# nvaccess/NVSpeechPlayer

Measured on AMD Instinct MI355X. Metric: audio samples/sec (whole node) at 22.05 kHz Klatt synth, batch-N utterances, higher is better.
Workload: dtype f64

## Files before the change

### include/speechPlayer_batch.h

```cpp
#ifndef NVSP_AMD_SPEECHPLAYER_BATCH_H
#define NVSP_AMD_SPEECHPLAYER_BATCH_H

#include "speechPlayer.h"

#ifdef __cplusplus
extern "C" {
#endif

typedef void* speechPlayer_batch_t;

#define SPEECHPLAYER_MODE_EXACT 0
#define SPEECHPLAYER_MODE_FAST 1

speechPlayer_batch_t speechPlayer_batch_create(int sampleRate, int device);
void speechPlayer_batch_destroy(speechPlayer_batch_t batch);

int speechPlayer_batch_setOption(speechPlayer_batch_t batch, const char* name, int value);

int speechPlayer_batch_setUtterances(speechPlayer_batch_t batch, long long nUtterances, const long long* frameStart,
	const speechPlayer_frame_t* frames, const unsigned int* minFrameDuration, const unsigned int* fadeDuration,
	const int* userIndex, const unsigned char* isNull, const unsigned int* noiseSeed);

#define SPEECHPLAYER_RECORD_SILENCE 0xFFFFFFFFu
typedef struct {
	double voicePitch, endVoicePitch;
	unsigned int shape;
	unsigned int minFrameDuration, fadeDuration;
	int userIndex;
} speechPlayer_frameRecord_t;
int speechPlayer_batch_setUtterancesShared(speechPlayer_batch_t batch, long long nLists, const long long* listStart,
	const speechPlayer_frame_t* frames, const unsigned int* minFrameDuration, const unsigned int* fadeDuration,
	const int* userIndex, const unsigned char* isNull, long long nUtterances, const unsigned int* listOf, const unsigned int* noiseSeed);
int speechPlayer_batch_setRecords(speechPlayer_batch_t batch, long long nShapes, const speechPlayer_frame_t* shapes,
	long long nLists, const long long* listStart, const speechPlayer_frameRecord_t* records,
	long long nUtterances, const unsigned int* listOf, const unsigned int* noiseSeed);
int speechPlayer_batch_setUtterancesDevice(speechPlayer_batch_t batch, long long nUtterances, const long long* frameStart,
	const speechPlayer_frame_t* deviceFrames, const unsigned int* minFrameDuration, const unsigned int* fadeDuration,
	const int* userIndex, const unsigned char* isNull, const unsigned int* noiseSeed, void* readyStream);
long long speechPlayer_batch_exportPcm(speechPlayer_batch_t batch, const long long* utterances, long long nUtterances,
	void* deviceOut, int format, long long rowStride, void* stream);
#define SPEECHPLAYER_TRACK_MARK  47
#define SPEECHPLAYER_TRACK_FRAME 48
long long speechPlayer_planTimeline(long long nUtterances, const long long* frameStart, const unsigned int* minFrameDuration,
	const unsigned int* fadeDuration, long long* firstSample, long long* length);
long long speechPlayer_batch_timeline(speechPlayer_batch_t batch, long long utterance, long long* firstSample, int* userIndex,
	long long capacity);
long long speechPlayer_batch_exportTracks(speechPlayer_batch_t batch, const long long* utterances, long long nUtterances,
	const int* columns, int nColumns, long long hop, long long phase, void* deviceOut, int format, long long rowStride, void* stream);
#define SPEECHPLAYER_SOURCE_F0            0
#define SPEECHPLAYER_SOURCE_PHASE         1
#define SPEECHPLAYER_SOURCE_VIBRATO_PHASE 2
#define SPEECHPLAYER_SOURCE_CYCLE         3
#define SPEECHPLAYER_SOURCE_OPEN          4
#define SPEECHPLAYER_SOURCE_WAVE          5
#define SPEECHPLAYER_SOURCE_COLUMNS       6
#define SPEECHPLAYER_EPOCH_COLUMNS 4
long long speechPlayer_batch_exportSource(speechPlayer_batch_t batch, const long long* utterances, long long nUtterances,
	const int* columns, int nColumns, long long hop, long long phase, void* deviceOut, int format, long long rowStride, void* stream);
long long speechPlayer_batch_epochCounts(speechPlayer_batch_t batch, const long long* utterances, long long nUtterances, long long* counts);
long long speechPlayer_batch_exportEpochs(speechPlayer_batch_t batch, const long long* utterances, long long nUtterances,
	void* deviceOut, long long rowStride, double pad, long long capacity, void* stream);
#define SPEECHPLAYER_RESPONSE_CASCADE_RE   0
#define SPEECHPLAYER_RESPONSE_CASCADE_IM   1
#define SPEECHPLAYER_RESPONSE_CASCADE_MAG  2
#define SPEECHPLAYER_RESPONSE_CASCADE_DB   3
#define SPEECHPLAYER_RESPONSE_PARALLEL_RE  4
#define SPEECHPLAYER_RESPONSE_PARALLEL_IM  5
#define SPEECHPLAYER_RESPONSE_PARALLEL_MAG 6
#define SPEECHPLAYER_RESPONSE_PARALLEL_DB  7
#define SPEECHPLAYER_RESPONSE_KINDS        8
long long speechPlayer_frameResponse(const speechPlayer_frame_t* frames, long long nFrames, int sampleRate, const double* frequencies,
	int nFrequencies, const int* kinds, int nKinds, int gain, double* out);
long long speechPlayer_batch_exportResponse(speechPlayer_batch_t batch, const long long* utterances, long long nUtterances,
	const double* frequencies, int nFrequencies, const int* kinds, int nKinds, int gain, long long hop, long long phase,
	void* deviceOut, int format, long long rowStride, void* stream);
#define SPEECHPLAYER_STEM_VOICE      0
#define SPEECHPLAYER_STEM_ASPIRATION 1
#define SPEECHPLAYER_STEM_SOURCE     2
#define SPEECHPLAYER_STEM_FRICATION  3
#define SPEECHPLAYER_STEM_CASCADE    4
#define SPEECHPLAYER_STEM_PARALLEL   5
#define SPEECHPLAYER_STEM_OUTPUT     6
#define SPEECHPLAYER_STEM_COLUMNS    7
long long speechPlayer_batch_exportStems(speechPlayer_batch_t batch, const long long* utterances, long long nUtterances,
	const int* columns, int nColumns, void* deviceOut, int format, long long rowStride, void* stream);
long long speechPlayer_resonatorCoefficients(const double* frequency, const double* bandwidth, long long n, int anti, int sampleRate,
	double* abc);
long long speechPlayer_pcmSpectrogram(const sample* pcm, long long length, int nFft, long long hop, long long phase, const double* window,
	const double* bank, int nBands, int power, double logScale, double floor, double* out);
long long speechPlayer_batch_exportSpectrogram(speechPlayer_batch_t batch, const long long* utterances, long long nUtterances, int nFft,
	long long hop, long long phase, const double* window, const double* bank, int nBands, int power, double logScale, double floor,
	void* deviceOut, int format, long long rowStride, void* stream);
int speechPlayer_batch_device(speechPlayer_batch_t batch);

long long speechPlayer_batch_frames(speechPlayer_batch_t batch, long long utterance, speechPlayer_frame_t* frames,
	unsigned int* minFrameDuration, unsigned int* fadeDuration, int* userIndex, unsigned char* isNull, long long capacity);

long long speechPlayer_batch_utteranceSamples(speechPlayer_batch_t batch, long long utterance);
long long speechPlayer_batch_lengths(speechPlayer_batch_t batch, long long* lengths, long long capacity);
long long speechPlayer_batch_totalSamples(speechPlayer_batch_t batch);
long long speechPlayer_batch_totalFrames(speechPlayer_batch_t batch);
int speechPlayer_batch_sampleRate(speechPlayer_batch_t batch);

int speechPlayer_batch_synthesize(speechPlayer_batch_t batch);
int speechPlayer_batch_wait(speechPlayer_batch_t batch);

long long speechPlayer_batch_read(speechPlayer_batch_t batch, long long utterance, sample* sampleBuf, long long capacity);
long long speechPlayer_batch_readFloat(speechPlayer_batch_t batch, long long utterance, float* sampleBuf, long long capacity);
long long speechPlayer_batch_readAll(speechPlayer_batch_t batch, sample* sampleBuf, long long capacity, long long* outStart);
void* speechPlayer_hostAlloc(long long bytes);
void speechPlayer_hostFree(void* p);
long long speechPlayer_batch_readAllAsync(speechPlayer_batch_t batch, sample* sampleBuf, long long capacity, long long* outStart);
int speechPlayer_batch_readWait(speechPlayer_batch_t batch);
int speechPlayer_batch_digest(speechPlayer_batch_t batch, unsigned long long* perUtterance, unsigned long long* whole);
int speechPlayer_batch_getLastIndex(speechPlayer_batch_t batch, long long utterance);

const sample* speechPlayer_batch_devicePcm(speechPlayer_batch_t batch);
long long speechPlayer_batch_deviceOffset(speechPlayer_batch_t batch, long long utterance);

int speechPlayer_batch_time(speechPlayer_batch_t batch, int launches, float* msPerLaunch);

int speechPlayer_batch_kernelInfo(speechPlayer_batch_t batch, int* info, int nInfo);

long long speechPlayer_planTracks(long long nUtterances, const long long* frameStart, const speechPlayer_frame_t* frames,
	const unsigned int* fadeDuration, const unsigned char* isNull, const unsigned char* eligible, long long budgetMB,
	unsigned long long* trackOff, unsigned int* trackMask, unsigned char* tracked, unsigned long long* nEntries);

long long speechPlayer_planTracksFacts(long long nUtterances, const long long* frameStart, const speechPlayer_frame_t* frames,
	const unsigned int* fadeDuration, const unsigned char* isNull, const unsigned char* eligible, long long budgetMB, const void* facts24,
	unsigned long long* trackOff, unsigned int* trackMask, unsigned char* tracked, unsigned long long* nEntries, long long* collisionAt);
long long speechPlayer_planDirect(long long nUtterances, const long long* frameStart, const unsigned char* isNull,
                                  unsigned int* from, unsigned int* to, unsigned int* flags);
long long speechPlayer_frameFacts(const speechPlayer_frame_t* frames, long long nFrames, int sampleRate, int onDevice, void* facts24);

typedef void* speechPlayer_node_t;
speechPlayer_node_t speechPlayer_node_create(int sampleRate, int nDevices, const int* devices);
void speechPlayer_node_destroy(speechPlayer_node_t node);
int speechPlayer_node_devices(speechPlayer_node_t node);
int speechPlayer_node_setOption(speechPlayer_node_t node, const char* name, int value);
int speechPlayer_node_setUtterances(speechPlayer_node_t node, long long nUtterances, const long long* frameStart,
	const speechPlayer_frame_t* frames, const unsigned int* minFrameDuration, const unsigned int* fadeDuration,
	const int* userIndex, const unsigned char* isNull, const unsigned int* noiseSeed);
int speechPlayer_node_setRecords(speechPlayer_node_t node, long long nShapes, const speechPlayer_frame_t* shapes, long long nLists,
	const long long* listStart, const speechPlayer_frameRecord_t* records, long long nUtterances, const unsigned int* listOf,
	const unsigned int* noiseSeed);
int speechPlayer_node_setIpa(speechPlayer_node_t node, int sampleRate, long long nTexts, const char* const* ipaUtf8, double speed,
	const double* basePitch, double inflection, const char* clauseTypes, const int* voiceOf, const char* voiceName,
	double trailingSilenceMs, const unsigned int* noiseSeed);
int speechPlayer_node_synthesize(speechPlayer_node_t node);
int speechPlayer_node_wait(speechPlayer_node_t node);
long long speechPlayer_node_totalSamples(speechPlayer_node_t node);
long long speechPlayer_node_read(speechPlayer_node_t node, long long utterance, sample* sampleBuf, long long capacity);
int speechPlayer_node_getLastIndex(speechPlayer_node_t node, long long utterance);
int speechPlayer_node_shardInfo(speechPlayer_node_t node, int shard, long long* firstUtterance, long long* nUtterances, long long* samples, int* device);
long long speechPlayer_node_shardUtterances(speechPlayer_node_t node, int shard, long long* utterances, long long capacity);
speechPlayer_batch_t speechPlayer_node_part(speechPlayer_node_t node, int shard);
int speechPlayer_node_time(speechPlayer_node_t node, int launches, float* msPerLaunch);

int speechPlayer_synthesizeMany(speechPlayer_handle_t* handles, int nHandles, unsigned int sampleCount, sample** sampleBufs, int* produced);
int speechPlayer_synthesizeManyDevice(speechPlayer_handle_t* handles, int nHandles, unsigned int sampleCount, const sample** devicePcm,
	long long* rowStride, int* produced);
int speechPlayer_synthesizeManyExport(speechPlayer_handle_t* handles, int nHandles, unsigned int sampleCount, void* deviceOut,
	int format, long long rowStride, void* stream, int* produced);
int speechPlayer_queueFramesMany(const speechPlayer_handle_t* handles, int nHandles, const long long* frameStart,
	const speechPlayer_frame_t* frames, const unsigned int* minFrameDuration, const unsigned int* fadeDuration,
	const int* userIndex, const unsigned char* isNull, const unsigned char* purge);
int speechPlayer_queueFramesManyDevice(const speechPlayer_handle_t* handles, int nHandles, const long long* frameStart,
	const speechPlayer_frame_t* deviceFrames, const unsigned int* minFrameDuration, const unsigned int* fadeDuration,
	const int* userIndex, const unsigned char* isNull, const unsigned char* purge, void* readyStream);
int speechPlayer_handleDevice(speechPlayer_handle_t handle);
float speechPlayer_lastLiveKernelMs(int device);
int speechPlayer_lastLiveLaunches(int device);
int speechPlayer_setGlobalOption(const char* name, int value);
int speechPlayer_setNoiseSeed(speechPlayer_handle_t playerHandle, unsigned int seed);

long long speechPlayer_ipa_frames(const char* ipaUtf8, double speed, double basePitch, double inflection, int clauseType,
	const char* voiceName, speechPlayer_frame_t* frames, unsigned char* isNull, double* durationMs, double* fadeMs, long long capacity);
long long speechPlayer_ipa_pack(int sampleRate, long long nTexts, const char* const* ipaUtf8, double speed, const double* basePitch,
	double inflection, const char* clauseTypes, const char* voiceName, double trailingSilenceMs,
	long long* frameStart, speechPlayer_frame_t* frames, unsigned int* minFrameDuration, unsigned int* fadeDuration,
	unsigned char* isNull, long long frameCapacity);
int speechPlayer_batch_setIpa(speechPlayer_batch_t batch, long long nTexts, const char* const* ipaUtf8, double speed,
	const double* basePitch, double inflection, const char* clauseTypes, const char* voiceName, double trailingSilenceMs,
	const unsigned int* noiseSeed);
int speechPlayer_batch_setIpaVoices(speechPlayer_batch_t batch, long long nTexts, const char* const* ipaUtf8, double speed,
	const double* basePitch, double inflection, const char* clauseTypes, const int* voiceOf, double trailingSilenceMs,
	const unsigned int* noiseSeed);
typedef void* speechPlayer_records_t;
typedef struct {
	long long nShapes; const speechPlayer_frame_t* shapes;
	long long nLists; const long long* listStart;
	long long nRecords; const speechPlayer_frameRecord_t* records;
	long long nUtterances; const unsigned int* listOf;
} speechPlayer_recordsView_t;
speechPlayer_records_t speechPlayer_ipa_records(int sampleRate, long long nTexts, const char* const* ipaUtf8, double speed, const double* basePitch,
	double inflection, const char* clauseTypes, const int* voiceOf, const char* voiceName, double trailingSilenceMs);
int speechPlayer_records_view(speechPlayer_records_t records, speechPlayer_recordsView_t* view);
void speechPlayer_records_free(speechPlayer_records_t records);
typedef struct {
	int phoneme;
	unsigned int flags;
	int unit;
	int textOffset;
} speechPlayer_frameLabel_t;
enum {
	SPEECHPLAYER_LABEL_STRESS_MASK    = 3,
	SPEECHPLAYER_LABEL_TIED_TO        = 4,
	SPEECHPLAYER_LABEL_TIED_FROM      = 8,
	SPEECHPLAYER_LABEL_LONG           = 16,
	SPEECHPLAYER_LABEL_WORD_START     = 32,
	SPEECHPLAYER_LABEL_SYLLABLE_START = 64,
	SPEECHPLAYER_LABEL_GAP            = 128,
	SPEECHPLAYER_LABEL_PUFF           = 256
};
long long speechPlayer_ipa_labels(const char* ipaUtf8, int* phoneme, unsigned int* flags, int* unit, int* textOffset, long long capacity);
int speechPlayer_records_labels(speechPlayer_records_t records, const speechPlayer_frameLabel_t** labels, long long* nLabels);
int speechPlayer_batch_setRecordsLabelled(speechPlayer_batch_t batch, long long nShapes, const speechPlayer_frame_t* shapes,
	long long nLists, const long long* listStart, const speechPlayer_frameRecord_t* records, const speechPlayer_frameLabel_t* labels,
	long long nUtterances, const unsigned int* listOf, const unsigned int* noiseSeed);
int speechPlayer_batch_hasLabels(speechPlayer_batch_t batch);
#define SPEECHPLAYER_ALIGN_PHONEME     0
#define SPEECHPLAYER_ALIGN_STRESS      1
#define SPEECHPLAYER_ALIGN_FLAGS       2
#define SPEECHPLAYER_ALIGN_UNIT        3
#define SPEECHPLAYER_ALIGN_TEXT_OFFSET 4
#define SPEECHPLAYER_ALIGN_FRAME       5
#define SPEECHPLAYER_ALIGN_POSITION    6
#define SPEECHPLAYER_ALIGN_REMAINING   7
#define SPEECHPLAYER_ALIGN_COLUMNS     8
long long speechPlayer_batch_exportAlignment(speechPlayer_batch_t batch, const long long* utterances, long long nUtterances,
	const int* columns, int nColumns, long long hop, long long phase, void* deviceOut, int format, long long rowStride, long long pad,
	long long capacity, void* stream);
#define SPEECHPLAYER_UNIT_COLUMNS 7
long long speechPlayer_batch_exportUnits(speechPlayer_batch_t batch, const long long* utterances, long long nUtterances, long long hop,
	long long phase, int byFrame, void* deviceOut, long long rowStride, long long pad, long long capacity, void* stream);
long long speechPlayer_batch_unitCounts(speechPlayer_batch_t batch, const long long* utterances, long long nUtterances, int byFrame, long long* counts);
int speechPlayer_text_available(void);
long long speechPlayer_text_clauses(const char* textUtf8, long long* begin, long long* end, char* clauseType, double* endPauseMs, long long capacity);
long long speechPlayer_text_fixups(const char* ipaUtf8, char* out, long long capacity);
long long speechPlayer_text_toIpa(const char* textUtf8, const char* espeakVoice, char* out, long long capacity);
int speechPlayer_batch_setText(speechPlayer_batch_t batch, long long nTexts, const char* const* textUtf8, const char* espeakVoice, double speed,
	const double* basePitch, double inflection, const char* voiceName, const unsigned int* noiseSeed);
int speechPlayer_ipa_phonemeCount(void);
int speechPlayer_ipa_phoneme(int index, char* symbolUtf8, int symbolCapacity, double* values, unsigned long long* fieldMask, unsigned int* classBits);
int speechPlayer_voiceCount(void);
int speechPlayer_voicePresetCount(void);
const char* speechPlayer_voiceName(int index);
int speechPlayer_voiceIndex(const char* voiceName);
int speechPlayer_voiceDefine(const char* voiceName, int nEntries, const int* param, const double* absValue, const double* multiplier);
int speechPlayer_applyVoiceToFrame(speechPlayer_frame_t* frame, const char* voiceName);

const char* speechPlayer_lastError(void);
#define SPEECHPLAYER_OK 0
#define SPEECHPLAYER_ERR_ARGUMENT 1
#define SPEECHPLAYER_ERR_NO_DEVICE 2
#define SPEECHPLAYER_ERR_HIP 3
#define SPEECHPLAYER_ERR_TEXT_FRONTEND 4
int speechPlayer_lastErrorCode(void);

#ifdef __cplusplus
}
#endif

#endif
```

### nvspeechplayer_amd/_native.py

```python
import ctypes
import os
import shutil
import subprocess

PKG_DIR = os.path.dirname(os.path.abspath(__file__))
CSRC = os.path.join(PKG_DIR, "csrc")
LIB_DIR = os.path.join(PKG_DIR, "lib")
LIB_PATH = os.path.join(LIB_DIR, "libspeechPlayer.so")
SOURCES = ["klatt_engine.hip", "frame_producer.cpp"]
INCLUDE_DIR = os.path.join(os.path.dirname(PKG_DIR), "include")
OBJ_DIR = os.path.join(PKG_DIR, "build_tmp")
HIPCC_FLAGS = ["-O3", "--offload-arch=gfx950", "-ffp-contract=off", "-fPIC", "-std=c++17", "-Wall", "-Wno-unused-function",
               "-mllvm", "-amdgpu-sched-strategy=max-memory-clause"]
CXX_FLAGS = ["-O2", "-ffp-contract=off", "-fPIC", "-std=c++17", "-Wall", "-Wextra", "-DSPEECHPLAYER_LABELLED_SET"]
LINK_FLAGS = ["-shared", "-fPIC", "--offload-arch=gfx950", "-Wl,-rpath,/opt/rocm/lib"]

EXPORTS = [
    "speechPlayer_initialize", "speechPlayer_queueFrame", "speechPlayer_synthesize",
    "speechPlayer_getLastIndex", "speechPlayer_terminate",
    "speechPlayer_batch_create", "speechPlayer_batch_destroy", "speechPlayer_batch_setOption",
    "speechPlayer_batch_setUtterances", "speechPlayer_batch_utteranceSamples",
    "speechPlayer_batch_totalSamples", "speechPlayer_batch_totalFrames", "speechPlayer_batch_sampleRate",
    "speechPlayer_batch_synthesize", "speechPlayer_batch_wait", "speechPlayer_batch_read",
    "speechPlayer_batch_readAll", "speechPlayer_batch_readAllAsync", "speechPlayer_batch_readWait", "speechPlayer_hostAlloc", "speechPlayer_hostFree",
    "speechPlayer_batch_readFloat", "speechPlayer_batch_digest", "speechPlayer_batch_getLastIndex", "speechPlayer_batch_devicePcm",
    "speechPlayer_batch_deviceOffset", "speechPlayer_batch_time", "speechPlayer_batch_kernelInfo",
    "speechPlayer_lastError", "speechPlayer_lastErrorCode", "speechPlayer_setNoiseSeed", "speechPlayer_synthesizeMany", "speechPlayer_setGlobalOption",
    "speechPlayer_synthesizeManyDevice", "speechPlayer_lastLiveKernelMs", "speechPlayer_lastLiveLaunches",
    "speechPlayer_ipa_frames", "speechPlayer_ipa_pack", "speechPlayer_batch_setIpa",
    "speechPlayer_text_available", "speechPlayer_text_clauses", "speechPlayer_text_fixups", "speechPlayer_text_toIpa", "speechPlayer_batch_setText",
    "speechPlayer_voiceCount", "speechPlayer_voiceName", "speechPlayer_applyVoiceToFrame",
    "speechPlayer_ipa_phonemeCount", "speechPlayer_ipa_phoneme",
    "speechPlayer_node_create", "speechPlayer_node_destroy", "speechPlayer_node_devices", "speechPlayer_node_setOption",
    "speechPlayer_node_setUtterances", "speechPlayer_node_synthesize", "speechPlayer_node_wait", "speechPlayer_node_totalSamples",
    "speechPlayer_node_read", "speechPlayer_node_getLastIndex", "speechPlayer_node_shardInfo", "speechPlayer_node_shardUtterances", "speechPlayer_node_part", "speechPlayer_node_setRecords", "speechPlayer_node_setIpa",
    "speechPlayer_node_time", "speechPlayer_planTracks", "speechPlayer_planDirect", "speechPlayer_frameFacts", "speechPlayer_planTracksFacts",
    "speechPlayer_batch_setUtterancesShared", "speechPlayer_batch_setRecords", "speechPlayer_batch_frames", "speechPlayer_batch_setIpaVoices",
    "speechPlayer_ipa_records", "speechPlayer_records_view", "speechPlayer_records_free", "speechPlayer_voiceIndex", "speechPlayer_voiceDefine", "speechPlayer_voicePresetCount",
    "speechPlayer_batch_setUtterancesDevice", "speechPlayer_batch_exportPcm", "speechPlayer_batch_device", "speechPlayer_batch_lengths",
    "speechPlayer_queueFramesMany", "speechPlayer_queueFramesManyDevice", "speechPlayer_synthesizeManyExport", "speechPlayer_handleDevice",
    "speechPlayer_planTimeline", "speechPlayer_batch_timeline", "speechPlayer_batch_exportTracks",
    "speechPlayer_ipa_labels", "speechPlayer_records_labels", "speechPlayer_batch_setRecordsLabelled", "speechPlayer_batch_hasLabels",
    "speechPlayer_batch_exportAlignment", "speechPlayer_batch_exportUnits", "speechPlayer_batch_unitCounts",
    "speechPlayer_batch_exportSource", "speechPlayer_batch_epochCounts", "speechPlayer_batch_exportEpochs",
    "speechPlayer_frameResponse", "speechPlayer_batch_exportResponse",
    "speechPlayer_batch_exportStems", "speechPlayer_resonatorCoefficients",
    "speechPlayer_pcmSpectrogram", "speechPlayer_batch_exportSpectrogram",
]


def _deps(source):
    own = [os.path.join(CSRC, f) for f in os.listdir(CSRC) if f.endswith((".h", ".inc"))]
    pub = [os.path.join(INCLUDE_DIR, f) for f in os.listdir(INCLUDE_DIR) if f.endswith(".h")]
    return [os.path.join(CSRC, source)] + own + pub


def _obj(source):
    return os.path.join(OBJ_DIR, os.path.splitext(source)[0] + ".o")


def _obj_stale(source):
    o = _obj(source)
    if not os.path.exists(o):
        return True
    t = os.path.getmtime(o)
    return any(os.path.getmtime(p) > t for p in _deps(source))


def _stale():
    if not os.path.exists(LIB_PATH):
        return True
    t = os.path.getmtime(LIB_PATH)
    return any(os.path.getmtime(p) > t for src in SOURCES for p in _deps(src))


def build(force=False, verbose=False, extra_hipcc_flags=(), lib_path=None):
    out = lib_path or LIB_PATH
    variant = bool(extra_hipcc_flags) or lib_path is not None
    if not force and not variant and not _stale():
        return out
    hipcc = shutil.which("hipcc") or "/opt/rocm/bin/hipcc"
    if not os.path.exists(hipcc):
        raise RuntimeError("hipcc not found; cannot build %s" % out)
    os.makedirs(os.path.dirname(out), exist_ok=True)
    os.makedirs(OBJ_DIR, exist_ok=True)
    import fcntl
    with open(os.path.join(OBJ_DIR, ".build.lock"), "w") as lock:
        fcntl.flock(lock, fcntl.LOCK_EX)
        if not force and not variant and not _stale():
            return out
        return _build_locked(hipcc, out, variant, force, verbose, extra_hipcc_flags)


def _build_locked(hipcc, out, variant, force, verbose, extra_hipcc_flags):
    objs = []
    for src in SOURCES:
        is_hip = src.endswith(".hip")
        own = variant and is_hip
        o = os.path.join(OBJ_DIR, os.path.basename(out) + "." + os.path.splitext(src)[0] + ".o") if own else _obj(src)
        if force or own or _obj_stale(src):
            flags = list(HIPCC_FLAGS)
            extra = list(extra_hipcc_flags)
            for f in [f for f in extra if f.startswith("--sched=")]:
                extra.remove(f)
                i = flags.index("-mllvm")
                del flags[i:i + 2]
                if f != "--sched=none":
                    flags += ["-mllvm", "-amdgpu-sched-strategy=" + f[len("--sched="):]]
            cmd = ([hipcc] + flags + extra if is_hip else ["g++"] + CXX_FLAGS) + ["-c", os.path.join(CSRC, src), "-o", o]
            if verbose:
                print(" ".join(cmd))
            subprocess.check_call(cmd)
        objs.append(o)
    tmp = out + ".tmp.%d" % os.getpid()
    cmd = [hipcc] + LINK_FLAGS + ["-o", tmp] + objs
    if verbose:
        print(" ".join(cmd))
    subprocess.check_call(cmd)
    os.replace(tmp, out)
    if variant:
        for o in objs:
            if os.path.basename(o).startswith(os.path.basename(out) + "."):
                try:
                    os.remove(o)
                except OSError:
                    pass
    return out


_lib = None


def load():
    global _lib
    if _lib is not None:
        return _lib
    path = os.environ.get("SPEECHPLAYER_LIB", LIB_PATH)
    if not os.path.exists(path):
        raise RuntimeError("%s is missing: run `python -c 'import __graft_entry__ as g; g.build()'` "
                           "(the engine has no CPU fallback)" % path)
    L = ctypes.CDLL(path)
    vp, u32, i32, i64 = ctypes.c_void_p, ctypes.c_uint, ctypes.c_int, ctypes.c_longlong
    L.speechPlayer_initialize.restype = vp
    L.speechPlayer_initialize.argtypes = [i32]
    L.speechPlayer_queueFrame.restype = None
    L.speechPlayer_queueFrame.argtypes = [vp, vp, u32, u32, i32, ctypes.c_bool]
    L.speechPlayer_synthesize.restype = i32
    L.speechPlayer_synthesize.argtypes = [vp, u32, vp]
    L.speechPlayer_getLastIndex.restype = i32
    L.speechPlayer_getLastIndex.argtypes = [vp]
    L.speechPlayer_terminate.restype = None
    L.speechPlayer_terminate.argtypes = [vp]
    L.speechPlayer_setNoiseSeed.restype = i32
    L.speechPlayer_setNoiseSeed.argtypes = [vp, u32]
    L.speechPlayer_synthesizeMany.restype = i32
    L.speechPlayer_synthesizeMany.argtypes = [vp, i32, u32, vp, vp]
    L.speechPlayer_synthesizeManyDevice.restype = i32
    L.speechPlayer_synthesizeManyDevice.argtypes = [vp, i32, u32, vp, vp, vp]
    L.speechPlayer_synthesizeManyExport.restype = i32
    L.speechPlayer_synthesizeManyExport.argtypes = [vp, i32, u32, vp, i32, i64, vp, vp]
    L.speechPlayer_queueFramesMany.restype = i32
    L.speechPlayer_queueFramesMany.argtypes = [vp, i32, vp, vp, vp, vp, vp, vp, vp]
    L.speechPlayer_queueFramesManyDevice.restype = i32
    L.speechPlayer_queueFramesManyDevice.argtypes = [vp, i32, vp, vp, vp, vp, vp, vp, vp, vp]
    L.speechPlayer_handleDevice.restype = i32
    L.speechPlayer_handleDevice.argtypes = [vp]
    L.speechPlayer_lastLiveKernelMs.restype = ctypes.c_float
    L.speechPlayer_lastLiveKernelMs.argtypes = [i32]
    L.speechPlayer_lastLiveLaunches.restype = i32
    L.speechPlayer_lastLiveLaunches.argtypes = [i32]
    L.speechPlayer_setGlobalOption.restype = i32
    L.speechPlayer_setGlobalOption.argtypes = [ctypes.c_char_p, i32]
    L.speechPlayer_lastError.restype = ctypes.c_char_p
    L.speechPlayer_lastError.argtypes = []
    L.speechPlayer_lastErrorCode.restype = i32
    L.speechPlayer_lastErrorCode.argtypes = []
    L.speechPlayer_batch_create.restype = vp
    L.speechPlayer_batch_create.argtypes = [i32, i32]
    L.speechPlayer_batch_destroy.restype = None
    L.speechPlayer_batch_destroy.argtypes = [vp]
    L.speechPlayer_batch_setOption.restype = i32
    L.speechPlayer_batch_setOption.argtypes = [vp, ctypes.c_char_p, i32]
    L.speechPlayer_batch_setUtterances.restype = i32
    L.speechPlayer_batch_setUtterances.argtypes = [vp, i64, vp, vp, vp, vp, vp, vp, vp]
    L.speechPlayer_batch_utteranceSamples.restype = i64
    L.speechPlayer_batch_utteranceSamples.argtypes = [vp, i64]
    L.speechPlayer_batch_totalSamples.restype = i64
    L.speechPlayer_batch_totalSamples.argtypes = [vp]
    L.speechPlayer_batch_totalFrames.restype = i64
    L.speechPlayer_batch_totalFrames.argtypes = [vp]
    L.speechPlayer_batch_synthesize.restype = i32
    L.speechPlayer_batch_synthesize.argtypes = [vp]
    L.speechPlayer_batch_wait.restype = i32
    L.speechPlayer_batch_wait.argtypes = [vp]
    L.speechPlayer_batch_read.restype = i64
    L.speechPlayer_batch_read.argtypes = [vp, i64, vp, i64]
    L.speechPlayer_batch_readFloat.restype = i64
    L.speechPlayer_batch_readFloat.argtypes = [vp, i64, vp, i64]
    L.speechPlayer_batch_readAll.restype = i64
    L.speechPlayer_batch_readAll.argtypes = [vp, vp, i64, vp]
    L.speechPlayer_batch_readAllAsync.restype = i64
    L.speechPlayer_batch_readAllAsync.argtypes = [vp, vp, i64, vp]
    L.speechPlayer_batch_readWait.restype = i32
    L.speechPlayer_batch_readWait.argtypes = [vp]
    L.speechPlayer_hostAlloc.restype = vp
    L.speechPlayer_hostAlloc.argtypes = [i64]
    L.speechPlayer_hostFree.restype = None
    L.speechPlayer_hostFree.argtypes = [vp]
    L.speechPlayer_batch_digest.restype = i32
    L.speechPlayer_batch_digest.argtypes = [vp, vp, vp]
    L.speechPlayer_batch_getLastIndex.restype = i32
    L.speechPlayer_batch_getLastIndex.argtypes = [vp, i64]
    L.speechPlayer_batch_devicePcm.restype = vp
    L.speechPlayer_batch_devicePcm.argtypes = [vp]
    L.speechPlayer_batch_deviceOffset.restype = i64
    L.speechPlayer_batch_deviceOffset.argtypes = [vp, i64]
    L.speechPlayer_batch_time.restype = i32
    L.speechPlayer_batch_time.argtypes = [vp, i32, vp]
    L.speechPlayer_batch_kernelInfo.restype = i32
    L.speechPlayer_batch_kernelInfo.argtypes = [vp, vp, i32]
    L.speechPlayer_batch_sampleRate.restype = i32
    L.speechPlayer_batch_sampleRate.argtypes = [vp]
    f64 = ctypes.c_double
    L.speechPlayer_ipa_frames.restype = i64
    L.speechPlayer_ipa_frames.argtypes = [ctypes.c_char_p, f64, f64, f64, i32, ctypes.c_char_p, vp, vp, vp, vp, i64]
    L.speechPlayer_ipa_pack.restype = i64
    L.speechPlayer_ipa_pack.argtypes = [i32, i64, vp, f64, vp, f64, ctypes.c_char_p, ctypes.c_char_p, f64, vp, vp, vp, vp, vp, i64]
    L.speechPlayer_text_available.restype = i32
    L.speechPlayer_text_available.argtypes = []
    L.speechPlayer_text_clauses.restype = i64
    L.speechPlayer_text_clauses.argtypes = [ctypes.c_char_p, vp, vp, vp, vp, i64]
    L.speechPlayer_text_fixups.restype = i64
    L.speechPlayer_text_fixups.argtypes = [ctypes.c_char_p, vp, i64]
    L.speechPlayer_text_toIpa.restype = i64
    L.speechPlayer_text_toIpa.argtypes = [ctypes.c_char_p, ctypes.c_char_p, vp, i64]
    L.speechPlayer_batch_setText.restype = i32
    L.speechPlayer_batch_setText.argtypes = [vp, i64, vp, ctypes.c_char_p, f64, vp, f64, ctypes.c_char_p, vp]
    L.speechPlayer_batch_setIpa.restype = i32
    L.speechPlayer_batch_setIpa.argtypes = [vp, i64, vp, f64, vp, f64, ctypes.c_char_p, ctypes.c_char_p, f64, vp]
    L.speechPlayer_node_create.restype = vp
    L.speechPlayer_node_create.argtypes = [i32, i32, vp]
    L.speechPlayer_node_destroy.restype = None
    L.speechPlayer_node_destroy.argtypes = [vp]
    L.speechPlayer_node_devices.restype = i32
    L.speechPlayer_node_devices.argtypes = [vp]
    L.speechPlayer_node_setOption.restype = i32
    L.speechPlayer_node_setOption.argtypes = [vp, ctypes.c_char_p, i32]
    L.speechPlayer_node_setUtterances.restype = i32
    L.speechPlayer_node_setUtterances.argtypes = [vp, i64, vp, vp, vp, vp, vp, vp, vp]
    L.speechPlayer_node_synthesize.restype = i32
    L.speechPlayer_node_synthesize.argtypes = [vp]
    L.speechPlayer_node_wait.restype = i32
    L.speechPlayer_node_wait.argtypes = [vp]
    L.speechPlayer_node_totalSamples.restype = i64
    L.speechPlayer_node_totalSamples.argtypes = [vp]
    L.speechPlayer_node_read.restype = i64
    L.speechPlayer_node_read.argtypes = [vp, i64, vp, i64]
    L.speechPlayer_node_getLastIndex.restype = i32
    L.speechPlayer_node_getLastIndex.argtypes = [vp, i64]
    L.speechPlayer_node_shardInfo.restype = i32
    L.speechPlayer_node_shardInfo.argtypes = [vp, i32, vp, vp, vp, vp]
    L.speechPlayer_node_shardUtterances.restype = i64
    L.speechPlayer_node_shardUtterances.argtypes = [vp, i32, vp, i64]
    L.speechPlayer_node_setRecords.restype = i32
    L.speechPlayer_node_setRecords.argtypes = [vp, i64, vp, i64, vp, vp, i64, vp, vp]
    L.speechPlayer_node_setIpa.restype = i32
    L.speechPlayer_node_setIpa.argtypes = [vp, i32, i64, vp, f64, vp, f64, ctypes.c_char_p, vp, ctypes.c_char_p, f64, vp]
    L.speechPlayer_node_part.restype = vp
    L.speechPlayer_node_part.argtypes = [vp, i32]
    L.speechPlayer_node_time.restype = i32
    L.speechPlayer_node_time.argtypes = [vp, i32, vp]
    L.speechPlayer_voiceCount.restype = i32
    L.speechPlayer_voiceCount.argtypes = []
    L.speechPlayer_voiceName.restype = ctypes.c_char_p
    L.speechPlayer_voiceName.argtypes = [i32]
    L.speechPlayer_applyVoiceToFrame.restype = i32
    L.speechPlayer_applyVoiceToFrame.argtypes = [vp, ctypes.c_char_p]
    L.speechPlayer_ipa_phonemeCount.restype = i32
    L.speechPlayer_ipa_phonemeCount.argtypes = []
    L.speechPlayer_ipa_phoneme.restype = i32
    L.speechPlayer_ipa_phoneme.argtypes = [i32, vp, i32, vp, vp, vp]
    L.speechPlayer_planTracks.restype = i64
    L.speechPlayer_planTracks.argtypes = [i64, vp, vp, vp, vp, vp, i64, vp, vp, vp, vp]
    L.speechPlayer_frameFacts.restype = i64
    L.speechPlayer_frameFacts.argtypes = [vp, i64, i32, i32, vp]
    L.speechPlayer_planDirect.restype = i64
    L.speechPlayer_planDirect.argtypes = [i64, vp, vp, vp, vp, vp]
    L.speechPlayer_planTracksFacts.restype = i64
    L.speechPlayer_planTracksFacts.argtypes = [i64, vp, vp, vp, vp, vp, i64, vp, vp, vp, vp, vp, vp]
    L.speechPlayer_batch_setUtterancesDevice.restype = i32
    L.speechPlayer_batch_setUtterancesDevice.argtypes = [vp, i64, vp, vp, vp, vp, vp, vp, vp, vp]
    L.speechPlayer_planTimeline.restype = i64
    L.speechPlayer_planTimeline.argtypes = [i64, vp, vp, vp, vp, vp]
    L.speechPlayer_batch_timeline.restype = i64
    L.speechPlayer_batch_timeline.argtypes = [vp, i64, vp, vp, i64]
    L.speechPlayer_batch_exportTracks.restype = i64
    L.speechPlayer_batch_exportTracks.argtypes = [vp, vp, i64, vp, i32, i64, i64, vp, i32, i64, vp]
    L.speechPlayer_batch_exportPcm.restype = i64
    L.speechPlayer_batch_exportPcm.argtypes = [vp, vp, i64, vp, i32, i64, vp]
    L.speechPlayer_batch_device.restype = i32
    L.speechPlayer_batch_device.argtypes = [vp]
    L.speechPlayer_batch_lengths.restype = i64
    L.speechPlayer_batch_lengths.argtypes = [vp, vp, i64]
    L.speechPlayer_batch_setUtterancesShared.restype = i32
    L.speechPlayer_batch_setUtterancesShared.argtypes = [vp, i64, vp, vp, vp, vp, vp, vp, i64, vp, vp]
    L.speechPlayer_batch_setRecords.restype = i32
    L.speechPlayer_batch_setRecords.argtypes = [vp, i64, vp, i64, vp, vp, i64, vp, vp]
    L.speechPlayer_batch_frames.restype = i64
    L.speechPlayer_batch_frames.argtypes = [vp, i64, vp, vp, vp, vp, vp, i64]
    L.speechPlayer_batch_setIpaVoices.restype = i32
    L.speechPlayer_batch_setIpaVoices.argtypes = [vp, i64, vp, f64, vp, f64, ctypes.c_char_p, vp, f64, vp]
    L.speechPlayer_ipa_records.restype = vp
    L.speechPlayer_ipa_records.argtypes = [i32, i64, vp, f64, vp, f64, ctypes.c_char_p, vp, ctypes.c_char_p, f64]
    L.speechPlayer_records_view.restype = i32
    L.speechPlayer_records_view.argtypes = [vp, vp]
    L.speechPlayer_records_free.restype = None
    L.speechPlayer_records_free.argtypes = [vp]
    L.speechPlayer_voicePresetCount.restype = i32
    L.speechPlayer_voicePresetCount.argtypes = []
    L.speechPlayer_voiceIndex.restype = i32
    L.speechPlayer_voiceIndex.argtypes = [ctypes.c_char_p]
    L.speechPlayer_voiceDefine.restype = i32
    L.speechPlayer_voiceDefine.argtypes = [ctypes.c_char_p, i32, vp, vp, vp]
    L.speechPlayer_ipa_labels.restype = i64
    L.speechPlayer_ipa_labels.argtypes = [ctypes.c_char_p, vp, vp, vp, vp, i64]
    L.speechPlayer_records_labels.restype = i32
    L.speechPlayer_records_labels.argtypes = [vp, vp, vp]
    L.speechPlayer_batch_setRecordsLabelled.restype = i32
    L.speechPlayer_batch_setRecordsLabelled.argtypes = [vp, i64, vp, i64, vp, vp, vp, i64, vp, vp]
    L.speechPlayer_batch_hasLabels.restype = i32
    L.speechPlayer_batch_hasLabels.argtypes = [vp]
    L.speechPlayer_batch_exportAlignment.restype = i64
    L.speechPlayer_batch_exportAlignment.argtypes = [vp, vp, i64, vp, i32, i64, i64, vp, i32, i64, i64, i64, vp]
    L.speechPlayer_batch_exportUnits.restype = i64
    L.speechPlayer_batch_exportUnits.argtypes = [vp, vp, i64, i64, i64, i32, vp, i64, i64, i64, vp]
    L.speechPlayer_batch_unitCounts.restype = i64
    L.speechPlayer_batch_unitCounts.argtypes = [vp, vp, i64, i32, vp]
    L.speechPlayer_batch_exportSource.restype = i64
    L.speechPlayer_batch_exportSource.argtypes = [vp, vp, i64, vp, i32, i64, i64, vp, i32, i64, vp]
    L.speechPlayer_batch_epochCounts.restype = i64
    L.speechPlayer_batch_epochCounts.argtypes = [vp, vp, i64, vp]
    L.speechPlayer_batch_exportEpochs.restype = i64
    L.speechPlayer_batch_exportEpochs.argtypes = [vp, vp, i64, vp, i64, f64, i64, vp]
    L.speechPlayer_frameResponse.restype = i64
    L.speechPlayer_frameResponse.argtypes = [vp, i64, i32, vp, i32, vp, i32, i32, vp]
    L.speechPlayer_batch_exportResponse.restype = i64
    L.speechPlayer_batch_exportResponse.argtypes = [vp, vp, i64, vp, i32, vp, i32, i32, i64, i64, vp, i32, i64, vp]
    L.speechPlayer_batch_exportStems.restype = i64
    L.speechPlayer_batch_exportStems.argtypes = [vp, vp, i64, vp, i32, vp, i32, i64, vp]
    L.speechPlayer_resonatorCoefficients.restype = i64
    L.speechPlayer_resonatorCoefficients.argtypes = [vp, vp, i64, i32, i32, vp]
    L.speechPlayer_pcmSpectrogram.restype = i64
    L.speechPlayer_pcmSpectrogram.argtypes = [vp, i64, i32, i64, i64, vp, vp, i32, i32, f64, f64, vp]
    L.speechPlayer_batch_exportSpectrogram.restype = i64
    L.speechPlayer_batch_exportSpectrogram.argtypes = [vp, vp, i64, i32, i64, i64, vp, vp, i32, i32, f64, f64, vp, i32, i64, vp]
    _lib = L
    return L


def last_error():
    return (load().speechPlayer_lastError() or b"").decode("utf8", "replace")


# ... 3 lines not shown
```

### nvspeechplayer_amd/csrc/klatt_device.h

```cpp
#pragma once

#include <hip/hip_runtime.h>
#include <stdint.h>
#include <type_traits>

#include "klatt_math.h"

namespace klatt {

constexpr int kNumParams = 47;
constexpr int kLanes = 64;
constexpr int kTile = 32;
constexpr int kTileStride = kTile * 2 + 8;
constexpr int kSlots = 45;
constexpr int kNumRes = 14;
constexpr int kBlock = 16;
constexpr int kStateDoubles = 240;

constexpr int MODE_EXACT = 0;
constexpr int MODE_FAST = 1;

constexpr uint32_t FRAME_NULL = 1u;
constexpr uint32_t UTT_NEEDS_NOISE = 1u;
constexpr uint32_t UTT_TRACKED = 4u;
// ... 2 lines not shown

struct FrameMeta {
    uint32_t minSamples;
    uint32_t fadeSamples;
    int32_t userIndex;
    uint32_t flags;
};

struct UttDesc {
    long long frameStart;
    long long outStart;
    uint32_t nFrames;
    uint32_t seed;
    uint32_t flags;
    uint32_t length;
};

struct UttResult {
    uint32_t produced;
    uint32_t framesTaken;
    int32_t lastIndex;
    uint32_t drained;
};

constexpr int kTrackEntries = 24;
constexpr int kTrackFirst = kTrackEntries + 1;
constexpr int kShapeValues = 45;
constexpr int kShapeStride = 46;
__host__ __device__ constexpr int shape_param(int i)
{
    constexpr int kF[14] = {13, 14, 12, 11, 10, 9, 8, 7, 25, 26, 27, 28, 29, 30};
    constexpr int kB[14] = {21, 22, 20, 19, 18, 17, 16, 15, 31, 32, 33, 34, 35, 36};
    constexpr int kG[17] = {23, 41, 42, 43, 45, 24, 44, 37, 38, 39, 40, 1, 2, 3, 4, 5, 6};
    return i < 28 ? ((i & 1) ? kB[i >> 1] : kF[i >> 1]) : kG[i - 28];
}
constexpr int kShapePreGain = 28 + 6;
__host__ __device__ constexpr int entry_value(int e, int half)
{
    constexpr int kV[10][2] = {{28, -1}, {29, 30}, {31, 32}, {33, 34}, {35, 36}, {37, 38}, {39, 40}, {41, 42}, {43, 44}, {34, -1}};
    return kV[e - 14][half];
}
struct TrackRef {
    unsigned long long off;
    uint32_t mask;
    uint32_t nSlots;
};
struct FlatRef {
    uint32_t off;
    uint32_t mask;
    uint32_t fadeSamples;
    uint32_t span;
};
struct SourceRef {
    double pitch;
    double pitchInc;
    double invFade;
    int32_t userIndex;
    uint32_t flags;
};
struct TrackJob {
    unsigned long long off;
    uint32_t fromShape, toShape;
    uint32_t fadeSamples;
    uint32_t mask;
};
__host__ __device__ inline uint32_t track_slots(uint32_t mask) { return (uint32_t)__builtin_popcount(mask) + (mask & 1u); }
constexpr int kTrackStages = 4;
#ifndef KLATT_FLAT_LAYOUT
#define KLATT_FLAT_LAYOUT 2
#endif
__host__ __device__ constexpr uint32_t track_stage_kinds(int s)
{
    return KLATT_FLAT_LAYOUT == 2 ? (s == 0 ? 0xF04003u : s == 1 ? 0x0000FCu : s == 2 ? 0x01B000u : 0x0E0F00u)
                                  : (s == 0 ? 0xF00000u : s == 1 ? 0x00403Fu : s == 2 ? 0x01B0C0u : 0x0E0F00u);
}
__host__ __device__ constexpr uint32_t track_stage_entries(int s)
{
    return KLATT_FLAT_LAYOUT == 2 ? (s == 0 ? 8u : s == 1 ? 6u : s == 2 ? 4u : 7u) : (s == 0 ? 4u : s == 1 ? 8u : s == 2 ? 6u : 7u);
}
constexpr int kTrackAntiStage = KLATT_FLAT_LAYOUT == 2 ? 0 : 1;
__host__ __device__ inline uint32_t track_stage_slots(uint32_t mask, int s) { return (uint32_t)__builtin_popcount(mask & track_stage_kinds(s)) + (s == kTrackAntiStage ? (mask & 1u) : 0u); }
__host__ __device__ inline uint32_t track_part(uint32_t mask, uint32_t F, int s)
{
    uint32_t at = 0;
    for (int k = 0; k < s; ++k) at += track_stage_entries(k) + (F - 1u) * track_stage_slots(mask, k);
    return at;
}

struct DirectHdr {
    uint32_t fadeSamples;
    uint32_t span;
    uint32_t bits;
    uint32_t pad;
};
struct DirectJob {
    uint32_t frame;
    uint32_t from, to;
    uint32_t flags;
};
constexpr uint32_t kNoFrame = 0xFFFFFFFFu;
constexpr uint32_t kDirectBwShift = 8, kDirectClsShift = 14, kDirectAllBits = 0x3FFFFFFu;
constexpr int kDirectStages = 8;
#ifndef KLATT_DIRECT_FAST_LAYOUT
#define KLATT_DIRECT_FAST_LAYOUT 1
#endif
__host__ __device__ constexpr int direct_layout(int mode) { return mode == MODE_FAST ? KLATT_DIRECT_FAST_LAYOUT : 0; }
__host__ __device__ constexpr int direct_stage_res(int s, int L = 0)
{
    return L == 1 ? (s < 2 ? 0 : (s == 3 || s == 4) ? 3 : 2) : (s == 0 ? 0 : 2);
}
__host__ __device__ constexpr int direct_stage_gains(int s, int L = 0)
{
    return L == 1 ? (s == 0 ? 1 : s == 1 ? 3 : s == 2 ? 1 : s == 5 ? 2 : s == 6 ? 1 : s == 7 ? 2 : 0)
                  : (s == 0 ? 4 : s == 1 ? 1 : s == 5 ? 2 : s == 6 ? 1 : s == 7 ? 2 : 0);
}
__host__ __device__ constexpr int direct_stage_entries(int s, int L = 0) { return 4 * direct_stage_res(s, L) + 3 * direct_stage_gains(s, L); }
__host__ __device__ constexpr int direct_stage_first(int s, int L = 0) { int at = 0; for (int k = 0; k < s; ++k) at += direct_stage_entries(k, L); return at; }
constexpr int kDirectEntries = direct_stage_first(kDirectStages);
static_assert(direct_stage_first(kDirectStages, 1) == kDirectEntries, "both layouts hold the same kinds");
__host__ __device__ constexpr int direct_stage_kind(int s, int e, int L = 0)
{
    constexpr int k0[kDirectStages][4] = {{20, 21, 22, 23}, {0, 1, 14, -1}, {2, 3, -1, -1}, {4, 5, -1, -1}, {6, 7, -1, -1}, {8, 9, 17, 18}, {10, 11, 19, -1}, {12, 13, 15, 16}};
    constexpr int k1[kDirectStages][4] = {{20, -1, -1, -1}, {21, 22, 23, -1}, {0, 1, 14, -1}, {2, 3, 4, -1}, {5, 6, 7, -1}, {8, 9, 17, 18}, {10, 11, 19, -1}, {12, 13, 15, 16}};
    return L == 1 ? k1[s][e] : k0[s][e];
}

struct KernelArgs {
    const DirectHdr* directHdr;
    const double2* directRec;
    const uint32_t* directFirst;
    uint32_t nDirect;
    const FlatRef* flatRef;
    const SourceRef* sourceRef;
    uint32_t trackBytes;
    const double2* track;
    const double* frames;
    const FrameMeta* meta;
    const UttDesc* utt;
    const uint32_t* order;
    int16_t* pcm;
    UttResult* result;
    double* state;
    double* const* statePtrs;
    const uint32_t* control;
    long long nSlots;
    uint32_t maxSamples;
    uint32_t ringMask;
    int sampleRate;
    double sampleRateF;
    double invSampleRate;
    double negPiOverSr;
    double twoPiOverSr;
    unsigned long long* debug;
};

__device__ constexpr int kResF[kNumRes] = {13, 14, 12, 11, 10, 9, 8, 7, 25, 26, 27, 28, 29, 30};
__device__ constexpr int kResB[kNumRes] = {21, 22, 20, 19, 18, 17, 16, 15, 31, 32, 33, 34, 35, 36};
constexpr int kNumHot = 17;
__device__ constexpr int kHot[kNumHot] = {1, 2, 3, 4, 5, 6, 23, 24, 37, 38, 39, 40, 41, 42, 43, 44, 45};


__device__ __forceinline__ double div_by(double x, double b, double y)
{
    double q = x * y;
    double r = __builtin_fma(-b, q, x);
    return __builtin_fma(r, y, q);
}

__device__ __forceinline__ double frac_toward_zero(double x) { return x - __builtin_trunc(x); }

__device__ __forceinline__ double fade_value(double from, double to, double ratio)
{
    double v = from + ((to - from) * ratio);
    return (to != to) ? from : v;
}

__device__ __forceinline__ uint32_t mix32(uint32_t x)
{
    x ^= x >> 16; x *= 0x7FEB352Du; x ^= x >> 15; x *= 0x846CA68Bu; x ^= x >> 16;
    return x;
}
__device__ __forceinline__ uint32_t noise_key(uint32_t seed) { return mix32(seed ^ 0x9E3779B9u); }
__device__ __forceinline__ uint32_t noise_inc(uint32_t seed) { return (mix32(seed + 0x85EBCA6Bu) << 1) | 1u; }
constexpr uint32_t kNoiseA = 1664525u;
constexpr uint32_t kNoiseA2 = kNoiseA * kNoiseA;
__device__ __forceinline__ uint32_t noise_inc2(uint32_t inc) { return (kNoiseA + 1u) * inc; }
__device__ __forceinline__ uint32_t noise_step(uint32_t s, uint32_t inc) { return s * kNoiseA + inc; }
__device__ __forceinline__ uint32_t noise_step2(uint32_t s, uint32_t inc2) { return s * kNoiseA2 + inc2; }
__device__ __forceinline__ uint32_t noise_first(uint32_t key, uint32_t inc) { return noise_step(key, inc); }
__device__ __forceinline__ double noise_uniform(uint32_t s)
{
    const double r = (double)(s >> 1);
    return __builtin_fma(r, 0x1.00000002p-31, r * 0x1p-93);
}

template <int MODE>
__device__ __forceinline__ double dot3(double a, double x, double b, double y, double c, double z)
{
    if (MODE == MODE_FAST) return __builtin_fma(c, z, __builtin_fma(b, y, a * x));
    return a * x + b * y + c * z;
}

#ifdef KLATT_SIGNAL_F32
typedef float sig_t;
#else
typedef double sig_t;
#endif
template <int MODE>
__device__ __forceinline__ float dot3(float a, float x, float b, float y, float c, float z)
{
    return __builtin_fmaf(c, z, __builtin_fmaf(b, y, a * x));
}
__device__ __forceinline__ float fade_value(float from, float to, float ratio)
{
    float v = from + ((to - from) * ratio);
    return (to != to) ? from : v;
}

struct Coef { double a, b, c; };
enum { COEF_UNREDUCED = 0, COEF_QUADRANT_M1 = 1, COEF_UNKNOWN = 2 };
#ifndef KLATT_COLD_CALL
#define KLATT_COLD_CALL 2
#endif
struct RadCos { double rad, cs; };
#if KLATT_COLD_CALL
__device__ __attribute__((noinline)) RadCos exp_cos_reduced(double ex, double th)
{
    RadCos o;
#if KLATT_COLD_CALL == 1
    if (__builtin_fabs(ex) <= 700.0 && __builtin_fabs(th) <= 1.0e4) { o.rad = fast_exp(ex); o.cs = fast_cos(th); }
    else
#endif
    { o.rad = exp(ex); o.cs = cos(th); }
    return o;
}
#endif
template <bool NESTED = true>
__device__ __forceinline__ RadCos coefficient_parts(double f, double bw, double negPiOverSr, double twoPiOverSr, int cls = COEF_UNKNOWN)
{
    const double ex = negPiOverSr * bw;
    const double th = twoPiOverSr * -f;
    double rad, cs;
    const bool eu = exp_is_unreduced(ex);
    if (cls == COEF_UNREDUCED) { rad = exp_unreduced(ex); cs = cos_unreduced(th); }
    else if (cls == COEF_QUADRANT_M1) { rad = exp_unreduced(ex); cs = cos_quadrant_m1(th); }
    else if (__all(eu && cos_is_unreduced(th))) { rad = exp_unreduced(ex); cs = cos_unreduced(th); }
    else if (__all(eu && cos_is_quadrant_m1(th))) { rad = exp_unreduced(ex); cs = cos_quadrant_m1(th); }
#if KLATT_COLD_CALL == 1
    else if (NESTED) { const RadCos o = exp_cos_reduced(ex, th); rad = o.rad; cs = o.cs; }
#endif
    else if (__builtin_fabs(ex) <= 700.0 && __builtin_fabs(th) <= 1.0e4) { rad = fast_exp(ex); cs = fast_cos(th); }
#if KLATT_COLD_CALL == 2
    else if (NESTED) { const RadCos o = exp_cos_reduced(ex, th); rad = o.rad; cs = o.cs; }
#endif
    else { rad = exp(ex); cs = cos(th); }
    RadCos o; o.rad = rad; o.cs = cs;
    return o;
}
__host__ __device__ __forceinline__ Coef coefficient_finish(double rad, double cs, bool anti, double f)
{
    double cc = -(rad * rad);
    double bb = rad * cs * 2.0;
    double aa = 1.0 - bb - cc;
    if (anti && f != 0) {
        aa = 1.0 / aa;
        cc *= -aa;
        bb *= -aa;
    }
    Coef k; k.a = aa; k.b = bb; k.c = cc;
    return k;
}
template <int MODE, bool NESTED = true>
__device__ __forceinline__ Coef resonator_coefficients_inline(double f, double bw, bool anti, double negPiOverSr, double twoPiOverSr,
                                                              int cls = COEF_UNKNOWN)
{
    const RadCos p = coefficient_parts<NESTED>(f, bw, negPiOverSr, twoPiOverSr, cls);
    return coefficient_finish(p.rad, p.cs, anti, f);
}
template <int MODE>
__device__ __attribute__((noinline)) Coef resonator_coefficients(double f, double bw, bool anti, double negPiOverSr, double twoPiOverSr)
{
    return resonator_coefficients_inline<MODE, false>(f, bw, anti, negPiOverSr, twoPiOverSr);
}

template <bool STREAM>
struct LdsLayout {
    static constexpr int kOld = 0;
    static constexpr int kNew = kOld + kSlots * kLanes * 8;
    static constexpr int kCurFB = kNew + kSlots * kLanes * 8;
    static constexpr int kTileOff = kCurFB + (STREAM ? 28 * kLanes * 8 : 0);
    static constexpr int kRowBase = kTileOff + kLanes * kTileStride;
    static constexpr int kRowCount = kRowBase + kLanes * 8;
    static constexpr int kBytes = kRowCount + kLanes * 4;
};

struct Lane {
    double cur[kNumParams];
    double old0, new0, oldInc, newInc, invFade;
    double ra[kNumRes], rb[kNumRes], rc[kNumRes], z1[kNumRes], z2[kNumRes];
    double pitchPhase, vibPhase, aspNoise, fricNoise;
    uint32_t cnt, oldMin, newMin, newFade;
    uint32_t resMask, nextFrame, noiseState, produced;
    int32_t lastIndex;
    bool hasNew, oldNull, newNull, done, drained;
    bool vibFrames;
};
// ... 381 lines not shown
```

### nvspeechplayer_amd/csrc/klatt_engine.hip

```cpp
#include "klatt_device.h"
#include "klatt_systolic.h"
#include "klatt_lanepipe.h"
#include "klatt_tracks.h"
#include "klatt_direct.h"
#include "klatt_plan.h"
#include "klatt_timeline.h"
#include "klatt_align.h"
#include "klatt_source.h"
#include "klatt_response.h"
#include "klatt_stems.h"
#include "klatt_spectrum.h"
#include "klatt_export.h"

#include <algorithm>
#include <cmath>
#include <cstdarg>
#include <cstdio>
#include <cstdlib>
#include <cstring>
#include <chrono>
#include <mutex>
#include <atomic>
#include <system_error>
#include <thread>
// ... 334 lines not shown
    a.sampleRate = sampleRate;
    a.sampleRateF = (double)sampleRate;
    a.invSampleRate = 1.0 / (double)sampleRate;
    a.negPiOverSr = -M_PI / sampleRate;
    a.twoPiOverSr = (M_PI * 2) / sampleRate;
    a.maxSamples = 0xFFFFFFFFu;
    return a;
}

template <bool NOISE, int CH, int WPS = 1, bool NASAL = true, bool STREAM = false, bool FLAT = false, bool LONE = false>
int launch_systolic(const KernelArgs& a, int mode, long long nGroups, hipStream_t stream)
{
    if (nGroups <= 0) return 0;
    if (nGroups > 0x7FFFFFFF) { set_error("too many workgroups: %lld", nGroups); return -1; }
    constexpr int ldsBytes = SysLds<NOISE, CH, FLAT, stream_split<STREAM, WPS, LONE>()>::kBytes + (LONE ? kStages * kLoneLdsPerStage : 0);
    static_assert(ldsBytes <= 160 * 1024, "a workgroup's LDS");
    auto go = [&](auto kernel) -> int {
        if (ensure_lds_limit(reinterpret_cast<const void*>(kernel), ldsBytes)) return -1;
        hipLaunchKernelGGL(kernel, dim3((unsigned)nGroups), dim3(kLanes * kStages), ldsBytes, stream, a);
        return 0;
    };
    int rc;
    switch (mode) {
    case MODE_EXACT: rc = go(klatt_systolic<MODE_EXACT, NOISE, CH, WPS, NASAL, STREAM, FLAT, LONE>); break;
    case MODE_FAST: rc = go(klatt_systolic<MODE_FAST, NOISE, CH, WPS, NASAL, STREAM, FLAT, LONE>); break;
    default: set_error("unknown arithmetic mode %d", mode); return -1;
    }
    if (rc) return rc;
    HIP_TRY(hipGetLastError());
    return 0;
}

constexpr int kDirectChunk = 16, kDirectLeanChunk = 8;
template <int CH, int WPE>
int launch_direct_as(const KernelArgs& a, int mode, long long nGroups, hipStream_t stream)
{
    constexpr int ldsBytes = DirectLds<CH>::kBytes;
    auto go = [&](auto kernel) -> int {
        if (ensure_lds_limit(reinterpret_cast<const void*>(kernel), ldsBytes)) return -1;
        hipLaunchKernelGGL(kernel, dim3((unsigned)nGroups), dim3(kLanes * kDirectStages), ldsBytes, stream, a);
        return 0;
    };
    int rc;
    switch (mode) {
    case MODE_EXACT: rc = go(klatt_direct<MODE_EXACT, CH, WPE>); break;
    case MODE_FAST: rc = go(klatt_direct<MODE_FAST, CH, WPE>); break;
    default: set_error("unknown arithmetic mode %d", mode); return -1;
    }
    if (rc) return rc;
    HIP_TRY(hipGetLastError());
    return 0;
}
int launch_direct(const KernelArgs& a, int mode, bool lean, long long nGroups, hipStream_t stream)
{
    if (nGroups <= 0) return 0;
    if (nGroups > 0x7FFFFFFF) { set_error("too many workgroups: %lld", nGroups); return -1; }
    return lean ? launch_direct_as<kDirectLeanChunk, 4>(a, mode, nGroups, stream) : launch_direct_as<kDirectChunk, 2>(a, mode, nGroups, stream);
}

#ifndef KLATT_LP_CH
#define KLATT_LP_CH 32
#endif
template <int CH, int WPS>
int launch_lanepipe(const KernelArgs& a, int mode, long long nGroups, hipStream_t stream)
{
    if (nGroups <= 0) return 0;
    if (nGroups > 0x7FFFFFFF) { set_error("too many workgroups: %lld", nGroups); return -1; }
    constexpr int ldsBytes = LpLds<CH>::kBytes;
    auto go = [&](auto kernel) -> int {
        if (ensure_lds_limit(reinterpret_cast<const void*>(kernel), ldsBytes)) return -1;
        hipLaunchKernelGGL(kernel, dim3((unsigned)nGroups), dim3(kLanes * kStages), ldsBytes, stream, a);
        return 0;
    };
    int rc;
    switch (mode) {
    case MODE_EXACT: rc = go(klatt_lanepipe<MODE_EXACT, CH, WPS>); break;
    case MODE_FAST: rc = go(klatt_lanepipe<MODE_FAST, CH, WPS>); break;
    default: set_error("unknown arithmetic mode %d", mode); return -1;
    }
    if (rc) return rc;
    HIP_TRY(hipGetLastError());
    return 0;
}

#ifndef KLATT_NOISY_CH
#define KLATT_NOISY_CH 8
#endif
struct GroupPlan { bool systolic; int chunk; };
GroupPlan plan_group(int layout, bool noisy, long long nUttBatch, long long nNoisyBatch, int cus)
{
    const long long groups = (nUttBatch + kLanes - 1) / kLanes + 1;
    GroupPlan p;
    p.systolic = layout != 0;
    (void)nNoisyBatch;
    p.chunk = noisy ? (groups <= cus ? 16 : 8)
                    : (groups <= cus ? 32 : 16);
    return p;
}

template <bool STREAM, bool NOISE>
int launch(const KernelArgs& a, int mode, long long nWaves, hipStream_t stream)
{
    if (nWaves <= 0) return 0;
    if (nWaves > 0x7FFFFFFF) { set_error("too many wavefronts: %lld", nWaves); return -1; }
    constexpr int ldsBytes = LdsLayout<STREAM>::kBytes;
    auto go = [&](auto kernel) -> int {
        if (ensure_lds_limit(reinterpret_cast<const void*>(kernel), ldsBytes)) return -1;
        hipLaunchKernelGGL(kernel, dim3((unsigned)nWaves), dim3(kLanes), ldsBytes, stream, a);
        return 0;
    };
    int rc;
    switch (mode) {
    case MODE_EXACT: rc = go(klatt_synthesize<MODE_EXACT, STREAM, NOISE>); break;
    case MODE_FAST: rc = go(klatt_synthesize<MODE_FAST, STREAM, NOISE>); break;
    default:
        set_error("unknown arithmetic mode %d", mode);
        return -1;
    }
    if (rc) return rc;
    HIP_TRY(hipGetLastError());
    return 0;
}

int pick_device(int device)
{
    int n = 0;
    hipError_t e = hipGetDeviceCount(&n);
    if (e != hipSuccess || n <= 0) {
        set_error_code(SPEECHPLAYER_ERR_NO_DEVICE);
        set_error("no HIP device available (%s); this engine has no CPU path", e == hipSuccess ? "count 0" : hipGetErrorString(e));
        return -1;
    }
    if (device < 0) {
        const char* env = getenv("SPEECHPLAYER_DEVICE");
        if (env) device = atoi(env);
        else if (hipGetDevice(&device) != hipSuccess) device = 0;
    }
    if (device >= n) { set_error("device %d out of range (%d devices)", device, n); return -1; }
    return device;
}

struct Batch {
    int sampleRate = 0;
    int device = 0;
    int mode = MODE_EXACT;
    int sortByLength = 1;
    int layout = -1;
    int cus = 256;
    hipStream_t stream = nullptr;
    int tracks = 1;
    long long trackBudgetMB = 4096;
    hipStream_t side[6] = {nullptr, nullptr, nullptr, nullptr, nullptr, nullptr};
    hipEvent_t forkEvent = nullptr, join[6] = {nullptr, nullptr, nullptr, nullptr, nullptr, nullptr};
    int quietLast = 1;
    long long nUtt = 0, nFrames = 0, nSlots = 0;
    long long nLists = 0, nFramesSpoken = 0;
    std::vector<long long> uttFrameStart;
    std::vector<uint32_t> uttFrames;
    bool launched = false;
    long long nQuiet = 0;
    long long nTracked = 0;
    long long nTrackedUtt = 0;
    long long nJobs = 0, trackEntries = 0;
    int directLean = -1;
    bool directAligned = false;
    int direct = 1;
    long long nDirect = 0;
    long long nDirectUtt = 0, nDirectFrames = 0;
    long long nNoNasal = 0;
    long long nNoNasalUtt = 0;
    long long totalSamples = 0, poolSamples = 0;
    std::vector<uint32_t> lens;
    std::vector<uint32_t> uttSeed;
    std::vector<long long> outStart;
    std::vector<UttResult> results;
    bool resultsFresh = false;
    DeviceBuffer<double> dFrames;
    DeviceBuffer<FrameMeta> dMeta;
    DeviceBuffer<UttDesc> dUtt;
    DeviceBuffer<uint32_t> dOrder;
    DeviceBuffer<int16_t> dPcm;
    DeviceBuffer<UttResult> dResult;
    DeviceBuffer<FlatRef> dFlatRef;
    DeviceBuffer<SourceRef> dSourceRef;
    DeviceBuffer<TrackJob> dJobs;
    DeviceBuffer<double> dShapes;
    DeviceBuffer<double2> dTrack;
    DeviceBuffer<DirectJob> dDirectJobs;
    DeviceBuffer<uint32_t> dDirectFirst;
    DeviceBuffer<DirectHdr> dDirectHdr;
    DeviceBuffer<double2> dDirectRec;
    DeviceBuffer<unsigned long long> dDebug;
    DeviceBuffer<float> dFloat;
    DeviceBuffer<unsigned long long> dDigest;
    PinnedPair bounce;
    DeviceBuffer<FrameRecord> dRecords;
    DeviceBuffer<double> dShapeTable;
    DeviceBuffer<uint32_t> dRep;
    DeviceBuffer<unsigned long long> dMismatch;
    DeviceBuffer<FrameFacts> dFacts;
    PinnedBlock hFacts;
    DeviceBuffer<int16_t> dDense;
    DeviceBuffer<long long> dDenseStart;
    std::vector<long long> denseStart;
    hipStream_t copyStream = nullptr;
    hipEvent_t denseReady = nullptr, copyDone = nullptr;
    bool copyPending = false;
    bool floatFresh = false;
    hipEvent_t inputReady = nullptr;
    DeviceBuffer<long long> dShapeIdx;
    DeviceBuffer<double> dShapeRows;
    hipEvent_t pcmReady = nullptr;
    struct ExportSlot { PinnedBlock host; DeviceBuffer<unsigned char> dev; hipEvent_t done = nullptr; bool used = false; };
    static constexpr int kExportSlots = 16;
    ExportSlot exportSlot[kExportSlots];
    unsigned exportNext = 0;
    struct SharedTable {
        hipEvent_t done = nullptr;
        bool used = false;
        int wait(hipStream_t st) { if (used) HIP_TRY(hipStreamWaitEvent(st, done, 0)); return 0; }
        int mark(hipStream_t st) { HIP_TRY(hipEventRecord(done, st)); used = true; return 0; }
    };
    std::vector<uint32_t> uttList;
    DeviceBuffer<long long> dListStart;
    DeviceBuffer<TimelineReq> dTimeline;
    hipEvent_t setDone = nullptr, setCopied = nullptr, timelineReady = nullptr;
    bool timelineFresh = false;
    ExportSlot trackSlot[kExportSlots];
    unsigned trackNext = 0;
    DeviceBuffer<double> dPitch;
    SharedTable pitchOrder;
    long long pitchBudgetMB = 256;
    DeviceBuffer<FrameLabel> dLabels;
    DeviceBuffer<uint32_t> dUnitFirst;
    std::vector<uint32_t> listUnits;
    bool hasLabels = false;
    DeviceBuffer<double> dSource;
    DeviceBuffer<double> dEpochs;
    SharedTable sourceOrder;
    DeviceBuffer<long long> dEpochCount;
    std::vector<long long> epochCount;
    bool epochFresh = false;
    long long sourceBudgetMB = 256;
    long long sourceLaneLists = 12288;
};

int wait_exports(Batch* b)
{
    for (auto& s : b->exportSlot)
        if (s.used) HIP_TRY(hipStreamWaitEvent(b->stream, s.done, 0));
    return 0;
}
int sync_exports(Batch* b)
{
    for (auto& s : b->exportSlot)
        if (s.used) { HIP_TRY(hipEventSynchronize(s.done)); s.used = false; }
    return 0;
}

int settle_track_exports(Batch* b, bool onHost)
{
    for (auto& s : b->trackSlot) {
        if (!s.used) continue;
        if (onHost) { HIP_TRY(hipEventSynchronize(s.done)); s.used = false; }
        else { HIP_TRY(hipStreamWaitEvent(b->stream, s.done, 0)); HIP_TRY(hipStreamWaitEvent(b->copyStream, s.done, 0)); }
    }
    return 0;
}


template <typename T>
int grow_table(Batch* b, DeviceBuffer<T>& buf, size_t n)
{
    if (n > buf.cap && settle_track_exports(b, true)) return -1;
    return buf.reserve(std::max<size_t>(n, 1));
}

int timeline_on_stream(Batch* b, hipStream_t st)
{
    if (b->timelineFresh) { HIP_TRY(hipStreamWaitEvent(st, b->timelineReady, 0)); return 0; }
    if (grow_table(b, b->dTimeline, (size_t)b->nFrames)) return -1;
    HIP_TRY(hipStreamWaitEvent(st, b->setDone, 0));
    HIP_TRY(hipStreamWaitEvent(st, b->setCopied, 0));
    const unsigned grid = (unsigned)std::min<long long>((b->nLists + 255) / 256, 4ll * b->cus);
    hipLaunchKernelGGL(klatt_timeline_requests, dim3(std::max(grid, 1u)), dim3(256), 0, st, b->dMeta.ptr, b->dListStart.ptr, b->nLists, b->dTimeline.ptr);
    HIP_TRY(hipGetLastError());
    HIP_TRY(hipEventRecord(b->timelineReady, st));
    b->timelineFresh = true;
    return 0;
}

template <class Fn>
long long batch_entry(const char* what, speechPlayer_batch_t batch, Fn fn)
{
    begin_call();
    Batch* b = static_cast<Batch*>(batch);
    if (!b) { set_error("%s: no batch", what); return -1; }
    try {
        return fn(b);
    } catch (const std::exception& e) { set_error("%s: %s", what, e.what()); return -1; }
}

long long check_selection(Batch* b, const char* what, const long long* utterances, long long nUtterances, bool frameLimit)
{
    const long long n = utterances ? nUtterances : b->nUtt;
    if (n < 0) { set_error("%s: %lld utterances", what, n); return -1; }
// ... 404 lines not shown
    });
    lap("parts planned");
    struct ShapeKey { const double* v; bool operator==(const ShapeKey& o) const { return !memcmp(v, o.v, kShapeValues * sizeof(double)); } };
    struct ShapeKeyHash { size_t operator()(const ShapeKey& k) const { return (size_t)hash_shape(k.v); } };
    struct FadeKey { uint32_t from, to, len; bool operator==(const FadeKey& o) const { return from == o.from && to == o.to && len == o.len; } };
    struct FadeKeyHash { size_t operator()(const FadeKey& k) const { unsigned long long h = ((unsigned long long)k.from << 32 | k.to) * 0x9E3779B97F4A7C15ull; h ^= h >> 29; h += k.len; h *= 0xFF51AFD7ED558CCDull; return (size_t)(h ^ (h >> 32)); } };
    long long eligibleAll = 0, missedSize = 0, missedBudget = 0;
    size_t nShapesUpper = 0;
    for (const TrackPlan& p : part) { eligibleAll += p.eligible; missedSize += p.missedSize; missedBudget += p.missedBudget; nShapesUpper += p.shapes.size() / kShapeStride; }
    if (missedBudget > 0) {
        part.clear();
        plan_tracks_pass(nUtterances, frameStart, frames, facts, meta, eligible, budgetMB, true, nullptr, out);
        return;
    }
    out.shapes.clear();
    out.shapes.reserve(nShapesUpper * kShapeStride);
    out.jobs.clear();
    out.entries = 0;
    std::unordered_map<ShapeKey, uint32_t, ShapeKeyHash> shapes;
    std::unordered_map<FadeKey, unsigned long long, FadeKeyHash> fades;
    std::vector<std::unordered_map<unsigned long long, unsigned long long>> offOf(nThreads);
    for (unsigned t = 0; t < nThreads; ++t) {
        const TrackPlan& p = part[t];
        std::vector<uint32_t> gid(p.shapes.size() / kShapeStride);
        for (size_t i = 0; i < gid.size(); ++i) {
            const ShapeKey key{&p.shapes[i * kShapeStride]};
            auto it = shapes.find(key);
            if (it == shapes.end()) {
                const uint32_t id = (uint32_t)(out.shapes.size() / kShapeStride);
                out.shapes.insert(out.shapes.end(), key.v, key.v + kShapeStride);
                it = shapes.emplace(ShapeKey{&out.shapes[(size_t)id * kShapeStride]}, id).first;
            }
            gid[i] = it->second;
        }
        for (const TrackJob& j : p.jobs) {
            const FadeKey key{gid[j.fromShape], gid[j.toShape], j.fadeSamples};
            auto it = fades.find(key);
            if (it == fades.end()) {
                it = fades.emplace(key, out.entries).first;
                out.jobs.push_back(TrackJob{out.entries, key.from, key.to, j.fadeSamples, j.mask});
                out.entries += (unsigned long long)kTrackFirst + (unsigned long long)(j.fadeSamples - 1u) * track_slots(j.mask);
            }
            offOf[t].emplace(j.off, it->second);
        }
    }
    const unsigned long long budget = std::min((unsigned long long)std::max(budgetMB, 0ll) * (1ull << 20) / sizeof(double2), (1ull << 28) - (1ull << 21) - kTrackPad);
    if (out.entries > budget) {
        plan_tracks_pass(nUtterances, frameStart, frames, facts, meta, eligible, budgetMB, true, nullptr, out);
        return;
    }
    out.eligible = eligibleAll; out.missedSize = missedSize; out.missedBudget = 0;
    out.ref.assign((size_t)nF, TrackRef{0, 0, 0});
    out.rep.assign(nF < 0xFFFFFFFFll ? (size_t)nF : 0, 0xFFFFFFFFu);
    out.tracked.assign((size_t)nUtterances, 0);
    out.kinds.assign((size_t)nUtterances, 0);
    if (missedSize * 10 > eligibleAll) { out.jobs.clear(); out.entries = 0; return; }
    run_parts(nThreads, [&](unsigned t) {
        const TrackPlan& p = part[t];
        const long long f0 = frameStart[cut[t]];
        for (long long u = cut[t]; u < cut[t + 1]; ++u) {
            if (!p.tracked[u - cut[t]]) continue;
            out.tracked[u] = 1;
            out.kinds[u] = p.kinds[u - cut[t]];
            for (long long k = frameStart[u]; k < frameStart[u + 1]; ++k) {
                TrackRef r = p.ref[k - f0];
                r.off = offOf[t].find(r.off)->second;
                out.ref[k] = r;
                if (!out.rep.empty() && !p.rep.empty()) out.rep[k] = p.rep[k - f0];
            }
        }
    });
    lap("merged");
}

#ifdef KLATT_TIMING_ONLY_BUILD
constexpr bool kTimingOnlyBuild = true;
#else
constexpr bool kTimingOnlyBuild = false;
#endif
bool refuse_timing_only(const char* what)
{
    if (!kTimingOnlyBuild || getenv("SPEECHPLAYER_ALLOW_TIMING_ONLY_PCM")) return false;
    set_error_code(SPEECHPLAYER_ERR_ARGUMENT);
    set_error("%s: this library was built with a timing-only experiment switch; its PCM is not valid", what);
    return true;
}

template <class V>
void walk_fade_ends(long long k0, long long k1, const FrameMeta* meta, V& out)
{
    uint32_t prevReal = kNoFrame;
    bool prevNull = true;
    for (long long k = k0; k < k1; ++k) {
        DirectJob j;
        j.frame = (uint32_t)k;
        if (meta[k].flags & FRAME_NULL) {
            j.from = prevReal; j.to = prevReal;
            j.flags = (prevNull ? 1u : 0u) | 2u;
            prevNull = true;
        } else {
            j.to = (uint32_t)k;
            j.from = prevNull ? (uint32_t)k : prevReal;
            j.flags = prevNull ? 1u : 0u;
            prevReal = (uint32_t)k;
            prevNull = false;
        }
        out.push_back(j);
    }
}

template <class T>
struct NoInitAlloc : std::allocator<T> {
    template <class U> struct rebind { using other = NoInitAlloc<U>; };
    NoInitAlloc() = default;
    template <class U> NoInitAlloc(const NoInitAlloc<U>&) {}
    template <class U> void construct(U* p) { ::new (static_cast<void*>(p)) U; }
    template <class U, class... A> void construct(U* p, A&&... a) { ::new (static_cast<void*>(p)) U(std::forward<A>(a)...); }
};
template <class T> using RawVector = std::vector<T, NoInitAlloc<T>>;

long long tracked_count(const Batch* b) { return (b->tracks && b->layout != 0) ? b->nTracked : 0; }
long long direct_count(const Batch* b) { return b->nDirect; }
bool direct_lean(const Batch* b, long long nGroups)
{
    if (b->directLean >= 0) return b->directLean != 0;
    if (b->directAligned) return false;
    return b->mode == MODE_FAST ? true : nGroups > 2ll * b->cus;
}

int batch_launch(Batch* b)
{
    KernelArgs a = base_args(b->sampleRate);
    a.frames = b->dFrames.ptr; a.meta = b->dMeta.ptr; a.utt = b->dUtt.ptr;
    a.pcm = b->dPcm.ptr; a.result = b->dResult.ptr; a.state = nullptr; a.control = nullptr;
    if (wait_exports(b)) return -1;
    b->resultsFresh = false;
    b->floatFresh = false;
    b->launched = true;
#ifdef KLATT_STAMPS
    if (b->dDebug.reserve((size_t)(b->nSlots / kLpUPG + 2) * 32 * 2)) return -1;
    HIP_TRY(hipMemsetAsync(b->dDebug.ptr, 0, b->dDebug.cap * 8, b->stream));
    a.debug = b->dDebug.ptr;
#endif
    const long long nLp = lanepipe_count(b);
    const bool laneKernel = b->layout == 0;
    const long long nTr = tracked_count(b);
    const long long nDir = direct_count(b);
    const long long nNoisyHead = b->nTracked - nTr;
    const long long nNoisy = b->nSlots - b->nQuiet - b->nTracked - nDir;
    const long long nNn = laneKernel ? 0 : b->nNoNasal - nLp;
    const long long nQ = b->nQuiet - nLp - nNn;
    const int parts = (nLp > 0) + (nNn > 0) + (nQ > 0) + (nNoisy > 0) + (nNoisyHead > 0) + (nTr > 0) + (nDir > 0);
    const bool fork = parts > 1;
    if (fork) HIP_TRY(hipEventRecord(b->forkEvent, b->stream));
    int sideUsed = 0, seen = 0;
    auto next_stream = [&](bool = false) -> hipStream_t {
        if (!fork || ++seen == parts) return b->stream;
        hipStream_t st = b->side[sideUsed++];
        (void)hipStreamWaitEvent(st, b->forkEvent, 0);
        return st;
    };
    const GroupPlan plq = plan_group(b->layout, false, b->nSlots, nNoisy, b->cus);
    auto launch_quiet = [&]() -> int {
    if (nLp > 0) {
        hipStream_t st = next_stream(true);
        a.order = b->dOrder.ptr; a.nSlots = nLp;
        const long long g = (nLp + kLpUPG - 1) / kLpUPG;
        if (g <= b->cus ? launch_lanepipe<KLATT_LP_CH, 1>(a, b->mode, g, st) : launch_lanepipe<16, 2>(a, b->mode, g, st)) return -1;
    }
    if (nNn > 0) {
        hipStream_t st = next_stream(true);
        a.order = b->dOrder.ptr + nLp; a.nSlots = nNn;
        const long long g = (nNn + kLanes - 1) / kLanes;
        if (plq.chunk == 32 ? launch_systolic<false, 32, 1, false>(a, b->mode, g, st) : launch_systolic<false, 16, 2, false>(a, b->mode, g, st)) return -1;
    }
    if (nQ > 0) {
        hipStream_t st = next_stream(true);
        a.order = b->dOrder.ptr + nLp + nNn; a.nSlots = nQ;
        const long long g = (nQ + kLanes - 1) / kLanes;
        if (plq.systolic ? (plq.chunk == 32 ? launch_systolic<false, 32>(a, b->mode, g, st) : launch_systolic<false, 16>(a, b->mode, g, st))
                         : launch<false, false>(a, b->mode, g, st)) return -1;
    }
        return 0;
    };
    const bool quietLast = b->quietLast && (nTr > 0 || nDir > 0) && nNoisy == 0 && nNoisyHead == 0;
    if (!quietLast && launch_quiet()) return -1;
    if (nTr > 0) {
        hipStream_t st = next_stream();
        TrackArgs t;
        t.jobs = b->dJobs.ptr; t.nJobs = b->nJobs; t.shapes = b->dShapes.ptr; t.track = b->dTrack.ptr;
        t.negPiOverSr = a.negPiOverSr; t.twoPiOverSr = a.twoPiOverSr;
        const long long tg = b->nJobs;
        if (tg > 0x7FFFFFFF) { set_error("too many tracks: %lld", b->nJobs); return -1; }
        hipLaunchKernelGGL(klatt_tracks, dim3((unsigned)tg), dim3(kLanes * kTrackWaves), 0, st, t);
        HIP_TRY(hipGetLastError());
        a.order = b->dOrder.ptr + b->nQuiet; a.nSlots = nTr;
        a.flatRef = b->dFlatRef.ptr; a.sourceRef = b->dSourceRef.ptr; a.track = b->dTrack.ptr;
        a.trackBytes = (uint32_t)std::min<unsigned long long>(((unsigned long long)b->trackEntries + kTrackPad) * sizeof(double2), 0xFFFFFFFFull);
        const GroupPlan pl = plan_group(b->layout, true, b->nSlots, nTr + nNoisy, b->cus);
        const long long g = (nTr + kLanes - 1) / kLanes;
        if (pl.chunk == 8 ? launch_systolic<true, KLATT_FLAT_CH, KLATT_FLAT_WPS, true, false, true>(a, b->mode, g, st)
                          : launch_systolic<true, 16, 1, true, false, true>(a, b->mode, g, st)) return -1;
        a.flatRef = nullptr; a.sourceRef = nullptr; a.track = nullptr;
    }
    if (nDir > 0) {
        hipStream_t st = next_stream();
        SeedArgs sa;
        sa.jobs = b->dDirectJobs.ptr; sa.nJobs = (uint32_t)b->nDirectFrames; sa.frames = b->dFrames.ptr; sa.meta = b->dMeta.ptr;
        sa.hdr = b->dDirectHdr.ptr; sa.rec = b->dDirectRec.ptr; sa.negPiOverSr = a.negPiOverSr; sa.twoPiOverSr = a.twoPiOverSr;
        const dim3 sg((unsigned)((b->nDirectFrames + 255) / 256), (unsigned)kDirectStages);
        constexpr int kSeedLds = 14 * 257 * (int)sizeof(double2);
        if (b->mode == MODE_FAST) hipLaunchKernelGGL(klatt_seeds<MODE_FAST>, sg, dim3(256), kSeedLds, st, sa);
        else hipLaunchKernelGGL(klatt_seeds<MODE_EXACT>, sg, dim3(256), kSeedLds, st, sa);
        HIP_TRY(hipGetLastError());
        a.order = b->dOrder.ptr + b->nQuiet + b->nTracked; a.nSlots = nDir;
        a.directHdr = b->dDirectHdr.ptr; a.directRec = b->dDirectRec.ptr; a.directFirst = b->dDirectFirst.ptr; a.nDirect = (uint32_t)b->nDirectFrames;
        a.sourceRef = b->dSourceRef.ptr;
        const long long g = (nDir + kLanes - 1) / kLanes;
        if (launch_direct(a, b->mode, direct_lean(b, g), g, st)) return -1;
        a.directHdr = nullptr; a.directRec = nullptr; a.directFirst = nullptr; a.nDirect = 0; a.sourceRef = nullptr;
    }
    for (int half = 0; half < 2; ++half) {
        const long long n = half ? nNoisy : nNoisyHead;
        if (n <= 0) continue;
        hipStream_t st = next_stream();
        a.order = b->dOrder.ptr + b->nQuiet + (half ? b->nTracked + nDir : 0); a.nSlots = n;
        const GroupPlan pl = plan_group(b->layout, true, b->nSlots, nTr + nNoisy + nNoisyHead, b->cus);
        const long long g = (n + kLanes - 1) / kLanes;
        if (pl.systolic ? (pl.chunk == 8 ? launch_systolic<true, KLATT_NOISY_CH, 2>(a, b->mode, g, st) : launch_systolic<true, 16>(a, b->mode, g, st))
                        : launch<false, true>(a, b->mode, g, st)) return -1;
    }
    if (quietLast && launch_quiet()) return -1;
    for (int i = 0; i < sideUsed; ++i) {
        HIP_TRY(hipEventRecord(b->join[i], b->side[i]));
        HIP_TRY(hipStreamWaitEvent(b->stream, b->join[i], 0));
    }
    return 0;
}

constexpr uint32_t kRing = 256;
constexpr size_t kLogEntries = 40960;
constexpr size_t kLogEager = 2560;
constexpr uint32_t kNoTarget = 0xFFFFFFFFu;

struct LogEntry {
    double p[kNumParams];
    FrameMeta meta;
    uint32_t target;
    uint32_t pad;
};
static_assert(sizeof(LogEntry) == 400, "LogEntry layout");

struct PendingFrame {
    double p[kNumParams];
    FrameMeta meta;
};

__global__ void __launch_bounds__(256) live_scatter(const LogEntry* __restrict__ log, uint32_t n, double* __restrict__ ringFrames,
                                                    FrameMeta* __restrict__ ringMeta)
{
    const uint32_t e = blockIdx.x * 4u + (threadIdx.x >> 6), j = threadIdx.x & 63u;
    if (e >= n) return;
    const uint32_t at = log[e].target;
    if (at == kNoTarget) return;
    if (j < (uint32_t)kNumParams) ringFrames[(size_t)at * kNumParams + j] = log[e].p[j];
    else if (j == (uint32_t)kNumParams) ringMeta[at] = log[e].meta;
}

struct LivePlace {
    FrameMeta meta;
    long long row;
    uint32_t target;
    uint32_t pad;
};
static_assert(sizeof(LivePlace) == 32, "LivePlace layout");

__global__ void __launch_bounds__(256) live_place(const double* __restrict__ frames, const LivePlace* __restrict__ place, long long n,
                                                  double* __restrict__ ringFrames, FrameMeta* __restrict__ ringMeta)
{
    const uint32_t j = threadIdx.x & 63u;
    const long long step = (long long)gridDim.x * 4;
    for (long long e = (long long)blockIdx.x * 4 + (threadIdx.x >> 6); e < n; e += step) {
        const LivePlace p = place[e];
        if (j < (uint32_t)kNumParams) ringFrames[(size_t)p.target * kNumParams + j] = p.row < 0 ? 0.0 : frames[p.row * kNumParams + j];
        else if (j == (uint32_t)kNumParams) ringMeta[p.target] = p.meta;
    }
}

inline uint32_t frame_span(const FrameMeta& m)
{
    const unsigned long long v = std::max<unsigned long long>(m.minSamples, (unsigned long long)m.fadeSamples + 1) + 1;
    return (uint32_t)std::min<unsigned long long>(v, 0xFFFFFFFFull);
}

struct Stream {
    int sampleRate = 0;
    int device = 0;
    int mode = MODE_EXACT;
    uint32_t seed = 0;
    uintptr_t id = 0;
    std::mutex mu;
    struct LiveContext* context = nullptr;
    uint32_t slot = 0;
    uint32_t ringHead = 0;
    uint32_t ringCount = 0;
    uint32_t span[kRing];
    std::vector<PendingFrame> overflow;
    size_t overHead = 0;
    uint32_t logEpoch = 0;
    std::vector<uint32_t> logIdx;
    bool purgePending = false;
    int lastIndex = -1;
};

std::mutex g_tableMutex;
std::vector<Stream*> g_streams;

Stream* lookup_locked(speechPlayer_handle_t h)
{
    uintptr_t id = reinterpret_cast<uintptr_t>(h);
    id &= 0xFFFFFFFFu;
    if (id == 0 || id > g_streams.size()) return nullptr;
    return g_streams[id - 1];
}
Stream* lookup(speechPlayer_handle_t h)
{
    std::lock_guard<std::mutex> g(g_tableMutex);
    return lookup_locked(h);
}

template <typename T>
struct PinnedBuffer {
    T* ptr = nullptr;
    size_t cap = 0;
    int reserve(size_t n)
    {
        if (n <= cap) return 0;
        n = std::max(n, cap * 2);
        if (ptr) (void)hipHostFree(ptr);
        ptr = nullptr; cap = 0;
        HIP_TRY(hipHostMalloc(reinterpret_cast<void**>(&ptr), n * sizeof(T), hipHostMallocDefault));
        cap = n;
        return 0;
    }
};

struct LiveContext {
    std::mutex mu;
    hipStream_t stream = nullptr;
    uint32_t slots = 0, nextSlot = 0;
    std::vector<uint32_t> freeSlots;
    DeviceBuffer<double> dState;
    DeviceBuffer<double> dRingFrames;
    DeviceBuffer<FrameMeta> dRingMeta;
    std::mutex logMu;
    PinnedBuffer<LogEntry> hLog;
// ... 771 lines not shown
    std::vector<Fill> fill;
    size_t nPlace = 0, nGather = 0;
    for (int i = 0; i < q.n; ++i) {
        const long long k0 = q.frameStart[i], k1 = q.frameStart[i + 1];
        if (k0 == k1) continue;
        Stream* s = ss[i];
        if (q.purge && q.purge[i]) stream_purge(c, s);
        for (long long k = k0; k < k1; ++k) {
            const FrameMeta meta = queue_meta(q, k);
            const bool null = (meta.flags & FRAME_NULL) != 0;
            if (ring_takes(s)) {
                LivePlace& p = c->hPlace.ptr[nPlace++];
                p.meta = meta; p.row = null ? -1 : k; p.pad = 0;
                p.target = ring_claim(s, meta);
            } else {
                overflow_push(s, nullptr, meta);
                if (!null) { c->hGatherIdx.ptr[nGather++] = k; fill.push_back(Fill{s, s->overflow.size() - 1}); }
            }
        }
    }
    if (nGather && (c->hGatherRows.reserve(nGather * kNumParams) || c->dGatherRows.reserve(c->hGatherRows.cap))) return -1;
    if (nPlace) {
        HIP_TRY(hipMemcpyAsync(c->dPlace.ptr, c->hPlace.ptr, nPlace * sizeof(LivePlace), hipMemcpyHostToDevice, c->stream));
        const unsigned grid = (unsigned)std::min<size_t>((nPlace + 3) / 4, (size_t)1 << 20);
        hipLaunchKernelGGL(live_place, dim3(grid), dim3(256), 0, c->stream, frames, c->dPlace.ptr, (long long)nPlace, c->dRingFrames.ptr, c->dRingMeta.ptr);
        HIP_TRY(hipGetLastError());
    }
    if (nGather) {
        HIP_TRY(hipMemcpyAsync(c->dGatherIdx.ptr, c->hGatherIdx.ptr, nGather * sizeof(long long), hipMemcpyHostToDevice, c->stream));
        const unsigned grid = (unsigned)std::min<size_t>((nGather * kNumParams + 255) / 256, (size_t)1 << 16);
        hipLaunchKernelGGL(klatt_gather_frames, dim3(grid), dim3(256), 0, c->stream, frames, c->dGatherIdx.ptr, (long long)nGather, c->dGatherRows.ptr);
        HIP_TRY(hipGetLastError());
        HIP_TRY(hipMemcpyAsync(c->hGatherRows.ptr, c->dGatherRows.ptr, nGather * kNumParams * sizeof(double), hipMemcpyDeviceToHost, c->stream));
    }
    HIP_TRY(hipStreamSynchronize(c->stream));
    {
        std::lock_guard<std::mutex> lg(c->logMu);
        if (c->logSent == c->logTail) c->logSent = c->logTail = 0;
    }
    for (size_t j = 0; j < nGather; ++j) memcpy(fill[j].s->overflow[fill[j].at].p, c->hGatherRows.ptr + j * kNumParams, kNumParams * sizeof(double));
    return 0;
}

static int queue_frames(const QueueCall& q)
{
    std::vector<Stream*> ss, order;
    if (queue_check(q, ss, order)) return -1;
    if (q.n == 0 || q.frameStart[q.n] == 0) return 0;
    for (Stream* s : order) s->mu.lock();
    const int rc = q.onDevice ? queue_device(q, ss.data()) : queue_host(q, ss.data());
    for (Stream* s : order) s->mu.unlock();
    return rc;
}

int speechPlayer_queueFramesMany(const speechPlayer_handle_t* handles, int nHandles, const long long* frameStart, const speechPlayer_frame_t* frames,
                                 const unsigned int* minFrameDuration, const unsigned int* fadeDuration, const int* userIndex,
                                 const unsigned char* isNull, const unsigned char* purge)
{
    begin_call();
    QueueCall q;
    q.what = "speechPlayer_queueFramesMany"; q.handles = handles; q.n = nHandles; q.frameStart = frameStart; q.frames = frames;
    q.minDur = minFrameDuration; q.fadeDur = fadeDuration; q.userIndex = userIndex; q.isNull = isNull; q.purge = purge;
    return queue_frames(q);
}

int speechPlayer_queueFramesManyDevice(const speechPlayer_handle_t* handles, int nHandles, const long long* frameStart,
                                       const speechPlayer_frame_t* deviceFrames, const unsigned int* minFrameDuration,
                                       const unsigned int* fadeDuration, const int* userIndex, const unsigned char* isNull,
                                       const unsigned char* purge, void* readyStream)
{
    begin_call();
    QueueCall q;
    q.what = "speechPlayer_queueFramesManyDevice"; q.handles = handles; q.n = nHandles; q.frameStart = frameStart; q.frames = deviceFrames;
    q.onDevice = true; q.minDur = minFrameDuration; q.fadeDur = fadeDuration; q.userIndex = userIndex; q.isNull = isNull; q.purge = purge;
    q.readyStream = static_cast<hipStream_t>(readyStream);
    return queue_frames(q);
}

int speechPlayer_handleDevice(speechPlayer_handle_t handle)
{
    begin_call();
    Stream* s = lookup(handle);
    if (!s) { set_error("speechPlayer_handleDevice: invalid handle"); return -1; }
    return s->device;
}

speechPlayer_batch_t speechPlayer_batch_create(int sampleRate, int device)
{
    begin_call();
    int dev = pick_device(device);
    if (dev < 0) return nullptr;
    Batch* b = new Batch;
    b->sampleRate = sampleRate;
    b->device = dev;
    { hipDeviceProp_t prop; if (hipGetDeviceProperties(&prop, dev) == hipSuccess && prop.multiProcessorCount > 0) b->cus = prop.multiProcessorCount; }
    bool ok = hipSetDevice(dev) == hipSuccess && hipStreamCreateWithFlags(&b->stream, hipStreamNonBlocking) == hipSuccess &&
              hipEventCreateWithFlags(&b->forkEvent, hipEventDisableTiming) == hipSuccess &&
              hipStreamCreateWithFlags(&b->copyStream, hipStreamNonBlocking) == hipSuccess &&
              hipEventCreateWithFlags(&b->denseReady, hipEventDisableTiming) == hipSuccess &&
              hipEventCreateWithFlags(&b->copyDone, hipEventDisableTiming) == hipSuccess &&
              hipEventCreateWithFlags(&b->inputReady, hipEventDisableTiming) == hipSuccess &&
              hipEventCreateWithFlags(&b->pcmReady, hipEventDisableTiming) == hipSuccess;
    for (auto& s : b->exportSlot) ok = ok && hipEventCreateWithFlags(&s.done, hipEventDisableTiming) == hipSuccess;
    for (auto& s : b->trackSlot) ok = ok && hipEventCreateWithFlags(&s.done, hipEventDisableTiming) == hipSuccess;
    for (hipEvent_t* e : {&b->setDone, &b->setCopied, &b->timelineReady, &b->pitchOrder.done, &b->sourceOrder.done}) ok = ok && hipEventCreateWithFlags(e, hipEventDisableTiming) == hipSuccess;
    { const char* e = getenv("SPEECHPLAYER_TRACKS"); if (e) b->tracks = atoi(e) ? 1 : 0; }
    { const char* e = getenv("SPEECHPLAYER_DIRECT"); if (e) b->direct = std::min(2, std::max(0, atoi(e))); }
    { const char* e = getenv("SPEECHPLAYER_DIRECT_LEAN"); if (e) b->directLean = std::min(1, std::max(-1, atoi(e))); }
    for (int i = 0; i < 6 && ok; ++i)
        ok = hipStreamCreateWithFlags(&b->side[i], hipStreamNonBlocking) == hipSuccess &&
             hipEventCreateWithFlags(&b->join[i], hipEventDisableTiming) == hipSuccess;
    { const char* e = getenv("SPEECHPLAYER_QUIET_LAST"); if (e) b->quietLast = atoi(e) ? 1 : 0; }
    if (!ok) {
        set_error("cannot create a stream on device %d", dev);
        speechPlayer_batch_destroy(b);
        return nullptr;
    }
    return b;
}

void speechPlayer_batch_destroy(speechPlayer_batch_t batch)
{
    Batch* b = static_cast<Batch*>(batch);
    if (!b) return;
    (void)hipSetDevice(b->device);
    (void)sync_exports(b);
    for (auto& s : b->exportSlot) {
        if (s.done) (void)hipEventDestroy(s.done);
        s.host.release(); s.dev.release();
    }
    (void)settle_track_exports(b, true);
    for (auto& s : b->trackSlot) {
        if (s.done) (void)hipEventDestroy(s.done);
        s.host.release(); s.dev.release();
    }
    for (hipEvent_t e : {b->setDone, b->setCopied, b->timelineReady, b->pitchOrder.done, b->sourceOrder.done}) if (e) (void)hipEventDestroy(e);
    b->dListStart.release(); b->dTimeline.release(); b->dPitch.release(); b->dLabels.release(); b->dUnitFirst.release();
    b->dSource.release(); b->dEpochs.release(); b->dEpochCount.release();
    if (b->inputReady) (void)hipEventDestroy(b->inputReady);
    if (b->pcmReady) (void)hipEventDestroy(b->pcmReady);
    b->dShapeIdx.release(); b->dShapeRows.release();
    if (b->stream) { (void)hipStreamSynchronize(b->stream); (void)hipStreamDestroy(b->stream); }
    for (int i = 0; i < 6; ++i) {
        if (b->side[i]) { (void)hipStreamSynchronize(b->side[i]); (void)hipStreamDestroy(b->side[i]); }
        if (b->join[i]) (void)hipEventDestroy(b->join[i]);
    }
    if (b->forkEvent) (void)hipEventDestroy(b->forkEvent);
    if (b->copyStream) { (void)hipStreamSynchronize(b->copyStream); (void)hipStreamDestroy(b->copyStream); }
    if (b->denseReady) (void)hipEventDestroy(b->denseReady);
    if (b->copyDone) (void)hipEventDestroy(b->copyDone);
    b->dDense.release(); b->dDenseStart.release(); b->dFacts.release(); b->hFacts.release();
    b->dRecords.release(); b->dShapeTable.release(); b->dRep.release(); b->dMismatch.release();
    b->dFrames.release(); b->dMeta.release(); b->dUtt.release(); b->dOrder.release(); b->dPcm.release(); b->dResult.release();
    b->dFloat.release(); b->dDebug.release(); b->dDigest.release(); b->bounce.release();
    b->dFlatRef.release(); b->dSourceRef.release(); b->dJobs.release(); b->dShapes.release(); b->dTrack.release();
    b->dDirectJobs.release(); b->dDirectFirst.release(); b->dDirectHdr.release(); b->dDirectRec.release();
    delete b;
}

int speechPlayer_batch_setOption(speechPlayer_batch_t batch, const char* name, int value)
{
    begin_call();
    Batch* b = static_cast<Batch*>(batch);
    if (!b || !name) return -1;
    if (!strcmp(name, "mode")) {
        if (value != MODE_EXACT && value != MODE_FAST) { set_error("mode %d not available", value); return -1; }
        b->mode = value;
        return 0;
    }
    if (!strcmp(name, "sort")) { b->sortByLength = value ? 1 : 0; return 0; }
    if (!strcmp(name, "quiet_last")) { b->quietLast = value ? 1 : 0; return 0; }
    if (!strcmp(name, "layout")) { b->layout = value < 0 ? -1 : (value > 2 ? 1 : value); return 0; }
    if (!strcmp(name, "tracks")) { b->tracks = value ? 1 : 0; return 0; }
    if (!strcmp(name, "track_budget_mb")) { b->trackBudgetMB = value < 0 ? 0 : value; return 0; }
    if (!strcmp(name, "direct")) { b->direct = value < 0 ? 0 : (value > 2 ? 2 : value); return 0; }
    if (!strcmp(name, "direct_lean")) { b->directLean = value < 0 ? -1 : (value ? 1 : 0); return 0; }
    if (!strcmp(name, "pitch_table_mb")) { b->pitchBudgetMB = value < 1 ? 1 : value; return 0; }
    if (!strcmp(name, "source_table_mb")) { b->sourceBudgetMB = value < 1 ? 1 : value; return 0; }
    if (!strcmp(name, "source_lane_lists")) { b->sourceLaneLists = value < 1 ? 1 : value; return 0; }
    set_error("unknown option %s", name);
    return -1;
}

struct SetInput {
    long long nLists = 0;
    const long long* listStart = nullptr;
    const speechPlayer_frame_t* frames = nullptr;
    const unsigned int* minDur = nullptr;
    const unsigned int* fadeDur = nullptr;
    const int* userIndex = nullptr;
    const unsigned char* isNull = nullptr;
    const speechPlayer_frameRecord_t* records = nullptr;
    long long nShapes = 0;
    const speechPlayer_frame_t* shapes = nullptr;
    long long nUtt = 0;
    const unsigned int* listOf = nullptr;
    const unsigned int* seeds = nullptr;
    const double* deviceFrames = nullptr;
    hipStream_t readyStream = nullptr;
    const speechPlayer_frameLabel_t* labels = nullptr;
    bool noTracks = false;
};
static_assert(sizeof(speechPlayer_frameRecord_t) == sizeof(FrameRecord), "record layout");
static_assert(sizeof(speechPlayer_frameLabel_t) == sizeof(FrameLabel), "label layout");
static_assert(SPEECHPLAYER_LABEL_GAP == kLabelGap && SPEECHPLAYER_LABEL_PUFF == kLabelPuff && SPEECHPLAYER_ALIGN_COLUMNS == kAlignColumns &&
              SPEECHPLAYER_UNIT_COLUMNS == kUnitColumns, "alignment constants");

static void batch_clear(Batch* b)
{
    b->nUtt = 0; b->nFrames = 0; b->nFramesSpoken = 0; b->nLists = 0; b->nSlots = 0; b->nQuiet = 0; b->nNoNasal = 0; b->nNoNasalUtt = 0; b->totalSamples = 0; b->poolSamples = 0;
    b->nTracked = 0; b->nTrackedUtt = 0; b->nJobs = 0; b->trackEntries = 0; b->nDirect = 0; b->nDirectUtt = 0; b->nDirectFrames = 0;
    b->lens.clear(); b->outStart.assign(1, 0); b->results.clear(); b->resultsFresh = false; b->floatFresh = false;
    b->uttFrameStart.clear(); b->uttFrames.clear(); b->uttList.clear(); b->uttSeed.clear(); b->timelineFresh = false; b->epochFresh = false;
    b->hasLabels = false; b->listUnits.clear();
}

static int batch_set(Batch* b, const SetInput& in);

static int batch_set_guarded(const char* what, speechPlayer_batch_t batch, const SetInput& in)
{
    begin_call();
    try {
        return batch_set(static_cast<Batch*>(batch), in);
    } catch (const std::exception& e) {
        set_error("%s: %s", what, e.what());
        return -1;
    }
}

int speechPlayer_batch_setUtterances(speechPlayer_batch_t batch, long long nUtterances, const long long* frameStart,
                                     const speechPlayer_frame_t* frames, const unsigned int* minFrameDuration,
                                     const unsigned int* fadeDuration, const int* userIndex, const unsigned char* isNull,
                                     const unsigned int* noiseSeed)
{
    SetInput in;
    in.nLists = nUtterances; in.listStart = frameStart; in.frames = frames; in.minDur = minFrameDuration; in.fadeDur = fadeDuration;
    in.userIndex = userIndex; in.isNull = isNull; in.nUtt = nUtterances; in.seeds = noiseSeed;
    return batch_set_guarded("setUtterances", batch, in);
}

static bool device_range(const void* p, size_t bytes, int device, size_t align, const char* what)
{
    hipPointerAttribute_t a;
    if (hipPointerGetAttributes(&a, p) != hipSuccess) {
        (void)hipGetLastError();
        set_error("%s: %p is not memory the HIP runtime knows (host memory?)", what, p);
        return false;
    }
    if (a.type != hipMemoryTypeDevice) { set_error("%s: %p is not device memory (memory type %d)", what, p, (int)a.type); return false; }
    if (a.device != device) { set_error("%s: %p is memory of device %d, the batch's is %d", what, p, a.device, device); return false; }
    if (reinterpret_cast<uintptr_t>(p) % align) { set_error("%s: %p is not %zu-byte aligned", what, p, align); return false; }
    hipDeviceptr_t base = nullptr;
    size_t size = 0;
    if (hipMemGetAddressRange(&base, &size, const_cast<void*>(p)) != hipSuccess) {
        (void)hipGetLastError();
        set_error("%s: the allocation that holds %p is unknown to the HIP runtime", what, p);
        return false;
    }
    if ((size_t)(static_cast<const char*>(p) - static_cast<const char*>(base)) + bytes > size) {
        set_error("%s: %zu bytes from %p run past the end of their allocation (%zu bytes from %p)", what, bytes, p, size, base);
        return false;
    }
    return true;
}

int speechPlayer_batch_setUtterancesDevice(speechPlayer_batch_t batch, long long nUtterances, const long long* frameStart,
                                           const speechPlayer_frame_t* deviceFrames, const unsigned int* minFrameDuration,
                                           const unsigned int* fadeDuration, const int* userIndex, const unsigned char* isNull,
                                           const unsigned int* noiseSeed, void* readyStream)
{
    begin_call();
    Batch* b = static_cast<Batch*>(batch);
    if (!b || nUtterances < 0 || !frameStart) { set_error("setUtterancesDevice: bad arguments"); return -1; }
    if (hipSetDevice(b->device) != hipSuccess) { set_error_code(SPEECHPLAYER_ERR_HIP); set_error("setUtterancesDevice: cannot select device %d", b->device); return -1; }
    const long long nF = frameStart[nUtterances];
    if (nF < 0 || nF > (1ll << 48)) { set_error("setUtterancesDevice: frameStart[%lld] = %lld", nUtterances, nF); return -1; }
    if (nF > 0 && !deviceFrames) { set_error("setUtterancesDevice: no frames"); return -1; }
    if (nF > 0 && !device_range(deviceFrames, (size_t)nF * sizeof(speechPlayer_frame_t), b->device, 8, "setUtterancesDevice")) return -1;
    SetInput in;
    in.nLists = nUtterances; in.listStart = frameStart; in.minDur = minFrameDuration; in.fadeDur = fadeDuration;
    in.userIndex = userIndex; in.isNull = isNull; in.nUtt = nUtterances; in.seeds = noiseSeed;
    in.deviceFrames = reinterpret_cast<const double*>(deviceFrames); in.readyStream = static_cast<hipStream_t>(readyStream);
    return batch_set_guarded("setUtterancesDevice", batch, in);
}

int speechPlayer_batch_setUtterancesShared(speechPlayer_batch_t batch, long long nLists, const long long* listStart,
                                           const speechPlayer_frame_t* frames, const unsigned int* minFrameDuration, const unsigned int* fadeDuration,
                                           const int* userIndex, const unsigned char* isNull, long long nUtterances, const unsigned int* listOf,
                                           const unsigned int* noiseSeed)
{
    SetInput in;
    in.nLists = nLists; in.listStart = listStart; in.frames = frames; in.minDur = minFrameDuration; in.fadeDur = fadeDuration;
    in.userIndex = userIndex; in.isNull = isNull; in.nUtt = nUtterances; in.listOf = listOf; in.seeds = noiseSeed;
    return batch_set_guarded("setUtterancesShared", batch, in);
}

int speechPlayer_batch_setRecords(speechPlayer_batch_t batch, long long nShapes, const speechPlayer_frame_t* shapes,
                                  long long nLists, const long long* listStart, const speechPlayer_frameRecord_t* records,
                                  long long nUtterances, const unsigned int* listOf, const unsigned int* noiseSeed)
{
    SetInput in;
    in.nLists = nLists; in.listStart = listStart; in.records = records; in.nShapes = nShapes; in.shapes = shapes;
    in.nUtt = nUtterances; in.listOf = listOf; in.seeds = noiseSeed;
    if (nShapes < 0 || (nShapes > 0 && !shapes)) { begin_call(); set_error("setRecords: bad shape table"); return -1; }
    if (!records && nLists > 0 && listStart && listStart[nLists] > 0) { begin_call(); set_error("setRecords: no records"); return -1; }
    static const speechPlayer_frameRecord_t none = {0.0, 0.0, SPEECHPLAYER_RECORD_SILENCE, 0u, 0u, -1};
    if (!in.records) in.records = &none;
    return batch_set_guarded("setRecords", batch, in);
}

int speechPlayer_batch_setRecordsLabelled(speechPlayer_batch_t batch, long long nShapes, const speechPlayer_frame_t* shapes,
                                          long long nLists, const long long* listStart, const speechPlayer_frameRecord_t* records,
                                          const speechPlayer_frameLabel_t* labels, long long nUtterances, const unsigned int* listOf,
                                          const unsigned int* noiseSeed)
{
    if (!labels) return speechPlayer_batch_setRecords(batch, nShapes, shapes, nLists, listStart, records, nUtterances, listOf, noiseSeed);
    SetInput in;
    in.nLists = nLists; in.listStart = listStart; in.records = records; in.nShapes = nShapes; in.shapes = shapes;
    in.nUtt = nUtterances; in.listOf = listOf; in.seeds = noiseSeed; in.labels = labels;
    if (nShapes < 0 || (nShapes > 0 && !shapes)) { begin_call(); set_error("setRecordsLabelled: bad shape table"); return -1; }
    if (!records && nLists > 0 && listStart && listStart[nLists] > 0) { begin_call(); set_error("setRecordsLabelled: no records"); return -1; }
    static const speechPlayer_frameRecord_t none = {0.0, 0.0, SPEECHPLAYER_RECORD_SILENCE, 0u, 0u, -1};
    if (!in.records) in.records = &none;
// ... 755 lines not shown
        while (u < b->nUtt) {
            const long long s0 = b->outStart[u], e0 = s0 + b->results[u].produced;
            if (s0 >= c1) break;
            const long long lo = std::max(s0, c0), hi = std::min(e0, c1);
            if (hi > lo) memcpy(dst + dstStart[u] + (lo - s0), src + (lo - c0), (size_t)(hi - lo) * sizeof(int16_t));
            if (e0 > c1) break;
            ++u;
        }
    }
    return pos;
}

long long speechPlayer_batch_readAll(speechPlayer_batch_t batch, sample* sampleBuf, long long capacity, long long* outStart)
{
    begin_call();
    if (refuse_timing_only("speechPlayer_batch_readAll")) return -1;
    Batch* b = static_cast<Batch*>(batch);
    if (!b || !sampleBuf) return -1;
    HIP_TRY(hipSetDevice(b->device));
    HIP_TRY(hipStreamSynchronize(b->stream));
    if (fetch_results(b)) return -1;
    bool whole = true;
    for (long long u = 0; u < b->nUtt && whole; ++u) whole = b->results[u].produced == b->lens[u];
    if (!whole) return read_all_padded(b, sampleBuf, capacity, outStart);
    const long long total = b->totalSamples;
    if (total > capacity) { set_error("readAll: capacity %lld too small for %lld samples", capacity, total); return -1; }
    if (outStart) memcpy(outStart, b->denseStart.data(), sizeof(long long) * ((size_t)b->nUtt + 1));
    if (total == 0) return 0;
    if (dense_prepare(b)) return -1;
    HIP_TRY(hipStreamWaitEvent(b->copyStream, b->denseReady, 0));
    if (is_pinned(sampleBuf)) {
        HIP_TRY(hipMemcpyAsync(sampleBuf, b->dDense.ptr, (size_t)total * sizeof(int16_t), hipMemcpyDeviceToHost, b->copyStream));
        HIP_TRY(hipStreamSynchronize(b->copyStream));
        return total;
    }
    constexpr long long kPiece = 16ll << 20;
    if (b->bounce.ensure((size_t)kPiece * sizeof(int16_t))) return -1;
    const long long nPieces = (total + kPiece - 1) / kPiece;
    auto issue = [&](long long k) -> int {
        const long long off = k * kPiece, n = std::min(kPiece, total - off);
        HIP_TRY(hipMemcpyAsync(b->bounce.buf[k & 1], b->dDense.ptr + off, (size_t)n * sizeof(int16_t), hipMemcpyDeviceToHost, b->copyStream));
        HIP_TRY(hipEventRecord(b->bounce.ev[k & 1], b->copyStream));
        return 0;
    };
    if (issue(0)) return -1;
    int16_t* const dst = reinterpret_cast<int16_t*>(sampleBuf);
    for (long long k = 0; k < nPieces; ++k) {
        HIP_TRY(hipEventSynchronize(b->bounce.ev[k & 1]));
        const long long off = k * kPiece, n = std::min(kPiece, total - off);
        if (k + 1 < nPieces && issue(k + 1)) return -1;
        const int16_t* const src = static_cast<const int16_t*>(b->bounce.buf[k & 1]);
        parallel_ranges(n, 1 << 21, [&](long long a, long long e) { memcpy(dst + off + a, src + a, (size_t)(e - a) * sizeof(int16_t)); });
    }
    return total;
}

long long speechPlayer_batch_readAllAsync(speechPlayer_batch_t batch, sample* sampleBuf, long long capacity, long long* outStart)
{
    begin_call();
    if (refuse_timing_only("speechPlayer_batch_readAllAsync")) return -1;
    Batch* b = static_cast<Batch*>(batch);
    if (!b || !sampleBuf) return -1;
    HIP_TRY(hipSetDevice(b->device));
    if (!is_pinned(sampleBuf)) { set_error("readAllAsync: the buffer is not page-locked (speechPlayer_hostAlloc)"); return -1; }
    if (!b->launched && b->nUtt > 0) { set_error("readAllAsync: the batch has not been synthesised since it was set"); return -1; }
    const long long total = b->totalSamples;
    if (total > capacity) { set_error("readAllAsync: capacity %lld too small for %lld samples", capacity, total); return -1; }
    if (outStart) memcpy(outStart, b->denseStart.data(), sizeof(long long) * ((size_t)b->nUtt + 1));
    if (total == 0) return 0;
    if (dense_prepare(b)) return -1;
    HIP_TRY(hipStreamWaitEvent(b->copyStream, b->denseReady, 0));
    HIP_TRY(hipMemcpyAsync(sampleBuf, b->dDense.ptr, (size_t)total * sizeof(int16_t), hipMemcpyDeviceToHost, b->copyStream));
    HIP_TRY(hipEventRecord(b->copyDone, b->copyStream));
    b->copyPending = true;
    return total;
}

int speechPlayer_batch_readWait(speechPlayer_batch_t batch)
{
    begin_call();
    Batch* b = static_cast<Batch*>(batch);
    if (!b) return -1;
    HIP_TRY(hipSetDevice(b->device));
    if (b->copyPending) { HIP_TRY(hipEventSynchronize(b->copyDone)); b->copyPending = false; }
    return 0;
}

void* speechPlayer_hostAlloc(long long bytes)
{
    begin_call();
    if (bytes <= 0) return nullptr;
    void* p = nullptr;
    if (hipHostMalloc(&p, (size_t)bytes, hipHostMallocDefault) != hipSuccess) {
        (void)hipGetLastError();
        set_error_code(SPEECHPLAYER_ERR_HIP);
        set_error("hostAlloc: cannot page-lock %lld bytes", bytes);
        return nullptr;
    }
    return p;
}
void speechPlayer_hostFree(void* p)
{
    if (p) (void)hipHostFree(p);
}

long long speechPlayer_batch_readFloat(speechPlayer_batch_t batch, long long u, float* sampleBuf, long long capacity)
{
    begin_call();
    if (refuse_timing_only("speechPlayer_batch_readFloat")) return -1;
    Batch* b = static_cast<Batch*>(batch);
    if (!b || u < 0 || u >= b->nUtt || !sampleBuf) return -1;
    HIP_TRY(hipSetDevice(b->device));
    if (!b->floatFresh) {
        if (b->dFloat.reserve(std::max<size_t>(b->poolSamples, 8))) return -1;
        const long long n8 = b->poolSamples / 8;
        if (n8 > 0) {
            const unsigned grid = (unsigned)std::min<long long>((n8 + 255) / 256, 2048);
            hipLaunchKernelGGL(pcm_to_float, dim3(grid), dim3(256), 0, b->stream, b->dPcm.ptr, b->dFloat.ptr, n8);
            HIP_TRY(hipGetLastError());
        }
        b->floatFresh = true;
    }
    HIP_TRY(hipStreamSynchronize(b->stream));
    if (fetch_results(b)) return -1;
    long long n = std::min<long long>(b->results[u].produced, capacity);
    if (n > 0) HIP_TRY(hipMemcpy(sampleBuf, b->dFloat.ptr + b->outStart[u], (size_t)n * sizeof(float), hipMemcpyDeviceToHost));
    return n;
}

int speechPlayer_batch_digest(speechPlayer_batch_t batch, unsigned long long* perUtterance, unsigned long long* whole)
{
    begin_call();
    Batch* b = static_cast<Batch*>(batch);
    if (!b) { set_error("digest: no batch"); return -1; }
    HIP_TRY(hipSetDevice(b->device));
    std::vector<unsigned long long> host((size_t)b->nUtt);
    if (b->nUtt) {
        if (b->dDigest.reserve((size_t)b->nUtt)) return -1;
        const unsigned grid = (unsigned)std::min<long long>((b->nUtt + 3) / 4, 16384);
        hipLaunchKernelGGL(pcm_digest, dim3(grid), dim3(256), 0, b->stream, b->dPcm.ptr, b->dUtt.ptr, b->dResult.ptr, b->dDigest.ptr, b->nUtt);
        HIP_TRY(hipGetLastError());
        HIP_TRY(hipMemcpyAsync(host.data(), b->dDigest.ptr, (size_t)b->nUtt * sizeof(unsigned long long), hipMemcpyDeviceToHost, b->stream));
        HIP_TRY(hipStreamSynchronize(b->stream));
    }
    if (perUtterance && b->nUtt) memcpy(perUtterance, host.data(), (size_t)b->nUtt * sizeof(unsigned long long));
    if (whole) {
        unsigned long long acc = 0;
        for (long long u = 0; u < b->nUtt; ++u) acc += digest_mix((unsigned long long)u, 0u) ^ host[u] * 0x9E3779B97F4A7C15ull;
        *whole = acc;
    }
    return 0;
}

int speechPlayer_batch_getLastIndex(speechPlayer_batch_t batch, long long u)
{
    begin_call();
    Batch* b = static_cast<Batch*>(batch);
    if (!b || u < 0 || u >= b->nUtt) return -1;
    if (hipSetDevice(b->device) != hipSuccess || hipStreamSynchronize(b->stream) != hipSuccess) return -1;
    if (fetch_results(b)) return -1;
    return b->results[u].lastIndex;
}

const sample* speechPlayer_batch_devicePcm(speechPlayer_batch_t batch)
{
    Batch* b = static_cast<Batch*>(batch);
    return b ? reinterpret_cast<const sample*>(b->dPcm.ptr) : nullptr;
}

long long speechPlayer_batch_deviceOffset(speechPlayer_batch_t batch, long long u)
{
    Batch* b = static_cast<Batch*>(batch);
    if (!b || u < 0 || u > b->nUtt) return -1;
    return b->outStart[u];
}

int speechPlayer_batch_device(speechPlayer_batch_t batch)
{
    begin_call();
    Batch* b = static_cast<Batch*>(batch);
    if (!b) { set_error("batch_device: no batch"); return -1; }
    return b->device;
}

long long speechPlayer_batch_exportPcm(speechPlayer_batch_t batch, const long long* utterances, long long nUtterances, void* deviceOut,
                                       int format, long long rowStride, void* stream)
{
    begin_call();
    if (refuse_timing_only("speechPlayer_batch_exportPcm")) return -1;
    return batch_entry("exportPcm", batch, [&](Batch* b) -> long long {
        if (format != 0 && format != 1) { set_error("exportPcm: format %d (0 int16, 1 float32)", format); return -1; }
        if (rowStride < 0) { set_error("exportPcm: rowStride %lld", rowStride); return -1; }
        const bool packed = rowStride == 0;
        std::vector<ExportRow> rows;
        ExportSelection s;
        if (export_selection(b, "exportPcm", utterances, nUtterances, false, s, [&](long long, long long u, long long) {
                rows.push_back(ExportRow{b->outStart[(size_t)u], (long long)b->lens[(size_t)u]});
                return rows.back().len;
            })) return -1;
        const long long n = s.n, maxLen = s.most, total = s.total;
        std::vector<long long> words;
        const RowTable table = packed ? packed_row_table(s.counts.data(), 0, n, kExportChunkLog2, words) : RowTable{0, 0};
        if (!packed && rowStride < maxLen) { set_error("exportPcm: rowStride %lld is below the longest chosen utterance (%lld samples)", rowStride, maxLen); return -1; }
        if (!packed && n > (1ll << 50) / rowStride) { set_error("exportPcm: %lld rows of %lld elements", n, rowStride); return -1; }
        const long long elements = packed ? total : n * rowStride;
        if (elements == 0) return 0;
        if (!b->launched) { set_error("exportPcm: the batch has not been synthesised since it was set"); return -1; }
        const size_t elSize = format ? sizeof(float) : sizeof(int16_t);
        HIP_TRY(hipSetDevice(b->device));
        if (!deviceOut) { set_error("exportPcm: no output buffer"); return -1; }
        if (!device_range(deviceOut, (size_t)elements * elSize, b->device, elSize, "exportPcm")) return -1;
        hipStream_t st = static_cast<hipStream_t>(stream);
        Batch::ExportSlot& slot = b->exportSlot[b->exportNext++ % Batch::kExportSlots];
        if (slot.used) { HIP_TRY(hipEventSynchronize(slot.done)); slot.used = false; }
        StageBlock block;
        const int rowsAt = block.add(rows), wordsAt = block.add(words);
        if (slot.host.ensure(block.bytes()) || slot.dev.reserve(block.bytes())) return -1;
        block.copy_to(slot.host.ptr);
        HIP_TRY(hipMemcpyAsync(slot.dev.ptr, slot.host.ptr, block.bytes(), hipMemcpyHostToDevice, st));
        HIP_TRY(hipEventRecord(b->pcmReady, b->stream));
        HIP_TRY(hipStreamWaitEvent(st, b->pcmReady, 0));
        const ExportRow* dRows = block.device<ExportRow>(rowsAt, slot.dev.ptr);
        const long long* dDst = packed ? block.device<long long>(wordsAt, slot.dev.ptr) + table.startOff : nullptr;
        const long long* dChunk = packed ? block.device<long long>(wordsAt, slot.dev.ptr) + table.chunkOff : nullptr;
        const long long n8 = (elements + 7) / 8;
        const unsigned grid = (unsigned)std::min<long long>((n8 + 255) / 256, 8ll * b->cus);
        const int vec = reinterpret_cast<uintptr_t>(deviceOut) % 16 == 0;
        if (format) hipLaunchKernelGGL(pcm_export<true>, dim3(grid), dim3(256), 0, st, b->dPcm.ptr, deviceOut, dRows, dDst, dChunk, n, rowStride, elements, vec);
        else hipLaunchKernelGGL(pcm_export<false>, dim3(grid), dim3(256), 0, st, b->dPcm.ptr, deviceOut, dRows, dDst, dChunk, n, rowStride, elements, vec);
        HIP_TRY(hipGetLastError());
        HIP_TRY(hipEventRecord(slot.done, st));
        slot.used = true;
        return elements;
    });
}

int speechPlayer_batch_time(speechPlayer_batch_t batch, int launches, float* msPerLaunch)
{
    begin_call();
    Batch* b = static_cast<Batch*>(batch);
    if (!b || launches <= 0 || !msPerLaunch) return -1;
    HIP_TRY(hipSetDevice(b->device));
    struct Events {
        std::vector<hipEvent_t> v;
        ~Events() { for (auto e : v) if (e) (void)hipEventDestroy(e); }
    } events;
    events.v.assign((size_t)launches * 2, nullptr);
    std::vector<hipEvent_t>& ev = events.v;
    for (auto& e : ev) HIP_TRY(hipEventCreate(&e));
    int rc = 0;
    for (int i = 0; i < launches && !rc; ++i) {
        HIP_TRY(hipEventRecord(ev[2 * i], b->stream));
        rc = batch_launch(b);
        HIP_TRY(hipEventRecord(ev[2 * i + 1], b->stream));
    }
    HIP_TRY(hipStreamSynchronize(b->stream));
    for (int i = 0; i < launches && !rc; ++i) HIP_TRY(hipEventElapsedTime(&msPerLaunch[i], ev[2 * i], ev[2 * i + 1]));
    return rc;
}

struct Node {
    int sampleRate = 0;
    std::vector<Batch*> parts;
    std::vector<long long> bounds;
    int deal = 0;
    bool sorted = false;
    std::vector<std::vector<long long>> members;
    std::vector<int> shardOf;
    std::vector<long long> localOf;
    long long nUtt = 0;
};

speechPlayer_node_t speechPlayer_node_create(int sampleRate, int nDevices, const int* devices)
{
    begin_call();
    if (nDevices <= 0) { set_error("node_create: need at least one device"); return nullptr; }
    Node* n = new Node;
    n->sampleRate = sampleRate;
    for (int d = 0; d < nDevices; ++d) {
        Batch* b = static_cast<Batch*>(speechPlayer_batch_create(sampleRate, devices ? devices[d] : d));
        if (!b) { speechPlayer_node_destroy(n); return nullptr; }
        n->parts.push_back(b);
    }
    n->bounds.assign((size_t)nDevices + 1, 0);
    return n;
}

void speechPlayer_node_destroy(speechPlayer_node_t node)
{
    Node* n = static_cast<Node*>(node);
    if (!n) return;
    for (Batch* b : n->parts) speechPlayer_batch_destroy(b);
    delete n;
}

int speechPlayer_node_devices(speechPlayer_node_t node) { return node ? (int)static_cast<Node*>(node)->parts.size() : -1; }

speechPlayer_batch_t speechPlayer_node_part(speechPlayer_node_t node, int shard)
{
    Node* n = static_cast<Node*>(node);
    return (n && shard >= 0 && shard < (int)n->parts.size()) ? n->parts[shard] : nullptr;
}

int speechPlayer_node_setOption(speechPlayer_node_t node, const char* name, int value)
{
    begin_call();
// ... 1141 lines not shown
```

### nvspeechplayer_amd/csrc/klatt_systolic.h

```cpp
#pragma once

#include <type_traits>

#include "klatt_device.h"

namespace klatt {

#ifndef KLATT_UNROLL
#define KLATT_UNROLL 8
#endif
#ifndef KLATT_MINWAVES
#define KLATT_MINWAVES 1
#endif
#ifndef KLATT_PAIR
#define KLATT_PAIR 1
#endif
#ifndef KLATT_NOISY_RUNS
#define KLATT_NOISY_RUNS 0
#endif
#ifndef KLATT_FADE_TIGHT
#define KLATT_FADE_TIGHT 1
#endif
#ifndef KLATT_NOISY_TIGHT
#define KLATT_NOISY_TIGHT 1
#endif
#define KLATT_STR2(x) #x
#define KLATT_STR(x) KLATT_STR2(x)

#ifndef KLATT_FLAT_EXHAUSTIVE
#define KLATT_FLAT_EXHAUSTIVE 1
#endif
constexpr int kStages = 4;
#ifndef KLATT_FLAT_SOURCE
#define KLATT_FLAT_SOURCE 1
#endif

template <bool NOISE, int CH, bool FLAT = false, int SPLIT = 0>
struct SysLds {
    static constexpr int MOVED = SPLIT & 3;
    static constexpr bool NP0 = (SPLIT >> 2) != 0;
    static constexpr int kBufs = 2;
    static constexpr int kBufsX = 2;
    static constexpr int kBufBytes = CH * kLanes * (FLAT ? (int)sizeof(sig_t) : 8);
    static constexpr int kPipeBytes = kBufs * kBufBytes;
    static constexpr int kNumPipes = NOISE ? 4 : 3;
    static constexpr int kPipeO = kBufsX * kBufBytes;
    static constexpr int kTileOff = kPipeO + (kNumPipes - 1) * kPipeBytes;
    static constexpr int kRowBase = kTileOff + kLanes * kTileStride;
    static constexpr int kRowCount = kRowBase + kLanes * 8;
    static constexpr int kMaxLen = kRowCount + kLanes * 4;
    static constexpr int kSync = kMaxLen + 16;
    static constexpr int kFrames = kSync + 32;
    static constexpr int kParams0 = (FLAT && KLATT_FLAT_SOURCE) ? 0 : (NP0 ? 12 : 7), kParams1 = FLAT ? 0 : (NOISE ? (NP0 ? 0 : 5) + 2 * (3 + MOVED) : 7), kParams2 = FLAT ? 0 : (NOISE ? 14 - 2 * MOVED : 6), kParams3 = FLAT ? 0 : (NOISE ? 14 : 5);
    static constexpr int kFrames1 = kFrames + 1 * kParams0 * kLanes * 8;
    static constexpr int kFrames2 = kFrames1 + 2 * kParams1 * kLanes * 8;
    static constexpr int kFrames3 = kFrames2 + 2 * kParams2 * kLanes * 8;
    static constexpr int kBytes = kFrames3 + 2 * kParams3 * kLanes * 8;
};

template <int NPARAM, int NRES, bool NWREG = false>
struct StageFrame {
    double* oldL;
    double* nwL;
    double nwR[NWREG && NPARAM > 0 ? NPARAM : 1];
    __device__ __forceinline__ double getNew(int k) const { return NWREG ? nwR[k] : nwL[k * kLanes]; }
    __device__ __forceinline__ void setNew(int k, double v) { if (NWREG) nwR[k] = v; else nwL[k * kLanes] = v; }
    double cur[NPARAM > 0 ? NPARAM : 1];
    double ra[NRES > 0 ? NRES : 1], rb[NRES > 0 ? NRES : 1], rc[NRES > 0 ? NRES : 1];
    double z1[NRES > 0 ? NRES : 1], z2[NRES > 0 ? NRES : 1];
    double invFade;
    uint32_t cnt, oldMin, newMin, newFade, nextFrame, resMask, parMask, produced;
    bool hasNew, oldNull, newNull, done;
};

struct PitchState {
    double cur0, old0, new0, oldInc, newInc;
};

template <int NPARAM, int NRES, bool NWREG>
__device__ __forceinline__ void stage_frame_init(StageFrame<NPARAM, NRES, NWREG>& f, bool live, unsigned char* region, int lane)
{
    f.oldL = reinterpret_cast<double*>(region) + lane;
    f.nwL = f.oldL + NPARAM * kLanes;
#pragma unroll
    for (int k = 0; k < NPARAM; ++k) { f.oldL[k * kLanes] = 0.0; f.setNew(k, 0.0); f.cur[k] = 0.0; }
#pragma unroll
    for (int r = 0; r < NRES; ++r) { f.ra[r] = 0.0; f.rb[r] = 2.0; f.rc[r] = -1.0; f.z1[r] = 0.0; f.z2[r] = 0.0; }
    f.invFade = 1.0;
    f.cnt = 0; f.oldMin = 0; f.newMin = 0; f.newFade = 1; f.nextFrame = 0; f.resMask = 0; f.parMask = 0; f.produced = 0;
    f.hasNew = false; f.oldNull = true; f.newNull = false; f.done = !live;
}

template <int NPARAM_, int NRES_, int GAIN_, bool PITCH_, bool ANTI0_, bool INLINE_COEF_ = false>
struct StageDesc {
    static constexpr int NPARAM = NPARAM_, NRES = NRES_, GAIN = GAIN_;
    static constexpr bool PITCH = PITCH_, ANTI0 = ANTI0_, INLINE_COEF = INLINE_COEF_;
};

struct StageCtx {
    const KernelArgs& A;
    const UttDesc& d;
    const double* myFrames;
    const FrameMeta* myMeta;
    uint32_t ringOff, ringMask;
    const FlatRef* myFlat;
    const SourceRef* mySrc;
    bool lone = false;
    double* loneLds = nullptr;
};
constexpr int kLoneLdsPerStage = 12288;
#ifndef KLATT_STREAM_SPLIT
#define KLATT_STREAM_SPLIT 5
#endif
#ifndef KLATT_LONE_SPLIT
#define KLATT_LONE_SPLIT 7
#endif
__device__ constexpr int final_param(int moved, int k) { constexpr int L0[14] = {9, 17, 8, 16, 7, 15, 29, 35, 30, 36, 41, 42, 43, 45}; return L0[k + 2 * moved < 13 ? k + 2 * moved : 13]; }
__device__ constexpr int final_res(int moved, int r) { constexpr int G0[5] = {5, 6, 7, 12, 13}; return G0[r + moved < 4 ? r + moved : 4]; }
template <bool STREAM, int WPS, bool LONE> constexpr int stream_split() { return (STREAM && WPS == 1) ? (LONE ? KLATT_LONE_SPLIT : KLATT_STREAM_SPLIT) : 0; }
__device__ constexpr int head_param(bool nasal, int ncasc, int k)
{
    constexpr int N[4] = {13, 21, 14, 22}, C[12] = {12, 20, 11, 19, 10, 18, 9, 17, 8, 16, 7, 15};
    if (nasal && k < 4) return N[k];
    const int j = nasal ? k - 4 : k;
    return j < 2 * ncasc ? C[j] : 23;
}

template <int NBITS>
__device__ __forceinline__ uint32_t wave_or_bits(uint32_t m)
{
    uint32_t w = 0;
#pragma unroll
    for (int k = 0; k < NBITS; ++k) w |= __any(m & (1u << k)) ? (1u << k) : 0u;
    return w;
}

constexpr uint32_t kNanTarget = 0x80000000u;
template <class SF>
__device__ __forceinline__ bool nan_target_live(const SF& f) { return __any(!f.done && (f.parMask & kNanTarget) != 0u); }

template <class D, class SF>
__device__ __forceinline__ bool stage_event(SF& f, PitchState* ps, int32_t* lastIndex, const int* P, const int* RF, const int* RB,
                                            const StageCtx& X)
{
    if (f.hasNew) {
#pragma unroll
        for (int k = 0; k < D::NPARAM; ++k) f.oldL[k * kLanes] = f.getNew(k);
        f.oldMin = f.newMin; f.oldNull = f.newNull;
        if (D::PITCH) { ps->old0 = ps->new0; ps->oldInc = ps->newInc; }
        f.hasNew = false;
        return true;
    }
    if (f.nextFrame >= X.d.nFrames) { f.done = true; return false; }
    const uint32_t at = (X.ringOff + f.nextFrame) & X.ringMask;
    const FrameMeta m = X.myMeta[at];
    const double* g = X.myFrames + (size_t)at * kNumParams;
    f.nextFrame++;
    f.newMin = m.minSamples; f.newFade = m.fadeSamples; f.newNull = (m.flags & FRAME_NULL) != 0;
    constexpr int GI = D::GAIN >= 0 ? D::GAIN : 0;
    double pNew0 = 0.0, pNewInc = 0.0, pOld0 = D::PITCH ? ps->old0 : 0.0;
    if (f.newNull) {
#pragma unroll
        for (int k = 0; k < D::NPARAM; ++k) f.setNew(k, f.oldL[k * kLanes]);
        uint32_t pm = 0;
        if (D::GAIN >= 0) { pm = (f.oldL[GI * kLanes] != 0.0) ? (1u << GI) : 0u; f.setNew(GI, 0.0); }
        if (D::PITCH) { pNew0 = ps->cur0; pNewInc = 0.0; }
        f.resMask = 0; f.parMask = pm;
    } else {
        uint32_t pm = 0, mk = 0;
        if (f.oldNull) {
#pragma unroll
            for (int k = 0; k < D::NPARAM; ++k) { const double v = g[P[k]]; f.setNew(k, v); f.oldL[k * kLanes] = v; pm |= (v != v) ? kNanTarget : 0u; }
            if (D::GAIN >= 0) { pm = (pm & kNanTarget) | ((f.getNew(GI) != 0.0) ? (1u << GI) : 0u); f.oldL[GI * kLanes] = 0.0; }
        } else {
            bool moved[D::NPARAM > 0 ? D::NPARAM : 1];
#pragma unroll
            for (int k = 0; k < D::NPARAM; ++k) {
                const double v = g[P[k]];
                moved[k] = !(v == f.oldL[k * kLanes]);
                f.setNew(k, v);
                pm |= moved[k] ? (1u << k) : 0u;
                pm |= (v != v) ? kNanTarget : 0u;
            }
#pragma unroll
            for (int r = 0; r < D::NRES; ++r) mk |= (moved[RF[r]] || moved[RB[r]]) ? (1u << r) : 0u;
        }
        if (D::PITCH) {
            const double g0 = g[0], g46 = g[46];
            pNew0 = g0;
            pNewInc = (g46 - g0) / (double)f.newMin;
            if (f.oldNull) pOld0 = g0;
        }
        f.resMask = mk; f.parMask = pm;
    }
    if (D::PITCH) { ps->new0 = pNew0; ps->newInc = pNewInc; ps->old0 = pOld0; }
    if (lastIndex && m.userIndex != -1) *lastIndex = m.userIndex;
    f.cnt = 0;
    if (D::PITCH) {
        ps->new0 += ps->newInc * (double)f.newFade;
        f.parMask |= (ps->new0 != ps->new0) ? kNanTarget : 0u;
    }
    f.invFade = 1.0 / (double)f.newFade;
    f.hasNew = true;
    return true;
}

constexpr uint32_t kCoefAllUnknown = 0xAAAAAAAAu;
template <class D, class SF>
__device__ __forceinline__ uint32_t fade_classes(const SF& f, const KernelArgs& A, const int* RF, const int* RB, uint32_t wRes)
{
    uint32_t bits = kCoefAllUnknown;
    if (!D::INLINE_COEF) return bits;
#pragma unroll
    for (int r = 0; r < D::NRES; ++r) {
        if (!(wRes & (1u << r))) continue;
        const double xo = A.negPiOverSr * f.oldL[RB[r] * kLanes] * kLog2e, xn = A.negPiOverSr * f.getNew(RB[r]) * kLog2e;
        const double to = A.twoPiOverSr * -f.oldL[RF[r] * kLanes] * kTwoOverPi, tn = A.twoPiOverSr * -f.getNew(RF[r]) * kTwoOverPi;
        const bool eu = __builtin_fabs(xo) <= 0.499 && __builtin_fabs(xn) <= 0.499;
        const bool c0 = __builtin_fabs(to) <= 0.499 && __builtin_fabs(tn) <= 0.499;
        const bool c1 = to <= -0.501 && to >= -1.499 && tn <= -0.501 && tn >= -1.499;
        const uint32_t cls = __all(f.done || (eu && c0)) ? COEF_UNREDUCED : (__all(f.done || (eu && c1)) ? COEF_QUADRANT_M1 : COEF_UNKNOWN);
        bits = (bits & ~(3u << (2 * r))) | (cls << (2 * r));
    }
    return bits;
}

__device__ __forceinline__ double lane_read(double v, int srcLane)
{
    const unsigned long long w = (unsigned long long)__double_as_longlong(v);
    const uint32_t lo = (uint32_t)__builtin_amdgcn_readlane((int)(uint32_t)w, srcLane), hi = (uint32_t)__builtin_amdgcn_readlane((int)(uint32_t)(w >> 32), srcLane);
    return __longlong_as_double((long long)(((unsigned long long)hi << 32) | lo));
}

template <class D, int MODE, bool PLAIN = false, class SF>
__device__ __forceinline__ void stage_fade(SF& f, PitchState* ps, const KernelArgs& A, const int* RF, const int* RB,
                                           bool lerp, uint32_t wRes, bool gainOnly = false, uint32_t coefCls = kCoefAllUnknown,
                                           const double* co = nullptr, const double* cn = nullptr)
{
    if (!D::PITCH && !lerp) return;
    const double ratio = div_by((double)f.cnt, (double)f.newFade, f.invFade);
    if (D::PITCH) ps->cur0 = fade_value(ps->old0, ps->new0, ratio);
    constexpr int GI = D::GAIN >= 0 ? D::GAIN : 0;
    if (D::GAIN >= 0 && lerp && gainOnly) {
        f.cur[GI] = fade_value(f.oldL[GI * kLanes], f.getNew(GI), ratio);
    } else if (lerp) {
        double o[D::NPARAM > 0 ? D::NPARAM : 1], n[D::NPARAM > 0 ? D::NPARAM : 1];
#pragma unroll
        for (int k = 0; k < D::NPARAM; ++k) { o[k] = co ? co[k] : f.oldL[k * kLanes]; n[k] = cn ? cn[k] : f.getNew(k); }
#pragma unroll
        for (int k = 0; k < D::NPARAM; ++k) f.cur[k] = PLAIN ? o[k] + ((n[k] - o[k]) * ratio) : fade_value(o[k], n[k], ratio);
    }
#pragma unroll
    for (int r = 0; r < D::NRES; ++r) {
        if (wRes & (1u << r)) {
            const Coef k = D::INLINE_COEF
                ? resonator_coefficients_inline<MODE>(f.cur[RF[r]], f.cur[RB[r]], D::ANTI0 && r == 0, A.negPiOverSr, A.twoPiOverSr,
                                                      (int)((coefCls >> (2 * r)) & 3u))
                : resonator_coefficients<MODE>(f.cur[RF[r]], f.cur[RB[r]], D::ANTI0 && r == 0, A.negPiOverSr, A.twoPiOverSr);
            f.ra[r] = k.a; f.rb[r] = k.b; f.rc[r] = k.c;
        }
    }
// ... 447 lines not shown
                        if (hold) { delay--; f.done = true; }
                        const bool emit = stage_advance<D, MODE>(f, ps, lastIndex, P, RF, RB, X);
                        if (hold) f.done = wasDone;
                        gen(c, i, emit);
                    } else if (K::CACHE) {
                        if (!cached) {
#pragma unroll
                            for (int k = 0; k < D::NPARAM; ++k) { co[k] = f.oldL[k * kLanes]; cn[k] = f.getNew(k); }
                            cached = true;
                        }
                        bool anyEvent = false;
                        const bool emit = stage_advance<D, MODE>(f, ps, lastIndex, P, RF, RB, X, co, cn, &anyEvent);
                        if (anyEvent) cached = false;
                        gen(c, i, emit);
                    } else {
                        const bool emit = stage_advance<D, MODE>(f, ps, lastIndex, P, RF, RB, X);
                        if (K::LONE) loneValid = false;
                        gen(c, i, emit);
                    }
                    ++i;
                }
            }
            perChunk();
        }
        STAMP_WORKED();
        STAGE_SYNC();
        STAMP_SYNCED();
    }
#ifdef KLATT_STAMPS
    if (X.A.debug && (threadIdx.x & (kLanes - 1)) == 0) {
        unsigned long long* o = X.A.debug + (blockIdx.x * 4 + stampSlot) * 8;
        o[0] = st.work; o[1] = st.wait; o[2] = st.n[0]; o[3] = st.n[1]; o[4] = st.n[2]; o[5] = st.c[0]; o[6] = st.c[1]; o[7] = st.c[2];
    }
#endif
    (void)stampSlot;
}

template <int STAGE_, int NRES_, int NGAIN_, bool ANTI0_, uint32_t USUAL_ = 0, uint32_t USUAL2_ = 0, class R_ = sig_t>
struct FlatDesc {
    using R = R_;
    static constexpr int STAGE = STAGE_;
    static constexpr int NRES = NRES_, NGAIN = NGAIN_, NE = NRES_ + NGAIN_;
    static constexpr bool ANTI0 = ANTI0_;
    static constexpr uint32_t USUAL = USUAL_, USUAL2 = USUAL2_;
};

struct BarrierSync {
    __device__ __forceinline__ void begin(int) const {}
    __device__ __forceinline__ void end(int) const { __syncthreads(); }
    __device__ __forceinline__ void idle() const { __syncthreads(); }
};

#ifndef KLATT_MIX_UNROLL
#define KLATT_MIX_UNROLL 4
#endif
template <int E> using KindTag = std::integral_constant<int, E>;
typedef unsigned int flat_u4 __attribute__((ext_vector_type(4)));
typedef unsigned int flat_u2 __attribute__((ext_vector_type(2)));
typedef double flat_d2 __attribute__((ext_vector_type(2)));
template <class FD>
struct FlatState2 {
    static constexpr int NR = FD::NRES > 0 ? FD::NRES : 1;
    using R = typename FD::R;
    R ra[NR], rb[NR], rc[NR], z1[NR], z2[NR];
    R cur[2 * FD::NGAIN > 0 ? 2 * FD::NGAIN : 1];
    uint32_t idx[FD::NE], stride[FD::NE];
    uint32_t startAt, left, next, nFrames, length, produced;
    FlatRef nextRef;
    uint32_t wmask;
    bool live;
};
template <class R> struct ResPre { R a, p1, p2; };
template <class T> __device__ __forceinline__ void flat_pin(T v) { asm volatile("" :: "v"(v) : "memory"); }
template <class R> __device__ __forceinline__ void flat_pin(const ResPre<R>& q) { asm volatile("" :: "v"(q.a), "v"(q.p1), "v"(q.p2) : "memory"); }
template <int NE>
__device__ __forceinline__ uint32_t flat2_wave_kinds(uint32_t flags, bool live, const int* GE)
{
    const uint32_t mine = live ? (flags >> kUttKindShift) : 0u;
    uint32_t w = 0;
#pragma unroll
    for (int e = 0; e < NE; ++e) w |= __any((mine >> GE[e]) & 1u) ? (1u << e) : 0u;
    return w;
}
template <class FD>
__device__ __forceinline__ void flat2_init(FlatState2<FD>& f, bool live, const UttDesc& d, const StageCtx& X, const int* GE)
{
#pragma unroll
    for (int r = 0; r < FD::NRES; ++r) { f.ra[r] = 0; f.rb[r] = 2; f.rc[r] = -1; f.z1[r] = 0; f.z2[r] = 0; }
#pragma unroll
    for (int k = 0; k < 2 * FD::NGAIN; ++k) f.cur[k] = 0;
#pragma unroll
    for (int e = 0; e < FD::NE; ++e) { f.idx[e] = 0; f.stride[e] = 0; }
    f.live = live && d.length > 0u;
    f.nFrames = d.nFrames; f.length = d.length; f.next = 0; f.left = 0; f.produced = 0;
    const bool any = live && d.nFrames > 0u;
    f.startAt = any ? 1u : 0xFFFFFFFFu;
    f.nextRef = FlatRef{0u, 0u, 1u, 0u};
    if (any) f.nextRef = X.myFlat[0];
    f.wmask = (uint32_t)__builtin_amdgcn_readfirstlane((int)flat2_wave_kinds<FD::NE>(d.flags, live, GE));
}
template <class FD>
__device__ __forceinline__ void flat2_switch(FlatState2<FD>& f, const StageCtx& X, const int* GE)
{
    const FlatRef p = f.nextRef;
    const uint32_t part = p.off + track_part(p.mask, p.fadeSamples, FD::STAGE);
    const uint32_t nMove = track_stage_slots(p.mask, FD::STAGE), hdr = track_stage_entries(FD::STAGE) - nMove;
    uint32_t moving = 0, still = 0;
#pragma unroll
    for (int e = 0; e < FD::NE; ++e) {
        const bool moves = (p.mask >> GE[e]) & 1u;
        f.idx[e] = (part + (moves ? hdr + moving : still)) * 16u;
        f.stride[e] = moves ? nMove * 16u : 0u;
        const uint32_t w = GE[e] == 0 ? 2u : 1u;
        moving += moves ? w : 0u; still += moves ? 0u : w;
    }
    f.left = nMove ? p.fadeSamples : 1u;
    f.next++;
    const bool more = f.next < f.nFrames;
    f.startAt = more ? f.startAt + p.span : 0xFFFFFFFFu;
#pragma unroll
    for (int e = 0; e < FD::NE; ++e) { flat_pin(f.idx[e]); flat_pin(f.stride[e]); }
    flat_pin(f.left); flat_pin(f.startAt);
    f.nextRef = X.myFlat[more ? f.next : f.nFrames - 1u];
}
template <class FD, uint32_t SET, bool ALLROWS = false>
struct FlatMid {
    FlatState2<FD>& f;
    __amdgpu_buffer_rsrc_t rsrc;
    bool has;
    template <class... T>
    __device__ __forceinline__ void operator()(T... firstHalf) const
    {
        using R = typename FD::R;
        (flat_pin(firstHalf), ...);
        if (ALLROWS || has) {
#pragma unroll
            for (int e = 0; e < FD::NE; ++e) {
                if (!(SET & (1u << e))) continue;
                const uint32_t off = f.idx[e];
                const flat_d2 v = __builtin_bit_cast(flat_d2, __builtin_amdgcn_raw_buffer_load_b128(rsrc, off, 0, 0));
                if (e < FD::NRES) {
                    f.rb[e < FD::NRES ? e : 0] = (R)v.x; f.rc[e < FD::NRES ? e : 0] = (R)v.y;
                    if (FD::ANTI0 && e == 0) f.ra[0] = (R)__builtin_bit_cast(double, __builtin_amdgcn_raw_buffer_load_b64(rsrc, off + 16u, 0, 0));
                } else {
                    const int g = e < FD::NRES ? 0 : e - FD::NRES;
                    f.cur[2 * g] = (R)v.x; f.cur[2 * g + 1] = (R)v.y;
                }
                f.idx[e] = off + f.stride[e];
            }
        }
    }
};
struct NoMid { template <class... T> __device__ __forceinline__ void operator()(T...) const {} };
template <int MODE, bool DERIVE, class R>
__device__ __forceinline__ ResPre<R> res_pre(R ra, R rb, R rc, R z1, R z2)
{
    ResPre<R> p;
    p.a = DERIVE ? (R)((R)1 - rb - rc) : ra;
    if (MODE == MODE_FAST || !std::is_same<R, double>::value) { p.p1 = rb; p.p2 = rc; }
    else { p.p1 = rb * z1; p.p2 = rc * z2; }
    return p;
}
template <int MODE, class R>
__device__ __forceinline__ R res_post(const ResPre<R>& p, R in, R& z1, R& z2)
{
    R y;
    if (MODE == MODE_FAST || !std::is_same<R, double>::value) y = dot3<MODE>(p.a, in, p.p1, z1, p.p2, z2);
    else y = p.a * in + p.p1 + p.p2;
    z2 = z1; z1 = y;
    return y;
}

template <class FD, int CH, class FBody, class FChunk, class FSync = BarrierSync>
__device__ __forceinline__ void flat2_loop(int depth, int nIter, int nChunks, int stampSlot, FlatState2<FD>& f, const StageCtx& X, const int* GE, FBody body, FChunk perChunk,
                                           const FSync& sync = FSync{})
{
#ifdef KLATT_STAMPS
    Stamps st;
#endif
    using R = typename FD::R;
    uint32_t staleG = 0;
    const __amdgpu_buffer_rsrc_t rsrc = __builtin_amdgcn_make_buffer_rsrc(const_cast<double2*>(X.A.track), 0, (int)X.A.trackBytes, 0x00020000);
    for (int iter = 0; iter < nIter; ++iter) {
        STAMP_BEGIN();
        STAMP_IDLE();
        const int c = iter - depth;
        const bool inRange = c >= 0 && c < nChunks;
        if (inRange) {
            sync.begin(c);
            const uint32_t t0 = (uint32_t)c * (uint32_t)CH, t1 = t0 + (uint32_t)CH;
            if (f.length <= t0) f.live = false;
            const bool busy = f.left > 0u || f.startAt <= t1;
            if (!__any(busy)) {
                if (staleG) {
#pragma unroll
                    for (int r = (FD::ANTI0 ? 1 : 0); r < FD::NRES; ++r)
                        if (staleG & (1u << r)) f.ra[r] = (R)((R)1 - f.rb[r] - f.rc[r]);
                    staleG = 0;
                }
                uint32_t run = f.live ? (f.startAt - t0 - 1u) / (uint32_t)CH : 0xFFFFFFFFu;
#pragma unroll
                for (int m = 32; m >= 1; m >>= 1) { const uint32_t o = (uint32_t)__shfl_xor((int)run, m, kLanes); run = o < run ? o : run; }
                run = (uint32_t)__builtin_amdgcn_readfirstlane((int)run);
                const uint32_t room = (uint32_t)(nChunks - c);
                run = run < room ? run : room;
                run = run < 1u ? 1u : run;
                int cc = c;
                STAMP_KIND(0);
                for (uint32_t q = 1; q < run; ++q) {
                    if (f.live) {
#pragma unroll
                        for (int i = 0; i < CH; ++i) body(cc, i, std::integral_constant<uint32_t, 0u>{}, NoMid{});
                    }
                    { const uint32_t e1 = (uint32_t)(cc + 1) * (uint32_t)CH; f.produced = f.length < e1 ? f.length : e1; }
                    perChunk();
                    STAMP_WORKED();
                    sync.end(cc);
                    STAMP_SYNCED();
                    STAMP_BEGIN();
                    ++iter; ++cc;
                    sync.begin(cc);
                }
                if (f.live) {
#pragma unroll
                    for (int i = 0; i < CH; ++i) body(cc, i, std::integral_constant<uint32_t, 0u>{}, NoMid{});
                }
                { const uint32_t e1 = (uint32_t)(cc + 1) * (uint32_t)CH; f.produced = f.length < e1 ? f.length : e1; }
                perChunk();
                STAMP_WORKED();
                sync.end(cc);
                STAMP_SYNCED();
                continue;
            }
            STAMP_KIND(-1);
            auto mixedChunk = [&](auto setTag, auto allRowsTag) __attribute__((always_inline)) {
                constexpr uint32_t SET = decltype(setTag)::value;
                constexpr bool ALLROWS = decltype(allRowsTag)::value;
                const uint32_t fix = staleG & ~SET;
                if (fix) {
#pragma unroll
                    for (int r = (FD::ANTI0 ? 1 : 0); r < FD::NRES; ++r)
                        if (fix & (1u << r)) f.ra[r] = (R)((R)1 - f.rb[r] - f.rc[r]);
                    staleG &= SET;
                }
                staleG |= SET;
#pragma unroll KLATT_MIX_UNROLL
                for (int i = 0; i < CH; ++i) {
                    if (!ALLROWS) {
                        const uint32_t tn = t0 + (uint32_t)i + 1u;
                        if (tn == f.startAt) flat2_switch<FD>(f, X, GE);
                    }
                    const bool has = ALLROWS || f.left > 0u;
                    body(c, i, setTag, FlatMid<FD, SET, ALLROWS>{f, rsrc, has});
                    if (!ALLROWS && has) f.left--;
                }
                if (ALLROWS) f.left = f.left > (uint32_t)CH ? f.left - (uint32_t)CH : 0u;
            };
            constexpr uint32_t ALL = (1u << FD::NE) - 1u;
            const bool usual = FD::USUAL != 0u && FD::USUAL != ALL && c != 0 && (f.wmask & ~FD::USUAL) == 0u;
            const bool allRows = usual && __all(!f.live || (f.left >= (uint32_t)CH && f.startAt > t1));
            if (allRows) mixedChunk(std::integral_constant<uint32_t, FD::USUAL>{}, std::true_type{});
            else if (usual) mixedChunk(std::integral_constant<uint32_t, FD::USUAL>{}, std::false_type{});
            else mixedChunk(std::integral_constant<uint32_t, ALL>{}, std::false_type{});
            f.produced = f.length < t1 ? f.length : t1;
            perChunk();
        }
        STAMP_WORKED();
        if (inRange) sync.end(c); else sync.idle();
        STAMP_SYNCED();
    }
#ifdef KLATT_STAMPS
    if (X.A.debug && (threadIdx.x & (kLanes - 1)) == 0) {
        unsigned long long* o = X.A.debug + (blockIdx.x * 4 + stampSlot) * 8;
        o[0] = st.work; o[1] = st.wait; o[2] = st.n[0]; o[3] = st.n[1]; o[4] = st.n[2]; o[5] = st.c[0]; o[6] = st.c[1]; o[7] = st.c[2];
    }
#endif
    (void)stampSlot;
}

template <int MODE, bool NOISE, int CH, int WPS = KLATT_MINWAVES, bool NASAL = true, bool STREAM = false, bool FLAT = false, bool LONE = false>
__global__ void __launch_bounds__(kLanes * kStages, WPS) klatt_systolic(const KernelArgs A)
{
    static_assert(!LONE || STREAM, "LONE: a live handle pulled alone");
    static_assert(NASAL || !NOISE, "only quiet launches have a nasal-free instantiation");
    static_assert(NOISE || !STREAM, "live handles take the noisy instantiation");
    static_assert(!FLAT || (NOISE && !STREAM), "tracks: noisy batch launches");
    constexpr int SPLIT = stream_split<STREAM, WPS, LONE>();
    constexpr int MOVED = SPLIT & 3;
    using L = SysLds<NOISE, CH, FLAT, SPLIT>;
    static_assert(SPLIT != 3, "eight resonators in the head stage: not built");
    constexpr int kChunk = CH;
    extern __shared__ __attribute__((aligned(16))) unsigned char lds[];
    using PipeT = typename std::conditional<FLAT, sig_t, double>::type;
    PipeT* const pipeX = reinterpret_cast<PipeT*>(lds);
    PipeT* const pipeO = reinterpret_cast<PipeT*>(lds + L::kPipeO);
    PipeT* const pipeA = reinterpret_cast<PipeT*>(lds + L::kPipeO + L::kPipeBytes);
    PipeT* const pipeB = reinterpret_cast<PipeT*>(lds + L::kPipeO + (NOISE ? 2 : 1) * L::kPipeBytes);
    constexpr int nbuf_pipeX = L::kBufsX, nbuf_pipeO = L::kBufs, nbuf_pipeA = L::kBufs, nbuf_pipeB = L::kBufs;
    (void)nbuf_pipeX; (void)nbuf_pipeO; (void)nbuf_pipeA; (void)nbuf_pipeB;
    unsigned char* const tile = lds + L::kTileOff;
    long long* const rowBase = reinterpret_cast<long long*>(lds + L::kRowBase);
    uint32_t* const rowCount = reinterpret_cast<uint32_t*>(lds + L::kRowCount);
    uint32_t* const maxLenP = reinterpret_cast<uint32_t*>(lds + L::kMaxLen);

    const int lane = threadIdx.x & (kLanes - 1);
    const int wave = __builtin_amdgcn_readfirstlane(threadIdx.x >> 6);
    const long long slot = (long long)blockIdx.x * kLanes + lane;
    const uint32_t u = (slot < A.nSlots) ? A.order[slot] : 0xFFFFFFFFu;
    const bool live = (u != 0xFFFFFFFFu);

    UttDesc d;
    d.frameStart = 0; d.outStart = 0; d.nFrames = 0; d.seed = 0; d.flags = 0; d.length = 0;
    if (live) d = A.utt[u];
    const FrameWindow fw = frame_window(A, d);
    const StageCtx X{A, d, A.frames + fw.base * kNumParams, A.meta + fw.base, fw.off, fw.mask,
                     FLAT ? A.flatRef + d.frameStart : nullptr, FLAT ? A.sourceRef + d.frameStart : nullptr, LONE,
                     LONE ? reinterpret_cast<double*>(lds + L::kBytes + wave * kLoneLdsPerStage) : nullptr};
    const uint32_t nkey = noise_key(d.seed), ninc = noise_inc(d.seed), ninc2 = noise_inc2(ninc);
    constexpr int FINAL = NOISE ? 2 : 3;
#ifndef KLATT_PRELOAD
#define KLATT_PRELOAD 1
#endif
    constexpr bool kPre = !NOISE && KLATT_PRELOAD;

    uint32_t* const stageMaskP = maxLenP + 1;
    uint32_t* const syncP = reinterpret_cast<uint32_t*>(lds + L::kSync);
    if (threadIdx.x == 0) { *maxLenP = 0; *stageMaskP = 0; }
    if (threadIdx.x < 8) syncP[threadIdx.x] = 0;
    __syncthreads();
    int cand = wave;
    if (KLATT_PAIR && WPS == 2 && (NOISE || !NASAL)) {
        const uint32_t hw = __builtin_amdgcn_s_getreg((4 << 0) | (0 << 6) | (31 << 11));
        cand = (int)((((hw >> 4) & 3u) + ((hw & 1u) ? 2u : 0u)) & 3u);
    }
    if (wave == 0) atomicMax(maxLenP, d.length);
    if (lane == 0) atomicOr(stageMaskP, 1u << cand);
    __syncthreads();
    const int stage = __builtin_amdgcn_readfirstlane((*stageMaskP == 0xFu) ? cand : wave);
    if (stage == FINAL) { rowBase[lane] = d.outStart; rowCount[lane] = 0; }
    const uint32_t maxLen = *maxLenP;
    const int nChunks = (int)((maxLen + kChunk - 1) / kChunk);
    const int nIter = nChunks + (NOISE ? 2 : 3);
    const int fullChunks = STREAM ? (int)(A.maxSamples / (uint32_t)kChunk) : nChunks;
    double* const streamState = (STREAM && live) ? (A.statePtrs ? A.statePtrs[u] : A.state + (size_t)u * kStateDoubles) : nullptr;
    const bool streamPurge = STREAM && live && A.control && (A.control[u] & 1u);
#define PIPE(p, c, i) (p)[(((nbuf_##p) == 2 ? ((c) & 1) : ((c) % (nbuf_##p))) * kChunk + (i)) * kLanes + lane]
    using KSrc = LoopKnobs<false, (!NOISE || KLATT_NOISY_RUNS), false, STREAM, NOISE, KLATT_UNROLL, LONE, (STREAM && WPS == 1 && !LONE)>;
    using KFil = LoopKnobs<kPre, (!NOISE || KLATT_NOISY_RUNS), false, STREAM, NOISE, KLATT_UNROLL, LONE, (STREAM && WPS == 1 && !LONE)>;
    uint32_t noDelay = 0;
    auto never = [&]() __attribute__((always_inline)) { return false; };
    auto noBegin = [&](int) __attribute__((always_inline)) { return false; };
    auto noAlt = [&](int) __attribute__((always_inline)) {};
    auto noAltSample = [&](int, int, double) __attribute__((always_inline)) {};
    auto noFadeAlt = [&](int, bool, bool) __attribute__((always_inline)) { return false; };
    auto nothing = [&](int) __attribute__((always_inline)) {};
    auto noChunk = [&]() __attribute__((always_inline)) {};

    auto make_sync = [&](auto, auto, auto, int, int, int) __attribute__((always_inline)) { return BarrierSync{}; };
    using I0 = std::integral_constant<int, 0>; using I1 = std::integral_constant<int, 1>; using I2 = std::integral_constant<int, 2>;
    if (FLAT && KLATT_FLAT_SOURCE && stage == 0) {
        if constexpr (FLAT) {
#if KLATT_FLAT_LAYOUT == 2
            using FD = FlatDesc<0, 2, 5, true, 0, 0, double>;
            constexpr int GE[7] = {0, 1, 14, 20, 21, 22, 23};
            constexpr int CB = 2;
            constexpr uint32_t kUsualS0 = 0x67u, kAllS0 = 0x7Fu, kVibBit = 8u;
            constexpr bool kHead = true;
#else
            using FD = FlatDesc<0, 0, 4, false, 0, 0, double>;
            constexpr int GE[4] = {20, 21, 22, 23};
            constexpr int CB = 0;
            constexpr uint32_t kUsualS0 = 0xCu, kAllS0 = 0xFu, kVibBit = 1u;
            constexpr bool kHead = false;
#endif
            bool staleNP = false;
            FlatState2<FD> f;
            flat2_init<FD>(f, live, d, X, GE);
            PitchState ps;
            ps.cur0 = 0.0; ps.old0 = 0.0; ps.new0 = 0.0; ps.oldInc = 0.0; ps.newInc = 0.0;
            double pitchPhase = 0.0, vibPhase = 0.0, aspNoise = 0.0, invFade = 1.0, nfD = 1.0;
            uint32_t noiseSt = noise_first(nkey, ninc), cntF = 0, nfU = 0;
            uint32_t fadeEndAt = 0xFFFFFFFFu;
            int32_t lastIndex = -1;
            bool oldNull = true, newNull = false;
            SourceRef nextSrc{0.0, 0.0, 1.0, -1, 0u};
            if (live && d.nFrames > 0u) nextSrc = X.mySrc[0];
            auto source = [&](bool waveVib, auto setTag, const auto& mid) __attribute__((always_inline)) -> double {
                constexpr uint32_t SET = decltype(setTag)::value;
                double vib = 1.0;
                if (waveVib) {
                    const double vs = f.cur[CB + 1];
                    const double adv = frac_toward_zero(div_by(vs, A.sampleRateF, A.invSampleRate) + vibPhase);
                    vibPhase = (vs != 0.0) ? adv : vibPhase;
                    vib = (sin(vibPhase * 6.283185307179586) * 0.06 * f.cur[CB + 0]) + 1.0;
                }
                const double turbGain = f.cur[CB + 2], openQ = f.cur[CB + 3], voiceAmp = f.cur[CB + 4], aspAmp = f.cur[CB + 5], preGain = f.cur[CB + 6];
                pitchPhase = frac_toward_zero(div_by(ps.cur0 * vib, A.sampleRateF, A.invSampleRate) + pitchPhase);
                double voice = (pitchPhase * 2.0) - 1.0;
                aspNoise = noise_uniform(noiseSt) + 0.75 * aspNoise;
                noiseSt = noise_step2(noiseSt, ninc2);
                double asp = aspNoise * 0.2;
                double turb = asp * turbGain;
                turb = (pitchPhase >= openQ) ? turb : turb * 0.01;
                voice += turb;
                voice *= voiceAmp;
                asp *= aspAmp;
                const double src = asp + voice;
                const double out = (src * preGain) * 0.5;
                if constexpr (kHead) {
                    const ResPre<double> q0 = res_pre<MODE, false>(f.ra[0], f.rb[0], f.rc[0], f.z1[0], f.z2[0]);
                    const ResPre<double> q1 = res_pre<MODE, ((SET >> 1) & 1u) != 0u>(f.ra[1], f.rb[1], f.rc[1], f.z1[1], f.z2[1]);
                    const double caNP = f.cur[0];
                    mid(out, q0, q1, caNP);
                    double zin = f.z1[0];
                    const double n0 = res_post<MODE>(q0, out, zin, f.z2[0]);
                    f.z1[0] = out;
                    const double np = res_post<MODE>(q1, n0, f.z1[1], f.z2[1]);
                    return fade_value(out, np, caNP);
                } else {
                    mid(out);
                    return out;
                }
            };
            auto vib_live = [&]() __attribute__((always_inline)) -> bool { return f.cur[CB + 0] != 0.0 || f.cur[CB + 1] != 0.0 || vibPhase != vibPhase; };
            const __amdgpu_buffer_rsrc_t rsrc = __builtin_amdgcn_make_buffer_rsrc(const_cast<double2*>(A.track), 0, (int)A.trackBytes, 0x00020000);
#ifdef KLATT_STAMPS
            Stamps st;
#endif
            const auto sync = make_sync(std::integral_constant<int, L::kBufsX>{}, I0{}, I1{}, 0, 0, 0);
            for (int iter = 0; iter < nIter; ++iter) {
                STAMP_BEGIN();
                STAMP_IDLE();
                const int c = iter;
                int lastChunk = -1;
                if (c < nChunks) {
                    sync.begin(c);
                    lastChunk = c;
                    const uint32_t t0 = (uint32_t)c * (uint32_t)CH, t1 = t0 + (uint32_t)CH;
                    if (f.length <= t0) f.live = false;
                    const bool busy = f.left > 0u || f.startAt <= t1 || cntF < nfU || fadeEndAt < t1 || vib_live();
                    STAMP_KIND(__any(busy) ? -1 : 0);
                    if (!__any(busy)) {
                        uint32_t run = f.live ? (f.startAt - t0 - 1u) / (uint32_t)CH : 0xFFFFFFFFu;
#pragma unroll
                        for (int m = 32; m >= 1; m >>= 1) { const uint32_t o = (uint32_t)__shfl_xor((int)run, m, kLanes); run = o < run ? o : run; }
                        run = (uint32_t)__builtin_amdgcn_readfirstlane((int)run);
                        const uint32_t room = (uint32_t)(nChunks - c);
                        run = run < room ? run : room;
                        run = run < 1u ? 1u : run;
                        int cc = c;
                        if (kHead && staleNP) { f.ra[1] = 1.0 - f.rb[1] - f.rc[1]; staleNP = false; }
                        for (uint32_t q = 0; q < run; ++q) {
                            if (f.live) {
#pragma unroll
                                for (int i = 0; i < CH; ++i) { ps.cur0 += ps.oldInc; PIPE(pipeX, cc, i) = source(false, std::integral_constant<uint32_t, 0u>{}, NoMid{}); }
                                ps.old0 = ps.cur0;
                            }
                            if (q + 1 < run) { STAMP_WORKED(); sync.end(cc); STAMP_SYNCED(); STAMP_BEGIN(); ++iter; ++cc; sync.begin(cc); lastChunk = cc; }
                        }
                    } else {
                        auto mixedChunk = [&](auto setTag, auto allFadeTag) __attribute__((always_inline)) {
                        constexpr uint32_t SET = decltype(setTag)::value;
                        constexpr bool ALLFADE = decltype(allFadeTag)::value;
                        const bool vibChunk = (SET & kVibBit) != 0u || __any(vib_live());
                        staleNP = true;
#pragma unroll KLATT_MIX_UNROLL
                        for (int i = 0; i < CH; ++i) {
                            const uint32_t t = t0 + (uint32_t)i;
                            const bool deq = !ALLFADE && t + 1u == f.startAt;
                            if (!ALLFADE && __any(deq)) {
                                if (deq) {
                                    const SourceRef m = nextSrc;
                                    const uint32_t nf = f.nextRef.fadeSamples;
                                    newNull = (m.flags & FRAME_NULL) != 0;
                                    ps.new0 = newNull ? ps.cur0 : m.pitch;
                                    ps.newInc = newNull ? 0.0 : m.pitchInc;
                                    if (!newNull && oldNull) ps.old0 = m.pitch;
                                    oldNull = newNull;
                                    if (m.userIndex != -1) lastIndex = m.userIndex;
                                    nfD = (double)nf; nfU = nf;
                                    ps.new0 += ps.newInc * nfD;
                                    invFade = m.invFade;
                                    cntF = 0;
                                    fadeEndAt = t + nf + 1u;
                                    flat_pin(ps.new0); flat_pin(ps.newInc); flat_pin(ps.old0); flat_pin(invFade); flat_pin(lastIndex); flat_pin(oldNull);
                                    flat2_switch<FD>(f, X, GE);
                                    nextSrc = X.mySrc[f.next < f.nFrames ? f.next : f.nFrames - 1u];
                                }
                            }
                            if (ALLFADE) {
                                cntF++;
                                ps.cur0 = fade_value(ps.old0, ps.new0, div_by((double)cntF, nfD, invFade));
                            } else {
                            const bool fad = !deq && cntF < nfU;
                            const bool ending = !deq && !fad && t == fadeEndAt;
                            const bool glide = !deq && !fad && !ending;
                            const uint32_t cn = cntF + 1u;
                            const double ratio = div_by((double)cn, nfD, invFade);
                            const double fv = fade_value(ps.old0, ps.new0, ratio);
                            const double gv = ps.cur0 + ps.oldInc;
                            ps.cur0 = fad ? fv : (glide ? gv : ps.cur0);
                            ps.old0 = ending ? ps.new0 : (glide ? gv : ps.old0);
                            ps.oldInc = ending ? ps.newInc : ps.oldInc;
                            cntF = fad ? cn : cntF;
                            fadeEndAt = ending ? 0xFFFFFFFFu : fadeEndAt;
                            }
                            const bool waveVib = vibChunk && __any(vib_live());
                            const bool has = f.left > 0u;
                            PIPE(pipeX, c, i) = source(waveVib, setTag, FlatMid<FD, SET>{f, rsrc, has});
                            if (has) f.left--;
                        }
                        };
                        const bool usual = c != 0 && (f.wmask & ~kUsualS0) == 0u;
                        const bool allFade = usual && !__any(vib_live()) && __all(!f.live || (cntF + (uint32_t)CH <= nfU && f.startAt > t1));
                        if (allFade) mixedChunk(std::integral_constant<uint32_t, kUsualS0>{}, std::true_type{});
                        else if (usual) mixedChunk(std::integral_constant<uint32_t, kUsualS0>{}, std::false_type{});
                        else mixedChunk(std::integral_constant<uint32_t, kAllS0>{}, std::false_type{});
                    }
                }
                STAMP_WORKED();
                if (lastChunk >= 0) sync.end(lastChunk); else sync.idle();
                STAMP_SYNCED();
            }
#ifdef KLATT_STAMPS
            if (A.debug && lane == 0) {
                unsigned long long* o = A.debug + (blockIdx.x * 4 + 0) * 8;
                o[0] = st.work; o[1] = st.wait; o[2] = st.n[0]; o[3] = st.n[1]; o[4] = st.n[2]; o[5] = st.c[0]; o[6] = st.c[1]; o[7] = st.c[2];
            }
#endif
            if (live) {
                UttResult res;
                res.produced = d.length; res.framesTaken = f.next; res.lastIndex = lastIndex; res.drained = 1u;
                A.result[u] = res;
            }
        }
    } else if (stage == 0) {
        constexpr bool NP0 = (SPLIT >> 2) != 0;
        using D = StageDesc<NP0 ? 12 : 7, NP0 ? 2 : 0, 6, true, NP0, NP0>;
        constexpr int P[12] = {1, 2, 3, 4, 5, 6, 44, 13, 21, 14, 22, 23};
        constexpr int RF[2] = {7, 9}, RB[2] = {8, 10};
        StageFrame<D::NPARAM, D::NRES, true> f;
        PitchState ps;
        stage_frame_init(f, live, lds + L::kFrames, lane);
        ps.cur0 = 0.0; ps.old0 = 0.0; ps.new0 = 0.0; ps.oldInc = 0.0; ps.newInc = 0.0;
        double pitchPhase = 0.0, vibPhase = 0.0, aspNoise = 0.0;
        uint32_t noiseSt = noise_first(nkey, ninc);
        int32_t lastIndex = -1;
        bool vibFrames = false;
        constexpr int GR0[2] = {0, 1};
        if (STREAM && live) {
            if (streamState[239] != 0.0) {
                pitchPhase = streamState[208]; vibPhase = streamState[209]; aspNoise = streamState[210];
                lastIndex = (int32_t)streamState[220]; noiseSt = (uint32_t)streamState[221];
            }
            stage_state_load<D>(f, &ps, streamState, P, RF, RB, GR0, streamPurge);
            vibFrames = f.oldL[0] != 0.0 || f.oldL[kLanes] != 0.0 || f.getNew(0) != 0.0 || f.getNew(1) != 0.0;
        }

        auto source = [&](bool waveVib) __attribute__((always_inline)) -> double {
            double vib = 1.0;
            if (waveVib) {
                const double vs = f.cur[1];
                const double adv = frac_toward_zero(div_by(vs, A.sampleRateF, A.invSampleRate) + vibPhase);
                vibPhase = (vs != 0.0) ? adv : vibPhase;
                vib = (sin(vibPhase * 6.283185307179586) * 0.06 * f.cur[0]) + 1.0;
            }
            pitchPhase = frac_toward_zero(div_by(ps.cur0 * vib, A.sampleRateF, A.invSampleRate) + pitchPhase);
            double voice = (pitchPhase * 2.0) - 1.0;
            double src;
            if (NOISE) {
                aspNoise = noise_uniform(noiseSt) + 0.75 * aspNoise;
                noiseSt = noise_step2(noiseSt, ninc2);
                double asp = aspNoise * 0.2;
                double turb = asp * f.cur[2];
                turb = (pitchPhase >= f.cur[3]) ? turb : turb * 0.01;
                voice += turb;
                voice *= f.cur[4];
                asp *= f.cur[5];
                src = asp + voice;
            } else {
                src = voice * f.cur[4];
            }
            const double x = (src * f.cur[6]) * 0.5;
            if (!NP0) return x;
            const double n0 = dot3<MODE>(f.ra[0], x, f.rb[0], f.z1[0], f.rc[0], f.z2[0]);
            f.z2[0] = f.z1[0]; f.z1[0] = x;
            const double np = resonate<MODE>(f.z1[NP0 ? 1 : 0], f.z2[NP0 ? 1 : 0], f.ra[NP0 ? 1 : 0], f.rb[NP0 ? 1 : 0], f.rc[NP0 ? 1 : 0], n0);
            return fade_value(x, np, f.cur[NP0 ? 11 : 0]);
        };
        auto vib_live_now = [&]() __attribute__((always_inline)) -> bool {
            return vibFrames || f.cur[0] != 0.0 || f.cur[1] != 0.0 || vibPhase != vibPhase;
        };
        stage_loop<D, MODE, CH, KSrc>(0, nIter, nChunks, fullChunks, stage, f, &ps, &lastIndex, noDelay, P, RF, RB, X,
            [&]() __attribute__((always_inline)) { return __any(!f.done && vib_live_now()); },
            [&](int kind) __attribute__((always_inline)) -> bool { return !NOISE && kind == 0 && !__any(!f.done && ps.oldInc != 0.0); },
            [&](int c) __attribute__((always_inline)) {
                ps.cur0 += ps.oldInc;
                const double inc = div_by(ps.cur0 * 1.0, A.sampleRateF, A.invSampleRate);
                double ph[kChunk];
#pragma unroll
                for (int i = 0; i < kChunk; ++i) { pitchPhase = frac_toward_zero(inc + pitchPhase); ph[i] = pitchPhase; }
#pragma unroll
                for (int i = 0; i < kChunk; ++i) PIPE(pipeX, c, i) = ((((ph[i] * 2.0) - 1.0) * f.cur[4]) * f.cur[6]) * 0.5;
            },
            noAltSample,
            [&](int, int) __attribute__((always_inline)) { return 0.0; },
            [&](int c, int i, bool steady, double) __attribute__((always_inline)) {
                if (steady) ps.cur0 += ps.oldInc;
                PIPE(pipeX, c, i) = source(false);
            },
            [&](int c, bool lerp, bool gainOnly) __attribute__((always_inline)) -> bool {
                if (NOISE || !gainOnly) return false;
                constexpr int GI = 6;
                const double g0 = lerp ? f.oldL[GI * kLanes] : f.cur[GI], g1 = lerp ? f.getNew(GI) : f.cur[GI];
                if (__any(g1 != g1 || ps.new0 != ps.new0)) return false;
                const double gd = g1 - g0, p0 = ps.old0, pd = ps.new0 - p0, nf = (double)f.newFade;
                if (!__any(pd != 0.0 || p0 != p0)) {
                    ps.cur0 = p0 + 0.0;
                    const double inc = div_by(ps.cur0 * 1.0, A.sampleRateF, A.invSampleRate);
#pragma unroll
                    for (int i = 0; i < kChunk; ++i) {
                        f.cnt++;
                        const double ratio = div_by((double)f.cnt, nf, f.invFade);
                        const double gain = g0 + (gd * ratio);
                        pitchPhase = frac_toward_zero(inc + pitchPhase);
                        PIPE(pipeX, c, i) = ((((pitchPhase * 2.0) - 1.0) * f.cur[4]) * gain) * 0.5;
                        if (i == kChunk - 1) f.cur[GI] = gain;
                    }
                } else {
#pragma unroll
                    for (int i = 0; i < kChunk; ++i) {
                        f.cnt++;
                        const double ratio = div_by((double)f.cnt, nf, f.invFade);
                        ps.cur0 = p0 + (pd * ratio);
                        const double gain = g0 + (gd * ratio);
                        pitchPhase = frac_toward_zero(div_by(ps.cur0 * 1.0, A.sampleRateF, A.invSampleRate) + pitchPhase);
                        PIPE(pipeX, c, i) = ((((pitchPhase * 2.0) - 1.0) * f.cur[4]) * gain) * 0.5;
                        if (i == kChunk - 1) f.cur[GI] = gain;
                    }
                }
                return true;
            },
            [&](int c, int i, bool emit) __attribute__((always_inline)) {
                if (emit && f.hasNew && f.cnt == 0)
                    vibFrames = f.oldL[0] != 0.0 || f.oldL[kLanes] != 0.0 || f.getNew(0) != 0.0 || f.getNew(1) != 0.0;
                const bool waveVib = __any(emit && vib_live_now());
                if (emit) { PIPE(pipeX, c, i) = source(waveVib); f.produced++; }
            },
            [&](int n) __attribute__((always_inline)) { ps.old0 = ps.cur0; f.produced += n; },
            [&](int n) __attribute__((always_inline)) { f.produced += n; },
            noChunk);
        if (live) {
            UttResult res;
            res.produced = f.produced; res.framesTaken = f.nextFrame; res.lastIndex = lastIndex; res.drained = STREAM ? (f.done ? 1u : 0u) : 1u;
            A.result[u] = res;
        }
        if (STREAM && live) {
            stage_state_save<D>(f, &ps, streamState, P, GR0);
            streamState[208] = pitchPhase; streamState[209] = vibPhase; streamState[210] = aspNoise;
            streamState[220] = (double)lastIndex; streamState[221] = (double)noiseSt;
        }
    } else if (FLAT && stage == 1) {
        if constexpr (FLAT) {
#if KLATT_FLAT_LAYOUT == 2
            using FD = FlatDesc<1, 6, 0, false, 0x38u>;
            constexpr int GE[6] = {2, 3, 4, 5, 6, 7};
            FlatState2<FD> f;
            flat2_init<FD>(f, live, d, X, GE);
            flat2_loop<FD, CH>(1, nIter, nChunks, stage, f, X, GE,
                [&](int c, int i, auto setTag, const auto& mid) __attribute__((always_inline)) {
                    constexpr uint32_t SET = decltype(setTag)::value;
                    ResPre<sig_t> q[6];
#pragma unroll
                    for (int r = 0; r < 6; ++r) q[r] = ((SET >> r) & 1u) ? res_pre<MODE, true>(f.ra[r], f.rb[r], f.rc[r], f.z1[r], f.z2[r])
                                                                         : res_pre<MODE, false>(f.ra[r], f.rb[r], f.rc[r], f.z1[r], f.z2[r]);
                    mid(q[0], q[1], q[2], q[3], q[4], q[5]);
                    sig_t o = PIPE(pipeX, c, i);
#pragma unroll
                    for (int r = 0; r < 6; ++r) o = res_post<MODE>(q[r], o, f.z1[r], f.z2[r]);
                    PIPE(pipeO, c, i) = o;
                },
                noChunk, make_sync(std::integral_constant<int, L::kBufs>{}, I1{}, I1{}, 0, 0, 2));
// ... 337 lines not shown
```

### nvspeechplayer_amd/speechPlayer.py

```python
import math
from ctypes import POINTER, Structure, byref, c_double, c_int, c_short, c_void_p, cast
from ctypes import c_longlong as ctypes_longlong

import numpy as np

from . import _native

speechPlayer_frameParam_t = c_double

FRAME_FIELDS = [
    'voicePitch',
    'vibratoPitchOffset',
    'vibratoSpeed',
    'voiceTurbulenceAmplitude',
    'glottalOpenQuotient',
    'voiceAmplitude',
    'aspirationAmplitude',
    'cf1', 'cf2', 'cf3', 'cf4', 'cf5', 'cf6', 'cfN0', 'cfNP',
    'cb1', 'cb2', 'cb3', 'cb4', 'cb5', 'cb6', 'cbN0', 'cbNP',
    'caNP',
    'fricationAmplitude',
    'pf1', 'pf2', 'pf3', 'pf4', 'pf5', 'pf6',
    'pb1', 'pb2', 'pb3', 'pb4', 'pb5', 'pb6',
    'pa1', 'pa2', 'pa3', 'pa4', 'pa5', 'pa6',
# ... 748 lines not shown
            return np.zeros(0, np.int64)
        counts = np.zeros(n, np.int64)
        self._check(self._dll.speechPlayer_batch_epochCounts(self._h, _ptr(sel), n, counts.ctypes.data))
        return counts[:n]

    def epochTensor(self, utterances=None, padded=True, pad=-1.0):
        import torch
        sel, n, _ = self._selection("epochTensor", utterances)

        def call(out, stride, numel, stream):
            return self._dll.speechPlayer_batch_exportEpochs(self._h, _ptr(sel), n, out, stride, float(pad), numel, stream)
        return self._export_rows(self.epochCounts(utterances), (len(EPOCH_COLUMNS),), torch.float64, padded, call)

    def setUtterancesShared(self, listStart, frames, minSamples, fadeSamples, listOf, userIndex=None, isNull=None, noiseSeed=None):
        ls = np.ascontiguousarray(listStart, dtype=np.int64)
        fr = np.ascontiguousarray(frames, dtype=np.float64).reshape(-1, 47)
        m = np.ascontiguousarray(minSamples, dtype=np.uint32)
        f = np.ascontiguousarray(fadeSamples, dtype=np.uint32)
        lo = np.ascontiguousarray(listOf, dtype=np.uint32)
        assert ls[-1] == len(fr) == len(m) == len(f)
        ix = None if userIndex is None else np.ascontiguousarray(userIndex, dtype=np.int32)
        nu = None if isNull is None else np.ascontiguousarray(isNull, dtype=np.uint8)
        sd = None if noiseSeed is None else np.ascontiguousarray(noiseSeed, dtype=np.uint32)
        p = lambda a: None if a is None else a.ctypes.data
        self._check(self._dll.speechPlayer_batch_setUtterancesShared(self._h, len(ls) - 1, p(ls), p(fr), p(m), p(f), p(ix), p(nu), len(lo), p(lo), p(sd)))
        self.nUtterances = len(lo)

    def setRecords(self, shapes, listStart, records, listOf=None, noiseSeed=None, labels=None):
        from .ipa import LABEL_DTYPE, RECORD_DTYPE
        sh = np.ascontiguousarray(shapes, dtype=np.float64).reshape(-1, 47)
        ls = np.ascontiguousarray(listStart, dtype=np.int64)
        rc = np.ascontiguousarray(records, dtype=RECORD_DTYPE)
        assert ls[-1] == len(rc)
        lo = None if listOf is None else np.ascontiguousarray(listOf, dtype=np.uint32)
        n_utt = len(ls) - 1 if lo is None else len(lo)
        sd = None if noiseSeed is None else np.ascontiguousarray(noiseSeed, dtype=np.uint32)
        p = lambda a: None if a is None else a.ctypes.data
        if labels is None:
            self._check(self._dll.speechPlayer_batch_setRecords(self._h, len(sh), p(sh), len(ls) - 1, p(ls), p(rc), n_utt, p(lo), p(sd)))
        else:
            lb = np.ascontiguousarray(labels, dtype=LABEL_DTYPE)
            if len(lb) != len(rc):
                raise ValueError("setRecords: %d labels for %d records" % (len(lb), len(rc)))
            lb = lb if len(lb) else np.zeros(1, LABEL_DTYPE)
            self._check(self._dll.speechPlayer_batch_setRecordsLabelled(self._h, len(sh), p(sh), len(ls) - 1, p(ls), p(rc), p(lb), n_utt, p(lo), p(sd)))
        self.nUtterances = n_utt

    def frames(self, u):
        n = self._check(self._dll.speechPlayer_batch_frames(self._h, u, None, None, None, None, None, 0))
        fr = np.zeros((n, 47)); m = np.zeros(n, np.uint32); f = np.zeros(n, np.uint32); ix = np.zeros(n, np.int32); nu = np.zeros(n, np.uint8)
        if n:
            self._check(self._dll.speechPlayer_batch_frames(self._h, u, fr.ctypes.data, m.ctypes.data, f.ctypes.data, ix.ctypes.data, nu.ctypes.data, n))
        return fr, m, f, ix, nu

    def setIpa(self, texts, speed=1, basePitch=100, inflection=0.5, clauseType=None, noiseSeed=None, voice=None,
               trailing_silence_ms=150.0, textOf=None):
        from .ipa import _text_pointers
        ptrs, n, keep = _text_pointers(texts, textOf)
        pitch = np.ascontiguousarray(np.broadcast_to(np.asarray(basePitch, dtype=np.float64), (n,)))
        code = lambda c: 0 if not c else ord(c[0])
        clauses = bytes([code(clauseType)]) * n if (clauseType is None or isinstance(clauseType, str)) else bytes(code(c) for c in clauseType)
        sd = None if noiseSeed is None else np.ascontiguousarray(noiseSeed, dtype=np.uint32)
        tail = -1.0 if trailing_silence_ms is None else float(trailing_silence_ms)
        if voice is None or isinstance(voice, str):
            self._check(self._dll.speechPlayer_batch_setIpa(self._h, n, ptrs.ctypes.data, float(speed), pitch.ctypes.data, float(inflection), clauses + b"\0",
                                                            None if not voice else voice.encode("utf8"), tail, None if sd is None else sd.ctypes.data))
        else:
            vo = np.ascontiguousarray(np.broadcast_to(np.asarray(voice, dtype=np.int32), (n,)))
            self._check(self._dll.speechPlayer_batch_setIpaVoices(self._h, n, ptrs.ctypes.data, float(speed), pitch.ctypes.data, float(inflection), clauses + b"\0",
                                                                  vo.ctypes.data, tail, None if sd is None else sd.ctypes.data))
        del keep
        self.nUtterances = n

    def setText(self, texts, speed=1, basePitch=100, inflection=0.5, noiseSeed=None, voice=None, espeakVoice="en"):
        import ctypes
        n = len(texts)
        enc = [t.encode("utf8") for t in texts]
        ptrs = (ctypes.c_char_p * max(n, 1))(*enc)
        pitch = np.ascontiguousarray(np.broadcast_to(np.asarray(basePitch, dtype=np.float64), (n,)))
        sd = None if noiseSeed is None else np.ascontiguousarray(noiseSeed, dtype=np.uint32)
        self._check(self._dll.speechPlayer_batch_setText(self._h, n, ptrs, None if not espeakVoice else espeakVoice.encode("utf8"), float(speed),
                                                         pitch.ctypes.data, float(inflection), None if not voice else voice.encode("utf8"),
                                                         None if sd is None else sd.ctypes.data))
        self.nUtterances = n

    @property
    def totalSamples(self):
        return self._dll.speechPlayer_batch_totalSamples(self._h)

    @property
    def totalFrames(self):
        return self._dll.speechPlayer_batch_totalFrames(self._h)

    def utteranceSamples(self, u):
        return self._dll.speechPlayer_batch_utteranceSamples(self._h, u)

    def synthesize(self, wait=True):
        self._check(self._dll.speechPlayer_batch_synthesize(self._h))
        if wait:
            self._check(self._dll.speechPlayer_batch_wait(self._h))

    def wait(self):
        self._check(self._dll.speechPlayer_batch_wait(self._h))

    def read(self, u):
        n = self.utteranceSamples(u)
        buf = np.zeros(max(n, 1), dtype=np.int16)
        got = self._check(self._dll.speechPlayer_batch_read(self._h, u, buf.ctypes.data, n))
        return buf[:got]

    def readFloat(self, u):
        n = self.utteranceSamples(u)
        buf = np.zeros(max(n, 1), dtype=np.float32)
        got = self._check(self._dll.speechPlayer_batch_readFloat(self._h, u, buf.ctypes.data, n))
        return buf[:got]

    def writeWav(self, u, path):
        import wave
        pcm = self.read(u)
        with wave.open(path, "wb") as w:
            w.setnchannels(1); w.setsampwidth(2); w.setframerate(self.sampleRate)
            w.writeframes(pcm.astype("<i2").tobytes())

    def readAll(self, out=None):
        total = self.totalSamples
        if out is not None:
            if out.dtype != np.int16 or not out.flags["C_CONTIGUOUS"] or out.size < total:
                raise ValueError("readAll: out must be a contiguous int16 array of at least %d samples" % total)
            buf = out
        else:
            buf = np.empty(max(total, 1), dtype=np.int16)
        starts = np.zeros(self.nUtterances + 1, dtype=np.int64)
        got = self._check(self._dll.speechPlayer_batch_readAll(self._h, buf.ctypes.data, total, starts.ctypes.data))
        return buf[:got], starts

    def readAllAsync(self, out):
        total = self.totalSamples
        if out.dtype != np.int16 or not out.flags["C_CONTIGUOUS"] or out.size < total:
            raise ValueError("readAllAsync: out must be a contiguous int16 array of at least %d samples" % total)
        starts = np.zeros(self.nUtterances + 1, dtype=np.int64)
        got = self._check(self._dll.speechPlayer_batch_readAllAsync(self._h, out.ctypes.data, out.size, starts.ctypes.data))
        return out[:got], starts

    def readWait(self):
        self._check(self._dll.speechPlayer_batch_readWait(self._h))

    def digest(self, per_utterance=False):
        import ctypes
        whole = ctypes.c_ulonglong(0)
        per = np.zeros(max(self.nUtterances, 1), dtype=np.uint64) if per_utterance else None
        self._check(self._dll.speechPlayer_batch_digest(self._h, None if per is None else per.ctypes.data, ctypes.byref(whole)))
        return (int(whole.value), per[:self.nUtterances]) if per_utterance else int(whole.value)

    def getLastIndex(self, u):
        return self._dll.speechPlayer_batch_getLastIndex(self._h, u)

    def time(self, launches):
        ms = np.zeros(launches, dtype=np.float32)
        self._check(self._dll.speechPlayer_batch_time(self._h, launches, ms.ctypes.data))
        return ms

    def kernelInfo(self):
        info = np.zeros(20, dtype=np.int32)
        self._check(self._dll.speechPlayer_batch_kernelInfo(self._h, info.ctypes.data, len(info)))
        return dict(vgprs=int(info[0]), lds_bytes=int(info[1]), wavefronts=int(info[2]), cus=int(info[3]),
                    workgroups_per_cu_by_lds=int(info[4]), scratch_bytes=int(info[5]),
                    stage_parallel_chunk=int(info[6]), noisy_group=bool(info[7]),
                    lane_pipelined=bool(info[8]), lane_pipelined_utterances=int(info[9]),
                    nasal_free=bool(info[10]), nasal_free_utterances=int(info[11]),
                    tracked_utterances=int(info[12]), tracks=int(info[13]), track_mbytes=int(info[14]), tracked=bool(info[15]),
                    direct_utterances=int(info[16]), direct=bool(info[17]), direct_mbytes=int(info[18]))

    def devicePcm(self):
        return self._dll.speechPlayer_batch_devicePcm(self._h)

    def deviceOffset(self, u):
        return self._dll.speechPlayer_batch_deviceOffset(self._h, u)

    def close(self):
        if getattr(self, "_h", None):
            self._dll.speechPlayer_batch_destroy(self._h)
            self._h = None

    def __del__(self):
        try:
            self.close()
        except Exception:
            pass


class NodePlayer(object):

    def __init__(self, sampleRate, devices, mode=0, layout=None):
        self.sampleRate = sampleRate
        self._dll = _native.load()
        dev = np.ascontiguousarray(devices, dtype=np.int32)
        self._h = self._dll.speechPlayer_node_create(sampleRate, len(dev), dev.ctypes.data)
        if not self._h:
            raise RuntimeError("speechPlayer_node_create failed: %s" % _native.last_error())
        self._check(self._dll.speechPlayer_node_setOption(self._h, b"mode", mode))
        if layout is not None:
            self._check(self._dll.speechPlayer_node_setOption(self._h, b"layout", layout))
        self.nUtterances = 0
        self._lens = None

    def _check(self, rc):
        if rc is None or rc < 0:
            raise RuntimeError("speechPlayer node call failed: %s" % _native.last_error())
        return rc

    def setUtterances(self, frameStart, frames, minSamples, fadeSamples, userIndex=None, isNull=None, noiseSeed=None):
        fs = np.ascontiguousarray(frameStart, dtype=np.int64)
        fr = np.ascontiguousarray(frames, dtype=np.float64).reshape(-1, 47)
        m = np.ascontiguousarray(minSamples, dtype=np.uint32)
        f = np.ascontiguousarray(fadeSamples, dtype=np.uint32)
        assert fs[-1] == len(fr) == len(m) == len(f)
        ix = None if userIndex is None else np.ascontiguousarray(userIndex, dtype=np.int32)
        nu = None if isNull is None else np.ascontiguousarray(isNull, dtype=np.uint8)
        sd = None if noiseSeed is None else np.ascontiguousarray(noiseSeed, dtype=np.uint32)
        p = lambda a: None if a is None else a.ctypes.data
        self._check(self._dll.speechPlayer_node_setUtterances(self._h, len(fs) - 1, p(fs), p(fr), p(m), p(f), p(ix), p(nu), p(sd)))
        self.nUtterances = len(fs) - 1
        per = np.maximum(m.astype(np.int64), np.maximum(f.astype(np.int64), 1) + 1) + 1
        c = np.concatenate([[0], np.cumsum(per)])
        self._lens = c[fs[1:]] - c[fs[:-1]]

    def setIpa(self, texts, speed=1, basePitch=100, inflection=0.5, clauseType=None, noiseSeed=None, voice=None,
               trailing_silence_ms=150.0, textOf=None):
        from .ipa import _text_pointers, _clauses
        ptrs, n, keep = _text_pointers(texts, textOf)
        pitch = np.ascontiguousarray(np.broadcast_to(np.asarray(basePitch, dtype=np.float64), (n,)))
        sd = None if noiseSeed is None else np.ascontiguousarray(noiseSeed, dtype=np.uint32)
        by_name = voice is None or isinstance(voice, str)
        vo = None if by_name else np.ascontiguousarray(np.broadcast_to(np.asarray(voice, dtype=np.int32), (n,)))
        self._check(self._dll.speechPlayer_node_setIpa(self._h, int(self.sampleRate), n, ptrs.ctypes.data, float(speed), pitch.ctypes.data, float(inflection),
                                                       _clauses(clauseType, n), None if vo is None else vo.ctypes.data,
                                                       (voice.encode("utf8") if (by_name and voice) else None),
                                                       -1.0 if trailing_silence_ms is None else float(trailing_silence_ms), None if sd is None else sd.ctypes.data))
        del keep
        self.nUtterances = n
        self._lens = None

    def utteranceSamples(self, u):
        for d in range(self._dll.speechPlayer_node_devices(self._h)):
            mem = self.shardUtterances(d)
            at = np.flatnonzero(mem == u)
            if len(at):
                return self._dll.speechPlayer_batch_utteranceSamples(self._dll.speechPlayer_node_part(self._h, d), int(at[0]))
        raise RuntimeError("NodePlayer.utteranceSamples: utterance %d out of range" % u)

    @property
    def totalSamples(self):
        return self._dll.speechPlayer_node_totalSamples(self._h)

    def shards(self):
        import ctypes
        out = []
        for d in range(self._dll.speechPlayer_node_devices(self._h)):
            a, n, s, dev = ctypes.c_longlong(), ctypes.c_longlong(), ctypes.c_longlong(), ctypes.c_int()
            self._check(self._dll.speechPlayer_node_shardInfo(self._h, d, ctypes.byref(a), ctypes.byref(n), ctypes.byref(s), ctypes.byref(dev)))
            out.append((a.value, n.value, s.value, dev.value))
        return out

    def synthesize(self, wait=True):
        self._check(self._dll.speechPlayer_node_synthesize(self._h))
        if wait:
            self._check(self._dll.speechPlayer_node_wait(self._h))

    def read(self, u):
        if not 0 <= u < self.nUtterances:
            raise RuntimeError("NodePlayer.read: utterance %d out of range" % u)
        n = int(self._lens[u]) if self._lens is not None else int(self.utteranceSamples(u))
        buf = np.zeros(max(n, 1), dtype=np.int16)
        got = self._check(self._dll.speechPlayer_node_read(self._h, u, buf.ctypes.data, n))
        return buf[:got]

    def getLastIndex(self, u):
        return self._dll.speechPlayer_node_getLastIndex(self._h, u)

    def setOption(self, name, value):
        self._check(self._dll.speechPlayer_node_setOption(self._h, name.encode(), int(value)))

    def shardUtterances(self, d):
        n = self._check(self._dll.speechPlayer_node_shardUtterances(self._h, d, None, 0))
        out = np.zeros(max(n, 1), dtype=np.int64)
        self._check(self._dll.speechPlayer_node_shardUtterances(self._h, d, out.ctypes.data, n))
        return out[:n]

    def digests(self):
        out = np.zeros(max(self.nUtterances, 1), dtype=np.uint64)
        for d in range(self._dll.speechPlayer_node_devices(self._h)):
            mem = self.shardUtterances(d)
            part = self._dll.speechPlayer_node_part(self._h, d)
            if not part:
                raise RuntimeError("speechPlayer_node_part(%d) failed: %s" % (d, _native.last_error()))
            per = np.zeros(max(len(mem), 1), dtype=np.uint64)
            self._check(self._dll.speechPlayer_batch_digest(part, per.ctypes.data, None))
            out[mem] = per[:len(mem)]
        return out[:self.nUtterances]

    def time(self, launches):
        ms = np.zeros(launches, dtype=np.float32)
        self._check(self._dll.speechPlayer_node_time(self._h, launches, ms.ctypes.data))
        return ms

    def close(self):
# ... 10 lines not shown
```

Baseline: 180.0 billion.

## Stage uniform track rows into LDS with cooperative wave-wide loads for flat chunks

When every live lane in a wave has identical track indices and strides for a chunk, the wave loads the whole chunk's track rows cooperatively into a new LDS area, one 128-bit buffer load per lane, and the per-sample bodies then read parameters from LDS. This is meant to replace per-lane scattered buffer loads issued inside each sample with one coalesced bulk load per chunk. In exchange it enlarges LDS for flat kernels, adds ballot and readlane checks per chunk, and raises the launch-bounds minimum waves for flat WPS=1 kernels, which affects register allocation. A counter and API for the number of uniform chunks are added for diagnostics.

```diff
diff --git a/include/speechPlayer_batch.h b/include/speechPlayer_batch.h
--- a/include/speechPlayer_batch.h
+++ b/include/speechPlayer_batch.h
@@ -113,6 +113,7 @@
 long long speechPlayer_batch_readAllAsync(speechPlayer_batch_t batch, sample* sampleBuf, long long capacity, long long* outStart);
 int speechPlayer_batch_readWait(speechPlayer_batch_t batch);
 int speechPlayer_batch_digest(speechPlayer_batch_t batch, unsigned long long* perUtterance, unsigned long long* whole);
+int speechPlayer_batch_uniformChunks(speechPlayer_batch_t batch, unsigned long long* chunks);
 int speechPlayer_batch_getLastIndex(speechPlayer_batch_t batch, long long utterance);
 
 const sample* speechPlayer_batch_devicePcm(speechPlayer_batch_t batch);
diff --git a/nvspeechplayer_amd/_native.py b/nvspeechplayer_amd/_native.py
--- a/nvspeechplayer_amd/_native.py
+++ b/nvspeechplayer_amd/_native.py
@@ -23,7 +23,7 @@
     "speechPlayer_batch_totalSamples", "speechPlayer_batch_totalFrames", "speechPlayer_batch_sampleRate",
     "speechPlayer_batch_synthesize", "speechPlayer_batch_wait", "speechPlayer_batch_read",
     "speechPlayer_batch_readAll", "speechPlayer_batch_readAllAsync", "speechPlayer_batch_readWait", "speechPlayer_hostAlloc", "speechPlayer_hostFree",
-    "speechPlayer_batch_readFloat", "speechPlayer_batch_digest", "speechPlayer_batch_getLastIndex", "speechPlayer_batch_devicePcm",
+    "speechPlayer_batch_readFloat", "speechPlayer_batch_digest", "speechPlayer_batch_uniformChunks", "speechPlayer_batch_getLastIndex", "speechPlayer_batch_devicePcm",
     "speechPlayer_batch_deviceOffset", "speechPlayer_batch_time", "speechPlayer_batch_kernelInfo",
     "speechPlayer_lastError", "speechPlayer_lastErrorCode", "speechPlayer_setNoiseSeed", "speechPlayer_synthesizeMany", "speechPlayer_setGlobalOption",
     "speechPlayer_synthesizeManyDevice", "speechPlayer_lastLiveKernelMs", "speechPlayer_lastLiveLaunches",
@@ -209,6 +209,8 @@
     L.speechPlayer_hostFree.argtypes = [vp]
     L.speechPlayer_batch_digest.restype = i32
     L.speechPlayer_batch_digest.argtypes = [vp, vp, vp]
+    L.speechPlayer_batch_uniformChunks.restype = i32
+    L.speechPlayer_batch_uniformChunks.argtypes = [vp, vp]
     L.speechPlayer_batch_getLastIndex.restype = i32
     L.speechPlayer_batch_getLastIndex.argtypes = [vp, i64]
     L.speechPlayer_batch_devicePcm.restype = vp
diff --git a/nvspeechplayer_amd/csrc/klatt_device.h b/nvspeechplayer_amd/csrc/klatt_device.h
--- a/nvspeechplayer_amd/csrc/klatt_device.h
+++ b/nvspeechplayer_amd/csrc/klatt_device.h
@@ -178,6 +178,8 @@
     double negPiOverSr;
     double twoPiOverSr;
     unsigned long long* debug;
+    unsigned long long* uniformCount;
+    uint32_t uniformRows;
 };
 
 __device__ constexpr int kResF[kNumRes] = {13, 14, 12, 11, 10, 9, 8, 7, 25, 26, 27, 28, 29, 30};
diff --git a/nvspeechplayer_amd/csrc/klatt_engine.hip b/nvspeechplayer_amd/csrc/klatt_engine.hip
--- a/nvspeechplayer_amd/csrc/klatt_engine.hip
+++ b/nvspeechplayer_amd/csrc/klatt_engine.hip
@@ -510,6 +510,9 @@
     long long trackBudgetMB = 4096;
     hipStream_t side[6] = {nullptr, nullptr, nullptr, nullptr, nullptr, nullptr};
     hipEvent_t forkEvent = nullptr, join[6] = {nullptr, nullptr, nullptr, nullptr, nullptr, nullptr};
+    int uniformRows = 1;
+    bool countUniform = false, uniformCounted = false;
+    DeviceBuffer<unsigned long long> dUniform;
     int quietLast = 1;
     long long nUtt = 0, nFrames = 0, nSlots = 0;
     long long nLists = 0, nFramesSpoken = 0;
@@ -1220,6 +1223,12 @@
     const long long nQ = b->nQuiet - nLp - nNn;
     const int parts = (nLp > 0) + (nNn > 0) + (nQ > 0) + (nNoisy > 0) + (nNoisyHead > 0) + (nTr > 0) + (nDir > 0);
     const bool fork = parts > 1;
+    b->uniformCounted = false;
+    if (b->countUniform) {
+        if (b->dUniform.reserve(1)) return -1;
+        HIP_TRY(hipMemsetAsync(b->dUniform.ptr, 0, sizeof(unsigned long long), b->stream));
+        b->uniformCounted = true;
+    }
     if (fork) HIP_TRY(hipEventRecord(b->forkEvent, b->stream));
     int sideUsed = 0, seen = 0;
     auto next_stream = [&](bool = false) -> hipStream_t {
@@ -1264,12 +1273,13 @@
         HIP_TRY(hipGetLastError());
         a.order = b->dOrder.ptr + b->nQuiet; a.nSlots = nTr;
         a.flatRef = b->dFlatRef.ptr; a.sourceRef = b->dSourceRef.ptr; a.track = b->dTrack.ptr;
+        a.uniformRows = b->uniformRows ? 1u : 0u; a.uniformCount = b->countUniform ? b->dUniform.ptr : nullptr;
         a.trackBytes = (uint32_t)std::min<unsigned long long>(((unsigned long long)b->trackEntries + kTrackPad) * sizeof(double2), 0xFFFFFFFFull);
         const GroupPlan pl = plan_group(b->layout, true, b->nSlots, nTr + nNoisy, b->cus);
         const long long g = (nTr + kLanes - 1) / kLanes;
         if (pl.chunk == 8 ? launch_systolic<true, KLATT_FLAT_CH, KLATT_FLAT_WPS, true, false, true>(a, b->mode, g, st)
                           : launch_systolic<true, 16, 1, true, false, true>(a, b->mode, g, st)) return -1;
-        a.flatRef = nullptr; a.sourceRef = nullptr; a.track = nullptr;
+        a.flatRef = nullptr; a.sourceRef = nullptr; a.track = nullptr; a.uniformCount = nullptr;
     }
     if (nDir > 0) {
         hipStream_t st = next_stream();
@@ -2347,7 +2357,7 @@
     b->dDense.release(); b->dDenseStart.release(); b->dFacts.release(); b->hFacts.release();
     b->dRecords.release(); b->dShapeTable.release(); b->dRep.release(); b->dMismatch.release();
     b->dFrames.release(); b->dMeta.release(); b->dUtt.release(); b->dOrder.release(); b->dPcm.release(); b->dResult.release();
-    b->dFloat.release(); b->dDebug.release(); b->dDigest.release(); b->bounce.release();
+    b->dFloat.release(); b->dDebug.release(); b->dDigest.release(); b->dUniform.release(); b->bounce.release();
     b->dFlatRef.release(); b->dSourceRef.release(); b->dJobs.release(); b->dShapes.release(); b->dTrack.release();
     b->dDirectJobs.release(); b->dDirectFirst.release(); b->dDirectHdr.release(); b->dDirectRec.release();
     delete b;
@@ -2364,6 +2374,11 @@
         return 0;
     }
     if (!strcmp(name, "sort")) { b->sortByLength = value ? 1 : 0; return 0; }
+    if (!strcmp(name, "uniform_rows")) {
+        if (value != 0 && value != 1) { set_error("uniform_rows %d: 0 or 1", value); return -1; }
+        b->uniformRows = value;
+        return 0;
+    }
     if (!strcmp(name, "quiet_last")) { b->quietLast = value ? 1 : 0; return 0; }
     if (!strcmp(name, "layout")) { b->layout = value < 0 ? -1 : (value > 2 ? 1 : value); return 0; }
     if (!strcmp(name, "tracks")) { b->tracks = value ? 1 : 0; return 0; }
@@ -3425,6 +3440,20 @@
     return 0;
 }
 
+int speechPlayer_batch_uniformChunks(speechPlayer_batch_t batch, unsigned long long* chunks)
+{
+    begin_call();
+    Batch* b = static_cast<Batch*>(batch);
+    if (!b || !chunks) { set_error("uniformChunks: bad arguments"); return -1; }
+    if (!b->launched) { set_error("uniformChunks: the batch has not been synthesised since it was set"); return -1; }
+    HIP_TRY(hipSetDevice(b->device));
+    b->countUniform = true;
+    if (!b->uniformCounted && batch_launch(b)) return -1;
+    HIP_TRY(hipMemcpyAsync(chunks, b->dUniform.ptr, sizeof(unsigned long long), hipMemcpyDeviceToHost, b->stream));
+    HIP_TRY(hipStreamSynchronize(b->stream));
+    return 0;
+}
+
 int speechPlayer_batch_getLastIndex(speechPlayer_batch_t batch, long long u)
 {
     begin_call();
diff --git a/nvspeechplayer_amd/csrc/klatt_systolic.h b/nvspeechplayer_amd/csrc/klatt_systolic.h
--- a/nvspeechplayer_amd/csrc/klatt_systolic.h
+++ b/nvspeechplayer_amd/csrc/klatt_systolic.h
@@ -55,7 +55,8 @@
     static constexpr int kFrames1 = kFrames + 1 * kParams0 * kLanes * 8;
     static constexpr int kFrames2 = kFrames1 + 2 * kParams1 * kLanes * 8;
     static constexpr int kFrames3 = kFrames2 + 2 * kParams2 * kLanes * 8;
-    static constexpr int kBytes = kFrames3 + 2 * kParams3 * kLanes * 8;
+    static constexpr int kRows = (kFrames3 + 2 * kParams3 * kLanes * 8 + 15) & ~15;
+    static constexpr int kBytes = FLAT ? kRows + CH * (int)(track_stage_entries(0) + track_stage_entries(1) + track_stage_entries(2) + track_stage_entries(3)) * 16 : kFrames3 + 2 * kParams3 * kLanes * 8;
 };
 
 template <int NPARAM, int NRES, bool NWREG = false>
@@ -107,6 +108,7 @@
     const SourceRef* mySrc;
     bool lone = false;
     double* loneLds = nullptr;
+    unsigned char* rowLds = nullptr;
 };
 constexpr int kLoneLdsPerStage = 12288;
 #ifndef KLATT_STREAM_SPLIT
@@ -860,6 +862,93 @@
     }
 };
 struct NoMid { template <class... T> __device__ __forceinline__ void operator()(T...) const {} };
+template <class FD, uint32_t SET>
+__host__ __device__ constexpr int flat_set_entries()
+{
+    int n = 0;
+    for (int e = 0; e < FD::NE; ++e) n += ((SET >> e) & 1u) ? ((FD::ANTI0 && e == 0) ? 2 : 1) : 0;
+    return n;
+}
+__host__ __device__ constexpr int flat_rows_first(int stage, int ch) { int at = 0; for (int k = 0; k < stage; ++k) at += ch * (int)track_stage_entries(k); return at; }
+template <class FD, uint32_t SET, int CH> struct UniformRows { uint32_t off[(CH * flat_set_entries<FD, SET>() + kLanes - 1) / kLanes]; };
+template <class FD, uint32_t SET, int CH>
+__device__ __forceinline__ bool flat2_uniform(const FlatState2<FD>& f, UniformRows<FD, SET, CH>& u)
+{
+    constexpr int NS = flat_set_entries<FD, SET>(), TOT = CH * NS, NP = (TOT + kLanes - 1) / kLanes;
+    static_assert(NS <= (int)track_stage_entries(FD::STAGE), "a row of SET fits the stage's area");
+    const unsigned long long liveMask = __ballot(f.live);
+    if (liveMask == 0ull) return false;
+    const int first = __builtin_ctzll(liveMask);
+    const uint32_t me = threadIdx.x & (kLanes - 1);
+    uint32_t row[NP], ent[NP], base[NP], str[NP];
+#pragma unroll
+    for (int p = 0; p < NP; ++p) { const uint32_t k = me + (uint32_t)(p * kLanes); row[p] = k / (uint32_t)NS; ent[p] = k - row[p] * (uint32_t)NS; base[p] = 0; str[p] = 0; }
+    bool same = true;
+    int at = 0;
+#pragma unroll
+    for (int e = 0; e < FD::NE; ++e) {
+        if (!(SET & (1u << e))) continue;
+        const uint32_t idx = (uint32_t)__builtin_amdgcn_readlane((int)f.idx[e], first), stride = (uint32_t)__builtin_amdgcn_readlane((int)f.stride[e], first);
+        same = same && f.idx[e] == idx && f.stride[e] == stride;
+        const int n = (FD::ANTI0 && e == 0) ? 2 : 1;
+#pragma unroll
+        for (int j = 0; j < n; ++j) {
+#pragma unroll
+            for (int p = 0; p < NP; ++p)
+                if (ent[p] == (uint32_t)(at + j)) { base[p] = idx + 16u * (uint32_t)j; str[p] = stride; }
+        }
+        at += n;
+    }
+#pragma unroll
+    for (int p = 0; p < NP; ++p) u.off[p] = base[p] + row[p] * str[p];
+    return __all(!f.live || same);
+}
+template <class FD, uint32_t SET, int CH>
+__device__ __forceinline__ void flat2_rows_to_lds(FlatState2<FD>& f, const UniformRows<FD, SET, CH>& u, __amdgpu_buffer_rsrc_t rsrc, flat_u4* area)
+{
+    constexpr int TOT = CH * flat_set_entries<FD, SET>();
+    const uint32_t me = threadIdx.x & (kLanes - 1);
+#pragma unroll
+    for (int p = 0; p * kLanes < TOT; ++p) {
+        const uint32_t k = me + (uint32_t)(p * kLanes);
+        if (k < (uint32_t)TOT) area[k] = __builtin_bit_cast(flat_u4, __builtin_amdgcn_raw_buffer_load_b128(rsrc, u.off[p], 0, 0));
+    }
+#pragma unroll
+    for (int e = 0; e < FD::NE; ++e)
+        if (SET & (1u << e)) f.idx[e] += (uint32_t)CH * f.stride[e];
+    __builtin_amdgcn_fence(__ATOMIC_RELEASE, "wavefront");
+    __builtin_amdgcn_wave_barrier();
+    __builtin_amdgcn_fence(__ATOMIC_ACQUIRE, "wavefront");
+}
+__device__ __forceinline__ void flat2_count_uniform(const KernelArgs& A, uint32_t n)
+{
+    if (A.uniformCount && (threadIdx.x & (kLanes - 1)) == 0) atomicAdd(A.uniformCount, (unsigned long long)n);
+}
+template <class FD, uint32_t SET>
+struct FlatTake {
+    FlatState2<FD>& f;
+    const flat_u4* row;
+    template <class... T>
+    __device__ __forceinline__ void operator()(T... firstHalf) const
+    {
+        using R = typename FD::R;
+        (flat_pin(firstHalf), ...);
+        int at = 0;
+#pragma unroll
+        for (int e = 0; e < FD::NE; ++e) {
+            if (!(SET & (1u << e))) continue;
+            const flat_d2 v = __builtin_bit_cast(flat_d2, row[at]);
+            if (e < FD::NRES) {
+                f.rb[e < FD::NRES ? e : 0] = (R)v.x; f.rc[e < FD::NRES ? e : 0] = (R)v.y;
+                if (FD::ANTI0 && e == 0) { f.ra[0] = (R)reinterpret_cast<const double*>(row + at + 1)[0]; ++at; }
+            } else {
+                const int g = e < FD::NRES ? 0 : e - FD::NRES;
+                f.cur[2 * g] = (R)v.x; f.cur[2 * g + 1] = (R)v.y;
+            }
+            ++at;
+        }
+    }
+};
 template <int MODE, bool DERIVE, class R>
 __device__ __forceinline__ ResPre<R> res_pre(R ra, R rb, R rc, R z1, R z2)
 {
@@ -889,6 +978,9 @@
     using R = typename FD::R;
     uint32_t staleG = 0;
     const __amdgpu_buffer_rsrc_t rsrc = __builtin_amdgcn_make_buffer_rsrc(const_cast<double2*>(X.A.track), 0, (int)X.A.trackBytes, 0x00020000);
+    flat_u4* const rowArea = reinterpret_cast<flat_u4*>(X.rowLds) + flat_rows_first(FD::STAGE, CH);
+    UniformRows<FD, FD::USUAL, CH> uni;
+    uint32_t nUniform = 0;
     for (int iter = 0; iter < nIter; ++iter) {
         STAMP_BEGIN();
         STAMP_IDLE();
@@ -941,9 +1033,11 @@
                 continue;
             }
             STAMP_KIND(-1);
-            auto mixedChunk = [&](auto setTag, auto allRowsTag) __attribute__((always_inline)) {
+            auto mixedChunk = [&](auto setTag, auto allRowsTag, auto uniformTag) __attribute__((always_inline)) {
                 constexpr uint32_t SET = decltype(setTag)::value;
                 constexpr bool ALLROWS = decltype(allRowsTag)::value;
+                constexpr bool UNIFORM = decltype(uniformTag)::value;
+                static_assert(!UNIFORM || ALLROWS, "a UNIFORM chunk is an ALLROWS chunk");
                 const uint32_t fix = staleG & ~SET;
                 if (fix) {
 #pragma unroll
@@ -952,6 +1046,12 @@
                     staleG &= SET;
                 }
                 staleG |= SET;
+                if constexpr (UNIFORM) {
+                    flat2_rows_to_lds<FD, SET, CH>(f, uni, rsrc, rowArea);
+                    ++nUniform;
+#pragma unroll KLATT_MIX_UNROLL
+                    for (int i = 0; i < CH; ++i) body(c, i, setTag, FlatTake<FD, SET>{f, rowArea + i * flat_set_entries<FD, SET>()});
+                } else {
 #pragma unroll KLATT_MIX_UNROLL
                 for (int i = 0; i < CH; ++i) {
                     if (!ALLROWS) {
@@ -962,14 +1062,18 @@
                     body(c, i, setTag, FlatMid<FD, SET, ALLROWS>{f, rsrc, has});
                     if (!ALLROWS && has) f.left--;
                 }
+                }
                 if (ALLROWS) f.left = f.left > (uint32_t)CH ? f.left - (uint32_t)CH : 0u;
             };
             constexpr uint32_t ALL = (1u << FD::NE) - 1u;
             const bool usual = FD::USUAL != 0u && FD::USUAL != ALL && c != 0 && (f.wmask & ~FD::USUAL) == 0u;
             const bool allRows = usual && __all(!f.live || (f.left >= (uint32_t)CH && f.startAt > t1));
-            if (allRows) mixedChunk(std::integral_constant<uint32_t, FD::USUAL>{}, std::true_type{});
-            else if (usual) mixedChunk(std::integral_constant<uint32_t, FD::USUAL>{}, std::false_type{});
-            else mixedChunk(std::integral_constant<uint32_t, ALL>{}, std::false_type{});
+            if (allRows) {
+                if (X.A.uniformRows && flat2_uniform<FD, FD::USUAL, CH>(f, uni)) mixedChunk(std::integral_constant<uint32_t, FD::USUAL>{}, std::true_type{}, std::true_type{});
+                else mixedChunk(std::integral_constant<uint32_t, FD::USUAL>{}, std::true_type{}, std::false_type{});
+            }
+            else if (usual) mixedChunk(std::integral_constant<uint32_t, FD::USUAL>{}, std::false_type{}, std::false_type{});
+            else mixedChunk(std::integral_constant<uint32_t, ALL>{}, std::false_type{}, std::false_type{});
             f.produced = f.length < t1 ? f.length : t1;
             perChunk();
         }
@@ -984,10 +1088,11 @@
     }
 #endif
     (void)stampSlot;
+    flat2_count_uniform(X.A, nUniform);
 }
 
 template <int MODE, bool NOISE, int CH, int WPS = KLATT_MINWAVES, bool NASAL = true, bool STREAM = false, bool FLAT = false, bool LONE = false>
-__global__ void __launch_bounds__(kLanes * kStages, WPS) klatt_systolic(const KernelArgs A)
+__global__ void __launch_bounds__(kLanes * kStages, (FLAT && WPS == 1) ? 2 : WPS) klatt_systolic(const KernelArgs A)
 {
     static_assert(!LONE || STREAM, "LONE: a live handle pulled alone");
     static_assert(NASAL || !NOISE, "only quiet launches have a nasal-free instantiation");
@@ -1023,7 +1128,7 @@
     const FrameWindow fw = frame_window(A, d);
     const StageCtx X{A, d, A.frames + fw.base * kNumParams, A.meta + fw.base, fw.off, fw.mask,
                      FLAT ? A.flatRef + d.frameStart : nullptr, FLAT ? A.sourceRef + d.frameStart : nullptr, LONE,
-                     LONE ? reinterpret_cast<double*>(lds + L::kBytes + wave * kLoneLdsPerStage) : nullptr};
+                     LONE ? reinterpret_cast<double*>(lds + L::kBytes + wave * kLoneLdsPerStage) : nullptr, FLAT ? lds + L::kRows : nullptr};
     const uint32_t nkey = noise_key(d.seed), ninc = noise_inc(d.seed), ninc2 = noise_inc2(ninc);
     constexpr int FINAL = NOISE ? 2 : 3;
 #ifndef KLATT_PRELOAD
@@ -1132,6 +1237,9 @@
             };
             auto vib_live = [&]() __attribute__((always_inline)) -> bool { return f.cur[CB + 0] != 0.0 || f.cur[CB + 1] != 0.0 || vibPhase != vibPhase; };
             const __amdgpu_buffer_rsrc_t rsrc = __builtin_amdgcn_make_buffer_rsrc(const_cast<double2*>(A.track), 0, (int)A.trackBytes, 0x00020000);
+            flat_u4* const rowArea = reinterpret_cast<flat_u4*>(X.rowLds) + flat_rows_first(FD::STAGE, CH);
+            UniformRows<FD, kUsualS0, CH> uni;
+            uint32_t nUniform = 0;
 #ifdef KLATT_STAMPS
             Stamps st;
 #endif
@@ -1167,9 +1275,12 @@
                             if (q + 1 < run) { STAMP_WORKED(); sync.end(cc); STAMP_SYNCED(); STAMP_BEGIN(); ++iter; ++cc; sync.begin(cc); lastChunk = cc; }
                         }
                     } else {
-                        auto mixedChunk = [&](auto setTag, auto allFadeTag) __attribute__((always_inline)) {
+                        auto mixedChunk = [&](auto setTag, auto allFadeTag, auto uniformTag) __attribute__((always_inline)) {
                         constexpr uint32_t SET = decltype(setTag)::value;
                         constexpr bool ALLFADE = decltype(allFadeTag)::value;
+                        constexpr bool UNIFORM = decltype(uniformTag)::value;
+                        static_assert(!UNIFORM || ALLFADE, "a UNIFORM chunk is an ALLFADE chunk");
+                        if constexpr (UNIFORM) { flat2_rows_to_lds<FD, SET, CH>(f, uni, rsrc, rowArea); ++nUniform; }
                         const bool vibChunk = (SET & kVibBit) != 0u || __any(vib_live());
                         staleNP = true;
 #pragma unroll KLATT_MIX_UNROLL
@@ -1213,17 +1324,27 @@
                             cntF = fad ? cn : cntF;
                             fadeEndAt = ending ? 0xFFFFFFFFu : fadeEndAt;
                             }
-                            const bool waveVib = vibChunk && __any(vib_live());
+                            static_assert(!UNIFORM || (SET & kVibBit) == 0u, "no vibrato row in a UNIFORM chunk: with nobody's vibrato alive at its top (allFade) none comes alive in it");
+                            const bool waveVib = !UNIFORM && vibChunk && __any(vib_live());
+                            if constexpr (UNIFORM) {
+                                PIPE(pipeX, c, i) = source(waveVib, setTag, FlatTake<FD, SET>{f, rowArea + i * flat_set_entries<FD, SET>()});
+                            } else {
                             const bool has = f.left > 0u;
                             PIPE(pipeX, c, i) = source(waveVib, setTag, FlatMid<FD, SET>{f, rsrc, has});
                             if (has) f.left--;
+                            }
                         }
+                        if (UNIFORM) f.left = f.left > (uint32_t)CH ? f.left - (uint32_t)CH : 0u;
                         };
                         const bool usual = c != 0 && (f.wmask & ~kUsualS0) == 0u;
                         const bool allFade = usual && !__any(vib_live()) && __all(!f.live || (cntF + (uint32_t)CH <= nfU && f.startAt > t1));
-                        if (allFade) mixedChunk(std::integral_constant<uint32_t, kUsualS0>{}, std::true_type{});
-                        else if (usual) mixedChunk(std::integral_constant<uint32_t, kUsualS0>{}, std::false_type{});
-                        else mixedChunk(std::integral_constant<uint32_t, kAllS0>{}, std::false_type{});
+                        if (allFade) {
+                            if (A.uniformRows && __all(!f.live || f.left >= (uint32_t)CH) && flat2_uniform<FD, kUsualS0, CH>(f, uni))
+                                mixedChunk(std::integral_constant<uint32_t, kUsualS0>{}, std::true_type{}, std::true_type{});
+                            else mixedChunk(std::integral_constant<uint32_t, kUsualS0>{}, std::true_type{}, std::false_type{});
+                        }
+                        else if (usual) mixedChunk(std::integral_constant<uint32_t, kUsualS0>{}, std::false_type{}, std::false_type{});
+                        else mixedChunk(std::integral_constant<uint32_t, kAllS0>{}, std::false_type{}, std::false_type{});
                     }
                 }
                 STAMP_WORKED();
@@ -1236,6 +1357,7 @@
                 o[0] = st.work; o[1] = st.wait; o[2] = st.n[0]; o[3] = st.n[1]; o[4] = st.n[2]; o[5] = st.c[0]; o[6] = st.c[1]; o[7] = st.c[2];
             }
 #endif
+            flat2_count_uniform(A, nUniform);
             if (live) {
                 UttResult res;
                 res.produced = d.length; res.framesTaken = f.next; res.lastIndex = lastIndex; res.drained = 1u;
diff --git a/nvspeechplayer_amd/speechPlayer.py b/nvspeechplayer_amd/speechPlayer.py
--- a/nvspeechplayer_amd/speechPlayer.py
+++ b/nvspeechplayer_amd/speechPlayer.py
@@ -924,6 +924,12 @@
         self._check(self._dll.speechPlayer_batch_digest(self._h, None if per is None else per.ctypes.data, ctypes.byref(whole)))
         return (int(whole.value), per[:self.nUtterances]) if per_utterance else int(whole.value)
 
+    def uniformChunks(self):
+        import ctypes
+        n = ctypes.c_ulonglong(0)
+        self._check(self._dll.speechPlayer_batch_uniformChunks(self._h, ctypes.byref(n)))
+        return int(n.value)
+
     def getLastIndex(self, u):
         return self._dll.speechPlayer_batch_getLastIndex(self._h, u)
 
```

After: 159.1 billion. -11.6%, worse.
